# Big-Brother-Pikachu/Where2edit

Hardware: AMD Instinct MI355X
Metric: 1024^2 edited images/sec per mapper step (higher is better)
Workload: dtype f32; 1 GPU; BASELINE configs[1]: FFHQ-1024 StyleGAN2 + clip_loss mapper step (coach.py:79-92), 4 latents/GPU, LevelsMapper, Ranger, id_lambda=0; global_batch=4, per_gpu_batch=4, micro_batch=4, parallelism=dp1, conv_precision=f32, stabilise_steps=6, stabilised=True, hip_graph=True, side_stream=False, clip_precision=f32

## Files before the change

### include/w2e.h

```cpp
#ifndef W2E_H
#define W2E_H

#include <stddef.h>
#include <stdint.h>

#ifdef __cplusplus
extern "C" {
#endif

#define W2E_VERSION 7

int w2e_version(void);
const char* w2e_last_error(void);

int w2e_set_option(const char* name, const char* value);

#define W2E_PLANAR_PITCH(w) ((((w) + 1) + 15) & ~15)
int w2e_get_option(const char* name, int* value);

int w2e_upfirdn2d(const float* x, const float* kern, float* y, int64_t planes, int in_h, int in_w, int out_h,
                  int out_w, int kh, int kw, int up, int down, int pad_x0, int pad_y0, int flip, int in_layout, int in_pitch,
                  int act, const float* out_scale, const float* noise, const float* noise_w, const float* bias,
                  int channels, float slope, float gain, void* stream);
int w2e_blur_adjoint_actbwd(const float* gy, const float* y_fwd, const float* noise, const float* kern, float* gt, float* sums,
                            int64_t planes, int h, int w, float slope, float gain, void* stream);

#define W2E_FIR_GENERIC 0
#define W2E_FIR_DOWN4 1
#define W2E_FIR_TILE 2
#define W2E_FIR_TILE4 3
#define W2E_FIR_BLUR4 4
#define W2E_FIR_STREAM4 5
#define W2E_FIR_PLAN_FIELDS 9
int w2e_upfirdn2d_plan(int64_t planes, int in_h, int in_w, int out_h, int out_w, int kh, int kw, int up, int down, int pad_x0,
                       int in_layout, int in_pitch, int act, int x_misalign, int y_misalign, int64_t* out);
int w2e_upfirdn2d_planar_ok(int kh, int kw, int up, int down, int out_w);
int w2e_blur_adjoint_actbwd_plan(int64_t planes, int h, int w, int kh, int kw, int* fused);

int w2e_bias_act_fwd(const float* x, const float* bias, const float* noise, const float* noise_w, float* y,
                     int64_t outer, int64_t channels, int64_t inner, float slope, float gain, void* stream);
int w2e_bias_act_bwd(const float* gy, const float* y, float* gx, int64_t n, float slope, float gain, void* stream);
int w2e_bias_act_bwd_reduce(const float* gy, const float* y, const float* noise, float* gx, float* sums,
                            int64_t outer, int64_t channels, int64_t inner, float slope, float gain, void* stream);

int w2e_conv_pack(const float* weight, float* wp, int cout, int cin, float scale, int transpose, int flip,
                  void* stream);

#define W2E_CONV_SAME 0
#define W2E_CONV_UP 1
#define W2E_CONV_DOWN 2

int w2e_modconv3x3(int mode, const float* x, const float* wp, const float* in_scale, const float* out_scale,
                   float* y, int batch, int k_ch, int n_ch, int h, int w, int y_pitch, int act, const float* noise,
                   const float* noise_w, const float* bias, const float* dot_with, float* dot_out, void* stream);

#define W2E_CONV_PLAN_FIELDS 15
int w2e_conv3x3_plan(int mode, int batch, int k_ch, int n_ch, int h, int w, int prelu, int down_pad, int64_t* out);

int w2e_modconv_upblur_plan(int batch, int k_ch, int n_ch, int h, int w, int* fused);
int w2e_modconv_upblur(const float* x, const float* wp, const float* in_scale, const float* out_scale, const float* kern,
                       float* y, int batch, int k_ch, int n_ch, int h, int w, const float* noise, const float* noise_w,
                       const float* bias, void* stream);

int w2e_modconv_down_rgbfold_plan(int batch, int k_ch, int n_ch, int h, int w, int* fold);
int w2e_modconv_down_rgbfold(const float* x, const float* wp, const float* in_scale, const float* out_scale, float* gpre, int batch,
                             int k_ch, int n_ch, int h, int w, const float* dot_with, float* dot_out, const float* gy,
                             const float* wrgb, const float* style, const float* noise, float* sums3, float* gw, float slope,
                             float gain, void* stream);

int w2e_wino_weights_fused(const float* wp, float* uf, int k_ch, int n_ch, void* stream);
int w2e_wino_fused(const float* x, const float* in_scale, const float* uf, const float* out_scale, float* y, int batch, int k_ch,
                   int n_ch, int h, int w, int act, const float* noise, const float* noise_w, const float* bias, const float* slope,
                   const float* dot_with, float* dot_out, int wgs, void* stream);

int w2e_wino_pack_input(const float* x, const float* in_scale, float* vf, int batch, int k_ch, int h, int w, int tiles_padded, void* stream);
int w2e_wino_gemm(const float* uf, const float* vf, const float* out_scale, float* y, int batch, int k_ch, int n_ch, int h, int w,
                  int tiles_padded, int splits, float* workspace, int act, const float* noise, const float* noise_w, const float* bias,
                  const float* slope, const float* dot_with, float* dot_out, void* stream);

#define W2E_WINO_GENERATOR 0
#define W2E_WINO_ENCODER 1
#define W2E_WINO_AUTO (-1)
#define W2E_WINO_EPI_PLAIN 0
#define W2E_WINO_EPI_ACT 1
#define W2E_WINO_EPI_PRELU 2
#define W2E_WINO_EPI_DOT 3
#define W2E_WINO_PLAN_FIELDS 6
int w2e_wino_plan(int family, int request, int fused_allowed, int epilogue, int batch, int k_ch, int n_ch, int h, int w, int force_splits,
                  int64_t* out);

int w2e_demod_fwd(const float* s, const float* wsq, float* d, int batch, int cin, int cout, float eps, void* stream);
#define W2E_DEMOD_MAX_LAYERS 32
typedef struct {
    const float* s;
    const float* wsq;
    float* d;
    int cin, cout;
} w2e_demod_layer;
int w2e_demod_all_fwd(const w2e_demod_layer* layers, int n_layers, int batch, float eps, void* stream);
int w2e_demod_bwd(const float* sums, const float* dz, const float* noise_w, const float* bias, const float* d,
                  const float* s, const float* wsq, float* gs, float* gd, int batch, int cin, int cout, void* stream);

int w2e_modconv_wgrad_plan(int mode, int batch, int cin, int cout, int h, int w, int* splits);
int w2e_modconv_wgrad(int mode, const float* g, const float* x, const float* d, const float* s, float* slab, int batch, int cin,
                      int cout, int h, int w, int splits, void* stream);
int w2e_modconv_wgrad_finish(const float* slab, int splits, const float* weight, const float* sums, const float* dz,
                             const float* noise_w, const float* bias, const float* d, const float* s, float* dw, int batch, int cin,
                             int cout, int taps, float scale, void* stream);
int w2e_modconv_wsq(const float* weight, float* wsq, int cout, int cin, int taps, float scale, void* stream);

int w2e_fromrgb_fwd(const float* x, const float* weight, const float* bias, float* y, int batch, int channels, int64_t hw, float scale,
                    void* stream);
int w2e_fromrgb_bwd_rows(int batch, int64_t hw);
int w2e_fromrgb_bwd(const float* gy, const float* y, const float* x, const float* weight, float* gx, float* part, float* dw, float* db,
                    int batch, int channels, int64_t hw, float scale, void* stream);
int w2e_mbstd_fwd(const float* x, float* y, int batch, int channels, int hw, void* stream);
int w2e_mbstd_bwd(const float* gy, const float* x, float* gx, int batch, int channels, int hw, void* stream);
int w2e_fromrgb_jvp(const float* dx, const float* y, const float* weight, float* t, int batch, int channels, int64_t hw, float scale,
                    void* stream);
int w2e_mbstd_jvp(const float* x, const float* dx, float* y, int batch, int channels, int hw, void* stream);
int w2e_mbstd_hvp(const float* gy, const float* x, const float* dx, float* mu, int batch, int channels, int hw, void* stream);
int w2e_sumsq_rows_parts(int64_t n);
int w2e_sumsq_rows(const float* x, float* part, float* out, int batch, int64_t n, void* stream);

int w2e_style_affine_fwd(const float* latent, const float* w, const float* bias, const int* meta, float* out, int batch,
                         int n_latent, int dim, int rows, void* stream);
int w2e_style_affine_bwd(const float* gout, const float* w, const int* meta, float* glatent, int batch, int n_latent,
                         int dim, int rows, void* stream);

int w2e_torgb_fwd(const float* x, const float* wmod, const float* bias, const float* skip, const float* upk,
                  float* y, int batch, int cin, int h, int w, void* stream);
int w2e_torgb_bwd(const float* x, const float* wmod, const float* gy, float* gx, float* gwmod, int batch, int cin,
                  int h, int w, void* stream);
int w2e_torgb_bwd_acc(const float* x, const float* wmod, const float* gy, const float* gx_acc, float* gx, float* gwmod,
                      int batch, int cin, int h, int w, void* stream);
int w2e_torgb_styled_fwd(const float* x, const float* wsc, const float* style, const float* bias, const float* skip,
                         const float* upk, float* y, int batch, int cin, int h, int w, void* stream);
int w2e_torgb_styled_bwd(const float* x, const float* wsc, const float* style, const float* gy, const float* gx_acc,
                         float* gx, float* gstyle, int batch, int cin, int h, int w, void* stream);
int w2e_torgb_bwd_actbwd(const float* x, const float* wmod, const float* style, const float* gy, const float* gx_acc,
                         const float* noise, float* gpre, float* gw, float* sums3, int batch, int cin, int h, int w, float slope,
                         float gain, void* stream);

int w2e_clip_preproc_fwd(const float* img, float* out, int64_t planes, int size, void* stream);
int w2e_clip_preproc_bwd(const float* gout, float* gimg, int64_t planes, int size, void* stream);

int w2e_id_preproc_fwd(const float* img, float* out, int64_t planes, int size, void* stream);
int w2e_id_preproc_bwd(const float* gout, float* gimg, int64_t planes, int size, void* stream);

int w2e_mask_blend_fwd(const float* a, const float* b, const float* mask, float* out, int batch, int channels,
                       int h, int w, int ms, void* stream);
int w2e_mask_blend_bwd(const float* gout, const float* a, const float* b, const float* mask, float* ga, float* gb,
                       float* gmask, int batch, int channels, int h, int w, int ms, void* stream);

int w2e_mapper_pixelnorm(const float* x, float* h, int batch, int n_latent, int groups, const int* l0, const int* len, void* stream);
int w2e_mapper_linear(int mode, const float* a, const float* y_act, float* out, const float* const* w, const float* const* bias,
                      int batch, int n_latent, int groups, const int* l0, const int* len, float w_scale, float b_scale, int scatter,
                      int gathered, void* stream);
int w2e_mapper_wgrad(const float* gy, const float* y, const float* h_in, float* const* gw, float* const* gb, int batch, int n_latent,
                     int groups, const int* l0, const int* len, float w_scale, float b_scale, int gathered, void* stream);

int w2e_ranger_step(int count, float* const* p, const float* const* grad, float* const* exp_avg, float* const* exp_avg_sq,
                    float* const* slow_buffer, const int64_t* numel, const int64_t* row_len, double beta1, double beta2, double eps,
                    double neg_step_size, int rectified, double decay, int lookahead, double alpha, void* stream);

int w2e_adam_step(int count, float* const* p, const float* const* grad, float* const* exp_avg, float* const* exp_avg_sq,
                  const int64_t* numel, double beta1, double beta2, double eps, double step_size, double bias_correction2_sqrt,
                  double weight_decay, void* stream);

int w2e_ssmapper_pixelnorm(const float* const* x, float* h, int batch, int groups, const int* dims, void* stream);
int w2e_ssmapper_gather(const float* const* src, float* dst, int batch, int groups, const int* dims, void* stream);
int w2e_ssmapper_linear(int mode, const float* a, const float* y_act, float* out, const float* const* w, const float* const* bias,
                        int batch, int groups, const int* dims, const float* w_scale, float b_scale, void* stream);
int w2e_ssmapper_wgrad(const float* gy, const float* y, const float* h_in, float* const* gw, float* const* gb, int batch, int groups,
                       const int* dims, const float* w_scale, float b_scale, void* stream);

#ifdef __cplusplus
}
#endif
#endif
```

### where2edit_amd/coach.py

```python
import os

import torch
from torch import nn

from . import dist as w2e_dist
from .clip_loss import CLIPLoss
from .ranger import Ranger
from .styleclip_mapper import StyleCLIPMapper


FUSED_LOSS_TAIL = os.environ.get("W2E_FUSED_LOSS_TAIL", "1") != "0"


class Coach:
    def __init__(self, opts, net=None, clip_loss=None, id_loss=None, text_inputs=None, device=None, data_parallel=False):
        self.opts = opts
        self.global_step = 0
        self.device = device if device is not None else "cuda:0"
        self.opts.device = self.device
        self.net = (net if net is not None else StyleCLIPMapper(self.opts)).to(self.device)
        self.net.decoder.requires_grad_(False)
        if self.opts.id_lambda > 0:
            if id_loss is None:
                from .id_loss import IDLoss
                id_loss = IDLoss(self.opts)
            self.id_loss = id_loss.to(self.device).eval()
        if self.opts.clip_lambda > 0:
            self.clip_loss = (clip_loss if clip_loss is not None else CLIPLoss(opts)).to(self.device)
        if self.opts.latent_l2_lambda > 0:
            self.latent_l2_loss = nn.MSELoss().to(self.device).eval()
        self.optimizer = self.configure_optimizers()
        if text_inputs is None:
            text_inputs = synthetic_tokens(1)
        self.text_inputs = text_inputs.to(self.device)
        self.bucket = w2e_dist.GradBucket(self.net.mapper.parameters()) if data_parallel else None
        self.best_val_loss = None
        self._side = torch.cuda.Stream(device=self.device) if os.environ.get("W2E_SIDE_STREAM", "0") == "1" else None
        self._side_primed = False
        self.merge_forward = os.environ.get("W2E_MERGE_FORWARD", "1") != "0"

    def configure_optimizers(self):
        params = list(self.net.mapper.parameters())
        if self.opts.optim_name == "adam":
            return torch.optim.Adam(params, lr=self.opts.learning_rate)
        return Ranger(params, lr=self.opts.learning_rate)

    def forward_pair(self, w, mask=None):
        dec = self.net.decoder
        s_space = getattr(self.opts, "work_in_stylespace", False)
        att_layer = getattr(self.opts, "attention_layer", 0)
        if mask is not None and att_layer > 0:
            with torch.no_grad():
                x, _, _, feats = dec([w], input_is_latent=True, randomize_noise=False, truncation=1, return_features=True,
                                     input_is_stylespace=s_space)
            self._x_ready = None
            if callable(mask):
                mask = mask(feats)
            if s_space:
                delta = self.net.mapper(w)
                w_hat = [c + 0.1 * dc for c, dc in zip(w, delta)]
                x_hat, _, w_hat = dec([w_hat], input_is_latent=True, return_latents=True, randomize_noise=False, truncation=1,
                                      input_is_stylespace=True, attention_layer=att_layer, attention_map=mask, feature_map=feats)
                return x, x_hat, w_hat
            w_hat = w + 0.1 * self.net.mapper(w)
            x_hat, w_hat, _ = dec([w_hat], input_is_latent=True, return_latents=True, randomize_noise=False, truncation=1,
                                  attention_layer=att_layer, attention_map=mask, feature_map=feats)
            return x, x_hat, w_hat
        if self.merge_forward and self._side is None and s_space and torch.is_grad_enabled():
            from . import functional as K
            n = w[0].shape[0]
            delta = self.net.mapper(w)
            w_hat = [c + 0.1 * dc for c, dc in zip(w, delta)]
            with K.nograd_prefix(n):
                both, _, codes = dec([[torch.cat([c.detach(), ch]) for c, ch in zip(w, w_hat)]], input_is_latent=True, return_latents=True,
                                     randomize_noise=False, truncation=1, input_is_stylespace=True)
            self._x_ready = None
            return both[:n].detach(), K.tail_rows(both, n), [c[n:] for c in codes]
        if self.merge_forward and self._side is None and not s_space and torch.is_grad_enabled():
            from . import functional as K
            n = w.shape[0]
            w_hat = w + 0.1 * self.net.mapper(w)
            with K.nograd_prefix(n):
                both, lat, _ = dec([torch.cat([w.detach(), w_hat])], input_is_latent=True, return_latents=True, randomize_noise=False,
                                   truncation=1)
            self._x_ready = None
            return both[:n].detach(), K.tail_rows(both, n), lat[n:]
        main = torch.cuda.current_stream()
        if self._side is not None and not self._side_primed:
            with torch.no_grad():
                dec([w[:1]] if not s_space else [[c[:1] for c in w]], input_is_latent=True, randomize_noise=False, truncation=1,
                    input_is_stylespace=s_space)
            self._side_primed = True
        if self._side is not None:
            self._side.wait_stream(main)
            with torch.cuda.stream(self._side), torch.no_grad():
                x, _ = dec([w], input_is_latent=True, randomize_noise=False, truncation=1, input_is_stylespace=s_space)
            x.record_stream(main)
            self._x_ready = self._side.record_event()
        else:
            with torch.no_grad():
                x, _ = dec([w], input_is_latent=True, randomize_noise=False, truncation=1, input_is_stylespace=s_space)
            self._x_ready = None
        if s_space:
            delta = self.net.mapper(w)
            w_hat = [c + 0.1 * dc for c, dc in zip(w, delta)]
            x_hat, _, w_hat = dec([w_hat], input_is_latent=True, return_latents=True, randomize_noise=False,
                                  truncation=1, input_is_stylespace=True)
        else:
            w_hat = w + 0.1 * self.net.mapper(w)
            x_hat, w_hat, _ = dec([w_hat], input_is_latent=True, return_latents=True, randomize_noise=False, truncation=1)
        return x, x_hat, w_hat

    def calc_loss(self, w, x, w_hat, x_hat):
        loss_dict = {}
        loss = 0.0
        if getattr(self, "_x_ready", None) is not None:
            torch.cuda.current_stream().wait_event(self._x_ready)
            self._x_ready = None
        if self.opts.id_lambda > 0:
            loss_id, sim_improvement = self.id_loss(x_hat, x)
            loss_dict["loss_id"] = loss_id.detach()
            loss_dict["id_improve"] = sim_improvement
            loss = loss_id * self.opts.id_lambda
        s_space = getattr(self.opts, "work_in_stylespace", False)
        if self.opts.clip_lambda > 0 and self.opts.latent_l2_lambda > 0 and not s_space and torch.is_tensor(w_hat) and w_hat.is_cuda \
                and w_hat.dtype == torch.float32 and torch.is_tensor(w) and w.shape == w_hat.shape and w.dtype == w_hat.dtype \
                and w.device == w_hat.device and FUSED_LOSS_TAIL:
            from . import vit_hip
            sim = self.clip_loss(x_hat, self.text_inputs)
            tail, loss_dict["loss_clip"], loss_dict["loss_l2_latent"] = vit_hip.step_loss(sim, w_hat, w, self.opts.clip_lambda,
                                                                                            self.opts.latent_l2_lambda)
            loss = tail if self.opts.id_lambda <= 0 else loss + tail
            loss_dict["loss"] = loss.detach()
            return loss, loss_dict
        if self.opts.clip_lambda > 0:
            loss_clip = self.clip_loss(x_hat, self.text_inputs).mean()
            loss_dict["loss_clip"] = loss_clip.detach()
            loss = loss + loss_clip * self.opts.clip_lambda
        if self.opts.latent_l2_lambda > 0:
            if getattr(self.opts, "work_in_stylespace", False):
                loss_l2_latent = sum(self.latent_l2_loss(c_hat, c) for c_hat, c in zip(w_hat, w))
            else:
                loss_l2_latent = self.latent_l2_loss(w_hat, w)
            loss_dict["loss_l2_latent"] = loss_l2_latent.detach()
            loss = loss + loss_l2_latent * self.opts.latent_l2_lambda
        loss_dict["loss"] = loss.detach()
        return loss, loss_dict

    def train_step(self, w, mask=None):
        if self.bucket is not None:
            self.bucket.zero()
        else:
            self.optimizer.zero_grad()
        x, x_hat, w_hat = self.forward_pair(w, mask)
        loss, loss_dict = self.calc_loss(w, x, w_hat, x_hat)
        loss.backward()
        if self.bucket is not None:
            self.bucket.all_reduce_mean()
        self.optimizer.step()
        self.global_step += 1
        return loss_dict

    def accumulated_step(self, chunks, step=None):
        if self.bucket is None:
            raise RuntimeError("accumulated_step needs the flat gradient bucket: build the Coach with data_parallel=True")
        n = len(chunks)
        if n == 1:
            return step(chunks[0]) if step is not None else self.train_step(chunks[0])
        if getattr(self, "_acc", None) is None:
            self._acc = torch.zeros_like(self.bucket.flat)
        self._acc.zero_()
        sums = {}
        for c in chunks:
            if c.shape != chunks[0].shape:
                raise ValueError("accumulated_step: micro-batches must have equal shapes (the mean of means is the mean only then)")
            if step is not None:
                d = step(c, finish=False)
            else:
                self.bucket.zero()
                x, x_hat, w_hat = self.forward_pair(c)
                loss, d = self.calc_loss(c, x, w_hat, x_hat)
                loss.backward()
            self._acc.add_(self.bucket.flat, alpha=1.0 / n)
            for k_, v in d.items():
                if torch.is_tensor(v):
                    sums[k_] = v.detach() / n if k_ not in sums else sums[k_] + v.detach() / n
        self.bucket.flat.copy_(self._acc)
        self.bucket.all_reduce_mean()
        self.optimizer.step()
        self.global_step += 1
        return sums

    def capture_step(self, w, mask=None, warmup=3, side_stream=False):
        from . import profiling
        if profiling._active is not None:
            raise RuntimeError("capture_step: per-kernel HIP-event timing cannot be recorded inside a graph")
        eager_side = self._side
        try:
            if side_stream and self._side is None:
                self._side = torch.cuda.Stream(device=self.device)
            s_space = getattr(self.opts, "work_in_stylespace", False)
            static_w = [c.clone() for c in w] if s_space else w.clone()
            static_mask = mask if (mask is None or callable(mask)) else mask.clone()
            params = list(self.net.mapper.parameters())

            def body():
                if self.bucket is not None:
                    self.bucket.zero()
                else:
                    for p in params:
                        p.grad = None
                x, x_hat, w_hat = self.forward_pair(static_w, static_mask)
                loss, loss_dict = self.calc_loss(static_w, x, w_hat, x_hat)
                loss.backward()
                return loss_dict

            graph, static_out = capture_graph(body, "capture_step: the step", self.device, warmup, leaves=params)
        finally:
            self._side = eager_side
        static_grads = [p.grad for p in params]

        def step(w_new, mask_new=None, finish=True):
            if s_space:
                for dst, src in zip(static_w, w_new):
                    dst.copy_(src)
            else:
                static_w.copy_(w_new)
            if static_mask is not None and mask_new is not None and not callable(static_mask):
                static_mask.copy_(mask_new)
            graph.replay()
            if self.bucket is None:
                for p, g in zip(params, static_grads):
                    p.grad = g
            if not finish:
                return static_out
            if self.bucket is not None:
                self.bucket.all_reduce_mean()
            self.optimizer.step()
            self.global_step += 1
            return static_out

        step.graph = graph
        return step

    def train(self, latents, max_steps=None, generator=None):
        self.net.train()
        max_steps = max_steps if max_steps is not None else self.opts.max_steps
        bs = self.opts.batch_size
        log = []
        while self.global_step < max_steps:
            perm = torch.randperm(latents.shape[0], generator=generator)
            for i in range(0, latents.shape[0] - bs + 1, bs):
                if self.global_step >= max_steps:
                    break
                log.append(self.train_step(latents[perm[i:i + bs]].to(self.device)))
        return log

    @torch.no_grad()
    def validate(self, latents):
        self.net.eval()
        agg = []
        bs = getattr(self.opts, "test_batch_size", 1)
        for i in range(0, min(latents.shape[0], 201 * bs) - bs + 1, bs):
# ... 66 lines not shown
```

### where2edit_amd/csrc/common.h

```cpp
#pragma once
#include <hip/hip_runtime.h>
#include <stdarg.h>
#include <stdint.h>
#include <stdio.h>

#include "../../include/w2e.h"

namespace w2e {

void set_error(const char* fmt, ...);
const char* refusal(const char* fmt, ...);

struct Options {
    int conv_precision;
    int deterministic;
    int tune_cfg, tune_cfg_splits, tune_cfg_mode;
    int tune_upall, tune_dma, tune_fuse;
    int tune_upblur;
    int tune_rgbfold;
    int tune_mw;
    int tune_xcd;
    int tune_print, tune_blur, tune_gemm_s;
    int tune_skip, tune_clock;
};
const Options& options();

static inline bool big_lds_once(const void* fn, unsigned* done_mask, int bytes = 160 * 1024) {
    int dev = 0;
    if (hipGetDevice(&dev) != hipSuccess || dev < 0 || dev >= 32) return false;
    if (*done_mask & (1u << dev)) return true;
    if (hipFuncSetAttribute(fn, hipFuncAttributeMaxDynamicSharedMemorySize, bytes) != hipSuccess) {
        (void)hipGetLastError();
        return false;
    }
    *done_mask |= 1u << dev;
    return true;
}

int cu_count();

#define W2E_REQUIRE(cond, ...)        \
    do {                              \
        if (!(cond)) {                \
            w2e::set_error(__VA_ARGS__); \
            return 1;                 \
        }                             \
    } while (0)

#define W2E_LAUNCH_CHECK(name)                                                          \
    do {                                                                                \
        hipError_t e_ = hipGetLastError();                                              \
        if (e_ != hipSuccess) {                                                         \
            w2e::set_error("%s: launch failed: %s", name, hipGetErrorString(e_));       \
            return 2;                                                                   \
        }                                                                               \
    } while (0)

static inline int64_t ceil_div(int64_t a, int64_t b) { return (a + b - 1) / b; }

hipError_t zero_async(void* p, size_t bytes, hipStream_t s);

static inline int stream_grid(int64_t work_items, int block) {
    int64_t g = ceil_div(work_items, block);
    if (g > 2048) g = 2048;
    if (g < 1) g = 1;
    return (int)g;
}

}
```

### where2edit_amd/csrc/elementwise.hip

```cpp
#include "device.h"

namespace w2e {

template <bool VEC4>
__global__ void bias_act_fwd_kernel(const float* __restrict__ x, const float* __restrict__ bias,
                                    const float* __restrict__ noise, const float* __restrict__ noise_w,
                                    float* __restrict__ y, int64_t total, int64_t C, int64_t inner, float slope,
                                    float gain) {
    const float nw = (noise != nullptr) ? noise_w[0] : 0.f;
    const int64_t step = (int64_t)gridDim.x * blockDim.x;
    if (VEC4) {
        const int64_t n4 = total >> 2;
        for (int64_t q = (int64_t)blockIdx.x * blockDim.x + threadIdx.x; q < n4; q += step) {
            const int64_t e = q << 2;
            float4 v = reinterpret_cast<const float4*>(x)[q];
            float add[4] = {0.f, 0.f, 0.f, 0.f};
            if (inner == 1) {
                const int64_t c = e % C;
                if (bias) {
                    const float4 b = *reinterpret_cast<const float4*>(bias + c);
                    add[0] = b.x, add[1] = b.y, add[2] = b.z, add[3] = b.w;
                }
                if (noise) {
                    const float nz = nw * noise[0];
                    add[0] += nz, add[1] += nz, add[2] += nz, add[3] += nz;
                }
            } else {
                const int64_t i = e % inner;
                const float b = bias ? bias[(e / inner) % C] : 0.f;
                add[0] = add[1] = add[2] = add[3] = b;
                if (noise) {
                    const float4 nz = *reinterpret_cast<const float4*>(noise + i);
                    add[0] += nw * nz.x, add[1] += nw * nz.y, add[2] += nw * nz.z, add[3] += nw * nz.w;
                }
            }
            float r[4] = {v.x + add[0], v.y + add[1], v.z + add[2], v.w + add[3]};
#pragma unroll
            for (int k = 0; k < 4; ++k) r[k] = (r[k] > 0.f ? r[k] : r[k] * slope) * gain;
            reinterpret_cast<float4*>(y)[q] = make_float4(r[0], r[1], r[2], r[3]);
        }
    } else {
        for (int64_t e = (int64_t)blockIdx.x * blockDim.x + threadIdx.x; e < total; e += step) {
            const int64_t i = e % inner;
            float v = x[e] + (bias ? bias[(e / inner) % C] : 0.f) + (noise ? nw * noise[i] : 0.f);
            y[e] = (v > 0.f ? v : v * slope) * gain;
        }
    }
}

template <bool VEC4>
__global__ void bias_act_bwd_kernel(const float* __restrict__ gy, const float* __restrict__ y, float* __restrict__ gx,
                                    int64_t total, float slope, float gain) {
    const int64_t step = (int64_t)gridDim.x * blockDim.x;
    if (VEC4) {
        const int64_t n4 = total >> 2;
        for (int64_t q = (int64_t)blockIdx.x * blockDim.x + threadIdx.x; q < n4; q += step) {
            const float4 g = reinterpret_cast<const float4*>(gy)[q];
            const float4 o = reinterpret_cast<const float4*>(y)[q];
            float4 r;
            r.x = g.x * gain * (o.x > 0.f ? 1.f : slope);
            r.y = g.y * gain * (o.y > 0.f ? 1.f : slope);
            r.z = g.z * gain * (o.z > 0.f ? 1.f : slope);
            r.w = g.w * gain * (o.w > 0.f ? 1.f : slope);
            reinterpret_cast<float4*>(gx)[q] = r;
        }
    } else {
        for (int64_t e = (int64_t)blockIdx.x * blockDim.x + threadIdx.x; e < total; e += step)
            gx[e] = gy[e] * gain * (y[e] > 0.f ? 1.f : slope);
    }
}

__global__ void bias_act_bwd_reduce_kernel(const float* __restrict__ gy, const float* __restrict__ y,
                                           const float* __restrict__ noise, float* __restrict__ gx,
                                           float* __restrict__ sums, int64_t inner, int splits, float slope,
                                           float gain) {
    const int64_t row = blockIdx.x / splits;
    const int split = blockIdx.x % splits;
    const int64_t per = ((inner + splits - 1) / splits + 3) & ~int64_t(3);
    const int64_t lo = split * per;
    const int64_t hi = (lo + per < inner) ? lo + per : inner;
    const float* g = gy + row * inner;
    const float* o = y + row * inner;
    float* d = gx + row * inner;
    const float inv_pos = 1.f / gain, inv_neg = 1.f / (gain * slope);
    float s0 = 0.f, s1 = 0.f, s2 = 0.f;
    const bool vec = (inner & 3) == 0;
    if (vec) {
        for (int64_t e = lo + threadIdx.x * 4; e < hi; e += blockDim.x * 4) {
            const float4 gv = *reinterpret_cast<const float4*>(g + e);
            const float4 ov = *reinterpret_cast<const float4*>(o + e);
            float4 nz = make_float4(0.f, 0.f, 0.f, 0.f);
            if (noise) nz = *reinterpret_cast<const float4*>(noise + e);
            const float ga[4] = {gv.x, gv.y, gv.z, gv.w}, oa[4] = {ov.x, ov.y, ov.z, ov.w};
            const float na[4] = {nz.x, nz.y, nz.z, nz.w};
            float r[4];
#pragma unroll
            for (int k = 0; k < 4; ++k) {
                const bool pos = oa[k] > 0.f;
                r[k] = ga[k] * gain * (pos ? 1.f : slope);
                s0 += r[k] * (oa[k] * (pos ? inv_pos : inv_neg));
                s1 += r[k] * na[k];
                s2 += r[k];
            }
            *reinterpret_cast<float4*>(d + e) = make_float4(r[0], r[1], r[2], r[3]);
        }
    } else {
        for (int64_t e = lo + threadIdx.x; e < hi; e += blockDim.x) {
            const bool pos = o[e] > 0.f;
            const float r = g[e] * gain * (pos ? 1.f : slope);
            d[e] = r;
            s0 += r * (o[e] * (pos ? inv_pos : inv_neg));
            s1 += r * (noise ? noise[e] : 0.f);
            s2 += r;
        }
    }
    __shared__ float red[4][3];
    s0 = wave_sum(s0), s1 = wave_sum(s1), s2 = wave_sum(s2);
    const int wave = threadIdx.x >> 6;
    if ((threadIdx.x & 63) == 0) red[wave][0] = s0, red[wave][1] = s1, red[wave][2] = s2;
    __syncthreads();
    if (threadIdx.x < 3) {
        const float t = red[0][threadIdx.x] + red[1][threadIdx.x] + red[2][threadIdx.x] + red[3][threadIdx.x];
        if (splits == 1)
            sums[row * 3 + threadIdx.x] = t;
        else
            atomicAdd(&sums[row * 3 + threadIdx.x], t);
    }
}

__global__ void mask_blend_fwd_kernel(const float* __restrict__ a, const float* __restrict__ b,
                                      const float* __restrict__ mask, float* __restrict__ out, int64_t total, int C,
                                      int H, int W, int ms) {
    const float sy = (float)ms / (float)H, sx = (float)ms / (float)W;
    const int64_t step = (int64_t)gridDim.x * blockDim.x;
    for (int64_t e = (int64_t)blockIdx.x * blockDim.x + threadIdx.x; e < total; e += step) {
        const int x = (int)(e % W);
        const int yy = (int)((e / W) % H);
        const int64_t bi = e / ((int64_t)W * H * C);
        const float m = mask[(bi * ms + nearest_src(yy, sy, ms)) * ms + nearest_src(x, sx, ms)];
        out[e] = m * a[e] + (1.f - m) * b[e];
    }
}

__global__ void mask_blend_bwd_kernel(const float* __restrict__ go, const float* __restrict__ a,
                                      const float* __restrict__ b, const float* __restrict__ mask,
                                      float* __restrict__ ga, float* __restrict__ gb, float* __restrict__ gmask, int C,
                                      int H, int W, int ms) {
    const int bi = blockIdx.x / H, yy = blockIdx.x % H;
    const float sy = (float)ms / (float)H, sx = (float)ms / (float)W;
    const int my = nearest_src(yy, sy, ms);
    for (int x = threadIdx.x; x < W; x += blockDim.x) {
        const int mx = nearest_src(x, sx, ms);
        const float m = mask[((int64_t)bi * ms + my) * ms + mx];
        float acc = 0.f;
        for (int c = 0; c < C; ++c) {
            const int64_t e = (((int64_t)bi * C + c) * H + yy) * W + x;
            const float g = go[e];
            ga[e] = m * g;
            if (gb) gb[e] = (1.f - m) * g;
            if (gmask) acc += g * (a[e] - b[e]);
        }
        if (gmask) atomicAdd(&gmask[((int64_t)bi * ms + my) * ms + mx], acc);
    }
}

__device__ __forceinline__ int overlap(int lo, int hi, int s) {
    const int a = lo > 7 * s ? lo : 7 * s;
    const int b = hi < 7 * s + 7 ? hi : 7 * s + 7;
    return b > a ? b - a : 0;
}

__global__ void clip_preproc_fwd_kernel(const float* __restrict__ img, float* __restrict__ out, int64_t total, int size,
                                        int k) {
    const float inv = 1.f / (float)(k * k);
    const int64_t step = (int64_t)gridDim.x * blockDim.x;
    for (int64_t e = (int64_t)blockIdx.x * blockDim.x + threadIdx.x; e < total; e += step) {
        const int X = (int)(e % 224), Y = (int)((e / 224) % 224);
        const int64_t p = e / (224 * 224);
        const float* src = img + p * (int64_t)size * size;
        const int y0 = (k * Y) / 7, y1 = (k * Y + k - 1) / 7, x0 = (k * X) / 7, x1 = (k * X + k - 1) / 7;
        float acc = 0.f;
        for (int yy = y0; yy <= y1; ++yy) {
            const float wy = (float)overlap(k * Y, k * Y + k, yy);
            float row = 0.f;
            for (int xx = x0; xx <= x1; ++xx) row += (float)overlap(k * X, k * X + k, xx) * src[(int64_t)yy * size + xx];
            acc += wy * row;
        }
        out[e] = acc * inv;
    }
}

__global__ void clip_preproc_bwd_kernel(const float* __restrict__ gout, float* __restrict__ gimg, int64_t total,
                                        int size, int k) {
    const float inv = 1.f / (float)(k * k);
    const int64_t step = (int64_t)gridDim.x * blockDim.x;
    for (int64_t e = (int64_t)blockIdx.x * blockDim.x + threadIdx.x; e < total; e += step) {
        const int x = (int)(e % size), y = (int)((e / size) % size);
        const int64_t p = e / ((int64_t)size * size);
        const float* g = gout + p * 224 * 224;
        const int Y0 = (7 * y) / k, Y1 = (7 * y + 6) / k, X0 = (7 * x) / k, X1 = (7 * x + 6) / k;
        float acc = 0.f;
        for (int Y = Y0; Y <= Y1; ++Y) {
            const float wy = (float)overlap(k * Y, k * Y + k, y);
            float row = 0.f;
            for (int X = X0; X <= X1; ++X) row += (float)overlap(k * X, k * X + k, x) * g[Y * 224 + X];
            acc += wy * row;
        }
        gimg[e] = acc * inv;
    }
}

__device__ __forceinline__ int apool_lo(int i) { return (i * 188) / 112; }
__device__ __forceinline__ int apool_hi(int i) { return ((i + 1) * 188 + 111) / 112; }

__global__ void id_preproc_fwd_kernel(const float* __restrict__ img, float* __restrict__ out, int64_t total, int size, int k) {
    const int64_t step = (int64_t)gridDim.x * blockDim.x;
    const float inv_k2 = 1.f / (float)(k * k);
    for (int64_t e = (int64_t)blockIdx.x * blockDim.x + threadIdx.x; e < total; e += step) {
        const int X = (int)(e % 112), Y = (int)((e / 112) % 112);
        const float* src = img + (e / (112 * 112)) * (int64_t)size * size;
        const int r0 = apool_lo(Y), r1 = apool_hi(Y), c0 = apool_lo(X), c1 = apool_hi(X);
        float acc = 0.f;
        for (int r = r0; r < r1; ++r)
            for (int c = c0; c < c1; ++c) {
                const float* blk = src + (int64_t)(35 + r) * k * size + (32 + c) * k;
                float s = 0.f;
                for (int a = 0; a < k; ++a)
                    for (int b = 0; b < k; ++b) s += blk[a * size + b];
                acc += s * inv_k2;
            }
        out[e] = acc / (float)((r1 - r0) * (c1 - c0));
    }
}

__global__ void id_preproc_bwd_kernel(const float* __restrict__ gout, float* __restrict__ gimg, int64_t total, int size, int k) {
    const int64_t step = (int64_t)gridDim.x * blockDim.x;
    const float inv_k2 = 1.f / (float)(k * k);
    for (int64_t e = (int64_t)blockIdx.x * blockDim.x + threadIdx.x; e < total; e += step) {
        const int x = (int)(e % size), y = (int)((e / size) % size);
        const float* g = gout + (e / ((int64_t)size * size)) * 112 * 112;
        const int r = y / k - 35, c = x / k - 32;
        float acc = 0.f;
        if (r >= 0 && r < 188 && c >= 0 && c < 188) {
            const int Yc = (r * 112) / 188, Xc = (c * 112) / 188;
            for (int Y = Yc - 1; Y <= Yc + 1; ++Y) {
                if (Y < 0 || Y >= 112 || r < apool_lo(Y) || r >= apool_hi(Y)) continue;
                const float wy = 1.f / (float)(apool_hi(Y) - apool_lo(Y));
                for (int X = Xc - 1; X <= Xc + 1; ++X) {
                    if (X < 0 || X >= 112 || c < apool_lo(X) || c >= apool_hi(X)) continue;
                    acc += wy / (float)(apool_hi(X) - apool_lo(X)) * g[Y * 112 + X];
                }
            }
        }
        gimg[e] = acc * inv_k2;
    }
}

__global__ __launch_bounds__(256) void demod_fwd_kernel(const float* __restrict__ s, const float* __restrict__ wsq,
                                                        float* __restrict__ d, int B, int Cin, int Cout, float eps) {
    const int lane = threadIdx.x & 63;
    const int row = blockIdx.x * 4 + (threadIdx.x >> 6);
    if (row >= B * Cout) return;
    const int b = row / Cout, o = row - b * Cout;
    float acc = 0.f;
    for (int i = lane; i < Cin; i += 64) {
        const float v = s[(int64_t)b * Cin + i];
        acc += v * v * wsq[(int64_t)o * Cin + i];
    }
    acc = wave_sum(acc);
    if (lane == 0) d[row] = rsqrtf(acc + eps);
}

struct DemodAllLaunch {
    w2e_demod_layer layer[W2E_DEMOD_MAX_LAYERS];
    int batch;
    float eps;
};

__global__ __launch_bounds__(256) void demod_all_fwd_kernel(const DemodAllLaunch L) {
    const w2e_demod_layer& y = L.layer[blockIdx.y];
    const int lane = threadIdx.x & 63;
    const int row = blockIdx.x * 4 + (threadIdx.x >> 6);
    if (row >= L.batch * y.cout) return;
    const int b = row / y.cout, o = row - b * y.cout;
    const float* s = y.s + (int64_t)b * y.cin;
    const float* w = y.wsq + (int64_t)o * y.cin;
    float acc = 0.f;
    for (int i = lane; i < y.cin; i += 64) {
        const float v = s[i];
        acc += v * v * w[i];
    }
    acc = wave_sum(acc);
    if (lane == 0) y.d[row] = rsqrtf(acc + L.eps);
}

constexpr int DEMOD_OCH = 32;
__global__ __launch_bounds__(256) void demod_bwd_kernel(const float* __restrict__ sums, const float* __restrict__ dz_in,
                                                        const float* __restrict__ noise_w, const float* __restrict__ bias,
                                                        const float* __restrict__ d, const float* __restrict__ s,
                                                        const float* __restrict__ wsq, float* __restrict__ gs,
                                                        float* __restrict__ gd_out, int Cin, int Cout) {
    __shared__ float coef[DEMOD_OCH];
    const int b = blockIdx.y;
    const float nw = noise_w ? noise_w[0] : 0.f;
    const bool serial = gridDim.z == 1 && Cout > DEMOD_OCH;
    const int i_ser = blockIdx.x * 256 + threadIdx.x;
    float total = 0.f;
    for (int o_lo = blockIdx.z * DEMOD_OCH; o_lo < Cout; o_lo += DEMOD_OCH) {
    const int o_n = (Cout - o_lo < DEMOD_OCH) ? Cout - o_lo : DEMOD_OCH;
    __syncthreads();
    for (int oo = threadIdx.x; oo < o_n; oo += 256) {
        const int o = o_lo + oo;
        float dz;
        if (sums) {
            const float* q = sums + ((int64_t)b * Cout + o) * 3;
            dz = q[0] - nw * q[1] - (bias ? bias[o] : 0.f) * q[2];
        } else {
            dz = dz_in[(int64_t)b * Cout + o];
        }
        const float dv = d[(int64_t)b * Cout + o];
        coef[oo] = dz * dv * dv;
        if (gd_out && blockIdx.x == 0) gd_out[(int64_t)b * Cout + o] = dz / dv;
    }
    __syncthreads();
    const int i = blockIdx.x * 256 + threadIdx.x;
    float acc = 0.f;
    if (i < Cin) {
        const float* wq = wsq + (int64_t)o_lo * Cin + i;
#pragma unroll 16
        for (int oo = 0; oo < o_n; ++oo) acc += coef[oo] * wq[(int64_t)oo * Cin];
    }
    if (!serial) {
        if (i < Cin) atomicAdd(&gs[(int64_t)b * Cin + i], -s[(int64_t)b * Cin + i] * acc);
        return;
    }
    total += acc;
    }
    if (i_ser < Cin) gs[(int64_t)b * Cin + i_ser] += -s[(int64_t)b * Cin + i_ser] * total;
}


__global__ __launch_bounds__(256) void style_affine_fwd_kernel(const float* __restrict__ latent, const float* __restrict__ w,
                                                               const float* __restrict__ bias, const int4* __restrict__ meta,
                                                               float* __restrict__ out, int B, int L, int D, int R) {
    const int lane = threadIdx.x & 63;
    const int r = blockIdx.x * 4 + (threadIdx.x >> 6);
    if (r >= R) return;
    const int4 m = meta[r];
    const float bs = bias ? bias[r] : 0.f;
    for (int b = 0; b < B; ++b) {
        const float* lat = latent + ((int64_t)b * L + m.x) * D;
        float acc = 0.f;
        for (int k = lane * 4; k < D; k += 256) {
            const float4 wv = *reinterpret_cast<const float4*>(w + (int64_t)r * D + k);
            const float4 lv = *reinterpret_cast<const float4*>(lat + k);
            acc += wv.x * lv.x + wv.y * lv.y + wv.z * lv.z + wv.w * lv.w;
        }
        acc = wave_sum(acc);
        if (lane == 0) out[(int64_t)m.y * B + (int64_t)b * m.z + m.w] = acc + bs;
    }
}

__global__ __launch_bounds__(256) void style_affine_bwd_kernel(const float* __restrict__ gout, const float* __restrict__ w,
                                                               const int4* __restrict__ meta, float* __restrict__ glatent,
                                                               int B, int L, int D, int R) {
    __shared__ float g[32];
    const int b = blockIdx.y;
    const bool serial = gridDim.x == 1 && R > 32;
    for (int r0 = blockIdx.x * 32; r0 < R; r0 += 32) {
    __syncthreads();
    if (threadIdx.x < 32) {
        const int r = r0 + threadIdx.x;
        float v = 0.f;
        if (r < R) {
            const int4 m = meta[r];
            v = gout[(int64_t)m.y * B + (int64_t)b * m.z + m.w];
        }
        g[threadIdx.x] = v;
    }
    __syncthreads();
    const int widx = meta[r0].x;
    const int nr = (R - r0 < 32) ? R - r0 : 32;
    for (int k = threadIdx.x; k < D; k += 256) {
        float acc = 0.f;
#pragma unroll 8
        for (int i = 0; i < nr; ++i) acc += g[i] * w[(int64_t)(r0 + i) * D + k];
        if (serial) glatent[((int64_t)b * L + widx) * D + k] += acc;
        else atomicAdd(&glatent[((int64_t)b * L + widx) * D + k], acc);
    }
    if (!serial) break;
    }
}

}

using namespace w2e;

extern "C" {


int w2e_bias_act_fwd(const float* x, const float* bias, const float* noise, const float* noise_w, float* y,
                     int64_t outer, int64_t channels, int64_t inner, float slope, float gain, void* stream) {
    W2E_REQUIRE(x && y, "bias_act_fwd: null tensor");
    W2E_REQUIRE(outer >= 0 && channels > 0 && inner > 0, "bias_act_fwd: bad dims %lld %lld %lld", (long long)outer,
                (long long)channels, (long long)inner);
    W2E_REQUIRE(!noise || noise_w, "bias_act_fwd: noise without noise_w");
    const int64_t total = outer * channels * inner;
    if (total == 0) return 0;
    const bool vec = ((inner & 3) == 0) || (inner == 1 && (channels & 3) == 0 && !noise);
    hipStream_t s = (hipStream_t)stream;
    if (vec)
        bias_act_fwd_kernel<true><<<stream_grid(total / 4, 256), 256, 0, s>>>(x, bias, noise, noise_w, y, total,
                                                                                channels, inner, slope, gain);
    else
        bias_act_fwd_kernel<false><<<stream_grid(total, 256), 256, 0, s>>>(x, bias, noise, noise_w, y, total, channels,
                                                                             inner, slope, gain);
    W2E_LAUNCH_CHECK("bias_act_fwd");
    return 0;
}

int w2e_bias_act_bwd(const float* gy, const float* y, float* gx, int64_t n, float slope, float gain, void* stream) {
    W2E_REQUIRE(gy && y && gx, "bias_act_bwd: null tensor");
    if (n <= 0) return 0;
    hipStream_t s = (hipStream_t)stream;
    if ((n & 3) == 0)
        bias_act_bwd_kernel<true><<<stream_grid(n / 4, 256), 256, 0, s>>>(gy, y, gx, n, slope, gain);
    else
        bias_act_bwd_kernel<false><<<stream_grid(n, 256), 256, 0, s>>>(gy, y, gx, n, slope, gain);
    W2E_LAUNCH_CHECK("bias_act_bwd");
    return 0;
}

int w2e_bias_act_bwd_reduce(const float* gy, const float* y, const float* noise, float* gx, float* sums,
                            int64_t outer, int64_t channels, int64_t inner, float slope, float gain, void* stream) {
    W2E_REQUIRE(gy && y && gx && sums, "bias_act_bwd_reduce: null tensor");
    W2E_REQUIRE(slope != 0.f && gain != 0.f, "bias_act_bwd_reduce: slope and gain must be non-zero");
    const int64_t rows = outer * channels;
    if (rows == 0 || inner == 0) return 0;
    hipStream_t s = (hipStream_t)stream;
    int splits = 1;
    if (rows < 2048 && !options().deterministic) {
        splits = (int)ceil_div(2048, rows);
        const int64_t max_splits = ceil_div(inner, 1024);
        if (splits > max_splits) splits = (int)max_splits;
        if (splits < 1) splits = 1;
    }
    W2E_REQUIRE(rows * splits < (int64_t)1 << 31, "bias_act_bwd_reduce: grid too large");
    if (splits > 1 && zero_async(sums, sizeof(float) * 3 * rows, s) != hipSuccess) {
        set_error("bias_act_bwd_reduce: memset failed");
        return 2;
    }
    bias_act_bwd_reduce_kernel<<<(int)(rows * splits), 256, 0, s>>>(gy, y, noise, gx, sums, inner, splits, slope, gain);
    W2E_LAUNCH_CHECK("bias_act_bwd_reduce");
    return 0;
}

int w2e_mask_blend_fwd(const float* a, const float* b, const float* mask, float* out, int batch, int channels, int h,
                       int w, int ms, void* stream) {
    W2E_REQUIRE(a && b && mask && out, "mask_blend_fwd: null tensor");
    W2E_REQUIRE(batch >= 0 && channels > 0 && h > 0 && w > 0 && ms > 0, "mask_blend_fwd: bad dims");
    const int64_t total = (int64_t)batch * channels * h * w;
    if (total == 0) return 0;
    mask_blend_fwd_kernel<<<stream_grid(total, 256), 256, 0, (hipStream_t)stream>>>(a, b, mask, out, total, channels, h,
                                                                                     w, ms);
    W2E_LAUNCH_CHECK("mask_blend_fwd");
    return 0;
}

int w2e_mask_blend_bwd(const float* gout, const float* a, const float* b, const float* mask, float* ga, float* gb,
                       float* gmask, int batch, int channels, int h, int w, int ms, void* stream) {
    W2E_REQUIRE(gout && mask && ga, "mask_blend_bwd: null tensor");
    W2E_REQUIRE(!gmask || (a && b), "mask_blend_bwd: gmask needs a and b");
    W2E_REQUIRE(batch >= 0 && channels > 0 && h > 0 && w > 0 && ms > 0, "mask_blend_bwd: bad dims");
    if (batch == 0) return 0;
    hipStream_t s = (hipStream_t)stream;
    W2E_REQUIRE(!(options().deterministic && gmask && (h != ms || w != ms)),
                "mask_blend_bwd: deterministic mode needs the mask at the feature resolution (%dx%d vs %d)", h, w, ms);
    if (gmask && zero_async(gmask, sizeof(float) * (size_t)batch * ms * ms, s) != hipSuccess) {
        set_error("mask_blend_bwd: memset failed");
        return 2;
    }
    const int threads = w >= 256 ? 256 : (w >= 128 ? 128 : 64);
    mask_blend_bwd_kernel<<<batch * h, threads, 0, s>>>(gout, a, b, mask, ga, gb, gmask, channels, h, w, ms);
    W2E_LAUNCH_CHECK("mask_blend_bwd");
    return 0;
}

int w2e_clip_preproc_fwd(const float* img, float* out, int64_t planes, int size, void* stream) {
    W2E_REQUIRE(img && out, "clip_preproc_fwd: null tensor");
    W2E_REQUIRE(size >= 32 && size % 32 == 0, "clip_preproc_fwd: size %d must be a positive multiple of 32", size);
    const int64_t total = planes * 224 * 224;
    if (total <= 0) return 0;
    clip_preproc_fwd_kernel<<<stream_grid(total, 256), 256, 0, (hipStream_t)stream>>>(img, out, total, size, size / 32);
    W2E_LAUNCH_CHECK("clip_preproc_fwd");
    return 0;
}

int w2e_clip_preproc_bwd(const float* gout, float* gimg, int64_t planes, int size, void* stream) {
    W2E_REQUIRE(gout && gimg, "clip_preproc_bwd: null tensor");
    W2E_REQUIRE(size >= 32 && size % 32 == 0, "clip_preproc_bwd: size %d must be a positive multiple of 32", size);
    const int64_t total = planes * (int64_t)size * size;
    if (total <= 0) return 0;
    clip_preproc_bwd_kernel<<<stream_grid(total, 256), 256, 0, (hipStream_t)stream>>>(gout, gimg, total, size, size / 32);
    W2E_LAUNCH_CHECK("clip_preproc_bwd");
    return 0;
}

int w2e_demod_fwd(const float* s, const float* wsq, float* d, int batch, int cin, int cout, float eps, void* stream) {
    W2E_REQUIRE(s && wsq && d, "demod_fwd: null tensor");
    W2E_REQUIRE(batch >= 0 && cin > 0 && cout > 0, "demod_fwd: bad dims");
    if (batch == 0) return 0;
    demod_fwd_kernel<<<(unsigned)ceil_div((int64_t)batch * cout, 4), 256, 0, (hipStream_t)stream>>>(s, wsq, d, batch, cin, cout, eps);
    W2E_LAUNCH_CHECK("demod_fwd");
    return 0;
}

int w2e_demod_all_fwd(const w2e_demod_layer* layers, int n_layers, int batch, float eps, void* stream) {
    W2E_REQUIRE(layers, "demod_all_fwd: null layers");
    W2E_REQUIRE(n_layers >= 1 && n_layers <= W2E_DEMOD_MAX_LAYERS, "demod_all_fwd: 1 <= n_layers <= %d", W2E_DEMOD_MAX_LAYERS);
    W2E_REQUIRE(batch >= 0, "demod_all_fwd: bad dims");
    if (batch == 0) return 0;
    DemodAllLaunch L{};
    int max_cout = 0;
    for (int j = 0; j < n_layers; ++j) {
        W2E_REQUIRE(layers[j].s && layers[j].wsq && layers[j].d && layers[j].cin > 0 && layers[j].cout > 0,
                    "demod_all_fwd: layer %d: null tensor or bad dims", j);
        L.layer[j] = layers[j];
        if (layers[j].cout > max_cout) max_cout = layers[j].cout;
    }
    L.batch = batch, L.eps = eps;
    dim3 grid((unsigned)ceil_div((int64_t)batch * max_cout, 4), (unsigned)n_layers);
    demod_all_fwd_kernel<<<grid, 256, 0, (hipStream_t)stream>>>(L);
    W2E_LAUNCH_CHECK("demod_all_fwd");
    return 0;
}

int w2e_demod_bwd(const float* sums, const float* dz, const float* noise_w, const float* bias, const float* d,
                  const float* s, const float* wsq, float* gs, float* gd, int batch, int cin, int cout, void* stream) {
    W2E_REQUIRE((sums != nullptr) != (dz != nullptr), "demod_bwd: give exactly one of sums / dz");
    W2E_REQUIRE(d && s && wsq && gs, "demod_bwd: null tensor");
    W2E_REQUIRE(batch >= 0 && cin > 0 && cout > 0 && batch < 65536, "demod_bwd: bad dims");
    if (batch == 0) return 0;
    dim3 grid((unsigned)ceil_div(cin, 256), (unsigned)batch, options().deterministic ? 1u : (unsigned)ceil_div(cout, DEMOD_OCH));
    demod_bwd_kernel<<<grid, 256, 0, (hipStream_t)stream>>>(sums, dz, noise_w, bias, d, s, wsq, gs, gd, cin, cout);
    W2E_LAUNCH_CHECK("demod_bwd");
    return 0;
}

int w2e_id_preproc_fwd(const float* img, float* out, int64_t planes, int size, void* stream) {
    W2E_REQUIRE(img && out, "id_preproc_fwd: null tensor");
    W2E_REQUIRE(size >= 256 && size % 256 == 0, "id_preproc_fwd: size %d must be a positive multiple of 256", size);
    const int64_t total = planes * 112 * 112;
    if (total <= 0) return 0;
    id_preproc_fwd_kernel<<<stream_grid(total, 256), 256, 0, (hipStream_t)stream>>>(img, out, total, size, size / 256);
    W2E_LAUNCH_CHECK("id_preproc_fwd");
    return 0;
}

int w2e_id_preproc_bwd(const float* gout, float* gimg, int64_t planes, int size, void* stream) {
    W2E_REQUIRE(gout && gimg, "id_preproc_bwd: null tensor");
    W2E_REQUIRE(size >= 256 && size % 256 == 0, "id_preproc_bwd: size %d must be a positive multiple of 256", size);
    const int64_t total = planes * (int64_t)size * size;
    if (total <= 0) return 0;
    id_preproc_bwd_kernel<<<stream_grid(total, 256), 256, 0, (hipStream_t)stream>>>(gout, gimg, total, size, size / 256);
    W2E_LAUNCH_CHECK("id_preproc_bwd");
    return 0;
}

int w2e_style_affine_fwd(const float* latent, const float* w, const float* bias, const int* meta, float* out, int batch,
                         int n_latent, int dim, int rows, void* stream) {
    W2E_REQUIRE(latent && w && meta && out, "style_affine_fwd: null tensor");
    W2E_REQUIRE(batch >= 0 && n_latent > 0 && dim > 0 && (dim & 3) == 0 && rows > 0, "style_affine_fwd: bad dims");
    if (batch == 0) return 0;
    style_affine_fwd_kernel<<<(unsigned)ceil_div(rows, 4), 256, 0, (hipStream_t)stream>>>(
        latent, w, bias, reinterpret_cast<const int4*>(meta), out, batch, n_latent, dim, rows);
    W2E_LAUNCH_CHECK("style_affine_fwd");
    return 0;
}

int w2e_style_affine_bwd(const float* gout, const float* w, const int* meta, float* glatent, int batch, int n_latent,
                         int dim, int rows, void* stream) {
    W2E_REQUIRE(gout && w && meta && glatent, "style_affine_bwd: null tensor");
    W2E_REQUIRE(batch >= 0 && batch < 65536 && n_latent > 0 && dim > 0 && rows > 0, "style_affine_bwd: bad dims");
    if (batch == 0) return 0;
    if (zero_async(glatent, sizeof(float) * (size_t)batch * n_latent * dim, (hipStream_t)stream) != hipSuccess) {
        set_error("style_affine_bwd: memset failed");
        return 2;
    }
    dim3 grid(options().deterministic ? 1u : (unsigned)ceil_div(rows, 32), (unsigned)batch);
    style_affine_bwd_kernel<<<grid, 256, 0, (hipStream_t)stream>>>(gout, w, reinterpret_cast<const int4*>(meta), glatent, batch,
                                                                 n_latent, dim, rows);
    W2E_LAUNCH_CHECK("style_affine_bwd");
    return 0;
}


}
```

### where2edit_amd/csrc/runtime.hip

```cpp
#include <stdlib.h>
#include <string.h>

#include "common.h"

namespace w2e {

static thread_local char g_err[512] = "";

void set_error(const char* fmt, ...) {
    va_list ap;
    va_start(ap, fmt);
    vsnprintf(g_err, sizeof(g_err), fmt, ap);
    va_end(ap);
}

const char* refusal(const char* fmt, ...) {
    static thread_local char text[256];
    va_list ap;
    va_start(ap, fmt);
    vsnprintf(text, sizeof(text), fmt, ap);
    va_end(ap);
    return text;
}

static Options g_opt;

static int parse_precision(const char* v) { return (v && strcmp(v, "bf16x3") == 0) ? 1 : 0; }

static bool apply(Options& o, const char* name, const char* value) {
    const int iv = value ? atoi(value) : 0;
    if (!strcmp(name, "conv_precision")) o.conv_precision = parse_precision(value);
    else if (!strcmp(name, "deterministic")) o.deterministic = iv != 0;
    else if (!strcmp(name, "tune_cfg")) {
        o.tune_cfg = -1, o.tune_cfg_splits = 1, o.tune_cfg_mode = -1;
        if (value && *value) sscanf(value, "%d,%d,%d", &o.tune_cfg, &o.tune_cfg_splits, &o.tune_cfg_mode);
    } else if (!strcmp(name, "tune_upall")) o.tune_upall = (value && *value) ? iv : -1;
    else if (!strcmp(name, "tune_dma")) o.tune_dma = (value && *value) ? iv : -1;
    else if (!strcmp(name, "tune_print")) o.tune_print = iv;
    else if (!strcmp(name, "tune_blur")) o.tune_blur = iv;
    else if (!strcmp(name, "tune_gemm_s")) o.tune_gemm_s = iv;
    else if (!strcmp(name, "tune_fuse")) o.tune_fuse = (value && *value) ? iv : -1;
    else if (!strcmp(name, "tune_xcd")) o.tune_xcd = (value && *value) ? iv : -1;
    else if (!strcmp(name, "tune_mw")) o.tune_mw = (value && *value) ? iv : -1;
    else if (!strcmp(name, "tune_upblur")) o.tune_upblur = (value && *value) ? iv : -1;
    else if (!strcmp(name, "tune_rgbfold")) o.tune_rgbfold = (value && *value) ? iv : -1;
#ifdef W2E_TUNING
    else if (!strcmp(name, "tune_skip")) o.tune_skip = iv;
    else if (!strcmp(name, "tune_clock")) o.tune_clock = iv;
#endif
    else return false;
    return true;
}

static Options from_env() {
    Options o{};
    o.tune_cfg = -1, o.tune_cfg_splits = 1, o.tune_cfg_mode = -1, o.tune_upall = -1, o.tune_dma = -1, o.tune_fuse = -1, o.tune_xcd = -1, o.tune_mw = -1, o.tune_upblur = -1, o.tune_rgbfold = -1;
    static const char* const kEnv[][2] = {
        {"W2E_CONV_PRECISION", "conv_precision"}, {"W2E_DETERMINISTIC", "deterministic"}, {"W2E_TUNE_CFG", "tune_cfg"},
        {"W2E_TUNE_UPALL", "tune_upall"},         {"W2E_TUNE_DMA", "tune_dma"},           {"W2E_TUNE_PRINT", "tune_print"},
        {"W2E_TUNE_BLUR", "tune_blur"},           {"W2E_TUNE_GEMM_S", "tune_gemm_s"},     {"W2E_TUNE_FUSE", "tune_fuse"},
        {"W2E_TUNE_SKIP", "tune_skip"},           {"W2E_TUNE_CLOCK", "tune_clock"},       {"W2E_TUNE_XCD", "tune_xcd"},
        {"W2E_TUNE_MW", "tune_mw"},               {"W2E_TUNE_UPBLUR", "tune_upblur"},
        {"W2E_TUNE_RGBFOLD", "tune_rgbfold"}};
    for (const auto& e : kEnv)
        if (const char* v = getenv(e[0])) apply(o, e[1], v);
    return o;
}

struct OptionsInit {
    OptionsInit() { g_opt = from_env(); }
};
static OptionsInit g_opt_init;

const Options& options() { return g_opt; }

int cu_count() {
    static int cached[32];
    int dev = 0;
    if (hipGetDevice(&dev) != hipSuccess || dev < 0 || dev >= 32) return 256;
    if (!cached[dev]) {
        hipDeviceProp_t prop;
        cached[dev] = (hipGetDeviceProperties(&prop, dev) == hipSuccess && prop.multiProcessorCount > 0) ? prop.multiProcessorCount : 256;
    }
    return cached[dev];
}

__global__ void zero_kernel(unsigned* __restrict__ p, size_t words) {
    const size_t step = (size_t)gridDim.x * blockDim.x;
    for (size_t i = (size_t)blockIdx.x * blockDim.x + threadIdx.x; i < words; i += step) p[i] = 0u;
}

__global__ void zero4_kernel(uint4* __restrict__ p, size_t quads) {
    const size_t step = (size_t)gridDim.x * blockDim.x;
    for (size_t i = (size_t)blockIdx.x * blockDim.x + threadIdx.x; i < quads; i += step) p[i] = make_uint4(0u, 0u, 0u, 0u);
}

hipError_t zero_async(void* p, size_t bytes, hipStream_t s) {
    if (bytes == 0) return hipSuccess;
    if ((bytes & 3) != 0 || ((uintptr_t)p & 3) != 0) return hipErrorInvalidValue;
    if (((uintptr_t)p & 15) == 0 && (bytes & 15) == 0) {
        const size_t quads = bytes >> 4;
        zero4_kernel<<<stream_grid((int64_t)quads, 256), 256, 0, s>>>(reinterpret_cast<uint4*>(p), quads);
    } else {
        const size_t words = bytes >> 2;
        zero_kernel<<<stream_grid((int64_t)words, 256), 256, 0, s>>>(reinterpret_cast<unsigned*>(p), words);
    }
    return hipGetLastError();
}

}

extern "C" {

int w2e_version(void) { return W2E_VERSION; }
const char* w2e_last_error(void) { return w2e::g_err; }

int w2e_set_option(const char* name, const char* value) {
    W2E_REQUIRE(name != nullptr, "set_option: null name");
    W2E_REQUIRE(w2e::apply(w2e::g_opt, name, value), "set_option: unknown option '%s'", name);
    return 0;
}

int w2e_get_option(const char* name, int* value) {
    W2E_REQUIRE(name && value, "get_option: null argument");
    const w2e::Options& o = w2e::g_opt;
    if (!strcmp(name, "conv_precision")) *value = o.conv_precision;
    else if (!strcmp(name, "deterministic")) *value = o.deterministic;
    else if (!strcmp(name, "tune_cfg")) *value = o.tune_cfg;
    else if (!strcmp(name, "tune_fuse")) *value = o.tune_fuse;
    else if (!strcmp(name, "tune_blur")) *value = o.tune_blur;
    else if (!strcmp(name, "tune_upblur")) *value = o.tune_upblur;
    else if (!strcmp(name, "tune_rgbfold")) *value = o.tune_rgbfold;
    else if (!strcmp(name, "tuning_build")) {
#ifdef W2E_TUNING
        *value = 1;
#else
        *value = 0;
#endif
    } else W2E_REQUIRE(false, "get_option: unknown option '%s'", name);
    return 0;
}

}
```

### where2edit_amd/csrc/torgb.hip

```cpp
#include "device.h"

namespace w2e {

template <int CG, int V>
__global__ __launch_bounds__(256) void torgb_fwd_kernel(const float* __restrict__ x, const float* __restrict__ wmod,
                                                        const float* __restrict__ style,
                                                        const float* __restrict__ bias, const float* __restrict__ skip,
                                                        const float* __restrict__ upk, float* __restrict__ y, int cin,
                                                        int H, int W) {
    constexpr int PQ = 256 / CG;
    extern __shared__ __attribute__((aligned(16))) float smem[];
    float* wsm = smem;
    float* red = smem + 3 * cin;
    __shared__ float kf[16];
    const int b = blockIdx.y, tid = threadIdx.x;
    const int64_t HW = (int64_t)H * W;
    if (style) {
        for (int i = tid; i < cin; i += 256) {
            const float st = style[(int64_t)b * cin + i];
            wsm[i] = wmod[i] * st, wsm[cin + i] = wmod[cin + i] * st, wsm[2 * cin + i] = wmod[2 * cin + i] * st;
        }
    } else {
        for (int i = tid; i < 3 * cin; i += 256) wsm[i] = wmod[(int64_t)b * 3 * cin + i];
    }
    if (tid < 16 && skip) kf[tid] = upk[15 - tid];
    __syncthreads();
    const int cg = tid / PQ, pq = tid % PQ;
    const int64_t p0 = ((int64_t)blockIdx.x * PQ + pq) * V;
    float acc[3][V];
#pragma unroll
    for (int c = 0; c < 3; ++c)
#pragma unroll
        for (int v = 0; v < V; ++v) acc[c][v] = 0.f;
    if (p0 < HW) {
        const float* xp = x + (int64_t)b * cin * HW + p0;
#pragma unroll 4
        for (int i = cg; i < cin; i += CG) {
            float xv[V];
            if (V == 4) {
                const float4 t = *reinterpret_cast<const float4*>(xp + i * HW);
                xv[0] = t.x, xv[1] = t.y, xv[2] = t.z, xv[3] = t.w;
            } else {
                xv[0] = xp[i * HW];
            }
            const float w0 = wsm[i], w1 = wsm[cin + i], w2 = wsm[2 * cin + i];
#pragma unroll
            for (int v = 0; v < V; ++v) acc[0][v] += w0 * xv[v], acc[1][v] += w1 * xv[v], acc[2][v] += w2 * xv[v];
        }
    }
    if (CG > 1) {
#pragma unroll
        for (int c = 0; c < 3; ++c)
#pragma unroll
            for (int v = 0; v < V; ++v) red[(cg * PQ + pq) * 3 * V + c * V + v] = acc[c][v];
        __syncthreads();
        if (cg != 0) return;
        for (int g = 1; g < CG; ++g)
#pragma unroll
            for (int c = 0; c < 3; ++c)
#pragma unroll
                for (int v = 0; v < V; ++v) acc[c][v] += red[(g * PQ + pq) * 3 * V + c * V + v];
    }
    if (p0 >= HW) return;
    const int Hs = H >> 1, Ws = W >> 1;
#pragma unroll
    for (int c = 0; c < 3; ++c) {
        const float bs = bias ? bias[c] : 0.f;
#pragma unroll
        for (int v = 0; v < V; ++v) {
            float r = acc[c][v] + bs;
            if (skip) {
                const int py = (int)((p0 + v) / W), px = (int)((p0 + v) % W);
                const float* sp = skip + ((int64_t)b * 3 + c) * Hs * Ws;
                float u = 0.f;
#pragma unroll
                for (int a = 0; a < 2; ++a) {
                    const int ky = (py & 1) + 2 * a, sy = (py + ky - 2) >> 1;
                    if (py + ky - 2 < 0 || sy >= Hs) continue;
#pragma unroll
                    for (int d = 0; d < 2; ++d) {
                        const int kx = (px & 1) + 2 * d, sx = (px + kx - 2) >> 1;
                        if (px + kx - 2 < 0 || sx >= Ws) continue;
                        u += kf[ky * 4 + kx] * sp[sy * Ws + sx];
                    }
                }
                r += u;
            }
            acc[c][v] = r;
        }
        float* dst = y + ((int64_t)b * 3 + c) * HW + p0;
        if (V == 4) *reinterpret_cast<float4*>(dst) = make_float4(acc[c][0], acc[c][1], acc[c][2], acc[c][3]);
        else dst[0] = acc[c][0];
    }
}

template <int V, bool ACC, bool ACTB>
__global__ __launch_bounds__(256) void torgb_bwd_kernel(const float* __restrict__ x, const float* __restrict__ wmod,
                                                        const float* __restrict__ style,
                                                        const float* __restrict__ gy, const float* __restrict__ gx_acc,
                                                        float* __restrict__ gx, float* __restrict__ gwmod, int cin,
                                                        int64_t HW, int splits, int64_t per_split,
                                                        const float* __restrict__ noise, float* __restrict__ sums3, float slope, float gain) {
    const int lane = threadIdx.x & 63, wave = threadIdx.x >> 6;
    const int split = blockIdx.x % splits;
    const int i = (blockIdx.x / splits) * 4 + wave;
    const int b = blockIdx.y;
    if (i >= cin) return;
    float w0, w1, w2;
    if (style) {
        const float st = style[(int64_t)b * cin + i];
        w0 = wmod[i] * st, w1 = wmod[cin + i] * st, w2 = wmod[2 * cin + i] * st;
    } else {
        w0 = wmod[((int64_t)b * 3 + 0) * cin + i], w1 = wmod[((int64_t)b * 3 + 1) * cin + i],
        w2 = wmod[((int64_t)b * 3 + 2) * cin + i];
    }
    const float* xp = x + ((int64_t)b * cin + i) * HW;
    float* gp = gx + ((int64_t)b * cin + i) * HW;
    const float* ap = ACC ? gx_acc + ((int64_t)b * cin + i) * HW : nullptr;
    const float* g0 = gy + (int64_t)b * 3 * HW;
    const int64_t lo = split * per_split, hi = (lo + per_split < HW) ? lo + per_split : HW;
    float s0 = 0.f, s1 = 0.f, s2 = 0.f;
    float t_pre = 0.f, t_noise = 0.f, t_sum = 0.f;
    const float inv_pos = 1.f / gain, inv_neg = 1.f / (gain * slope);
    auto act_bwd = [&](float r, float xval, float nz) __attribute__((always_inline)) {
        const bool pos = xval > 0.f;
        const float g = r * gain * (pos ? 1.f : slope);
        t_pre += g * (xval * (pos ? inv_pos : inv_neg)), t_noise += g * nz, t_sum += g;
        return g;
    };
    if (V == 4) {
#pragma unroll 2
        for (int64_t p = lo + lane * 4; p < hi; p += 256) {
            const float4 xv = *reinterpret_cast<const float4*>(xp + p);
            const float4 a = *reinterpret_cast<const float4*>(g0 + p);
            const float4 bb = *reinterpret_cast<const float4*>(g0 + HW + p);
            const float4 c = *reinterpret_cast<const float4*>(g0 + 2 * HW + p);
            float4 nz = make_float4(0.f, 0.f, 0.f, 0.f);
            if (ACTB && noise) nz = *reinterpret_cast<const float4*>(noise + p);
            float4 r;
            r.x = w0 * a.x + w1 * bb.x + w2 * c.x;
            r.y = w0 * a.y + w1 * bb.y + w2 * c.y;
            r.z = w0 * a.z + w1 * bb.z + w2 * c.z;
            r.w = w0 * a.w + w1 * bb.w + w2 * c.w;
            if (ACC) {
                const float4 av = *reinterpret_cast<const float4*>(ap + p);
                r.x += av.x, r.y += av.y, r.z += av.z, r.w += av.w;
            }
            if (ACTB) r.x = act_bwd(r.x, xv.x, nz.x), r.y = act_bwd(r.y, xv.y, nz.y), r.z = act_bwd(r.z, xv.z, nz.z), r.w = act_bwd(r.w, xv.w, nz.w);
            *reinterpret_cast<float4*>(gp + p) = r;
            s0 += xv.x * a.x + xv.y * a.y + xv.z * a.z + xv.w * a.w;
            s1 += xv.x * bb.x + xv.y * bb.y + xv.z * bb.z + xv.w * bb.w;
            s2 += xv.x * c.x + xv.y * c.y + xv.z * c.z + xv.w * c.w;
        }
    } else {
        for (int64_t p = lo + lane; p < hi; p += 64) {
            const float xv = xp[p], a = g0[p], bb = g0[HW + p], c = g0[2 * HW + p];
            float r = w0 * a + w1 * bb + w2 * c + (ACC ? ap[p] : 0.f);
            if (ACTB) r = act_bwd(r, xv, noise ? noise[p] : 0.f);
            gp[p] = r;
            s0 += xv * a, s1 += xv * bb, s2 += xv * c;
        }
    }
    if (ACTB) {
        t_pre = wave_sum(t_pre), t_noise = wave_sum(t_noise), t_sum = wave_sum(t_sum);
        if (lane == 0) {
            float* d3 = sums3 + ((int64_t)b * cin + i) * 3;
            if (splits == 1) d3[0] = t_pre, d3[1] = t_noise, d3[2] = t_sum;
            else atomicAdd(d3, t_pre), atomicAdd(d3 + 1, t_noise), atomicAdd(d3 + 2, t_sum);
        }
    }
    s0 = wave_sum(s0), s1 = wave_sum(s1), s2 = wave_sum(s2);
    if (lane == 0) {
        if (style) {
            const float g = wmod[i] * s0 + wmod[cin + i] * s1 + wmod[2 * cin + i] * s2;
            float* d = gwmod + (int64_t)b * cin + i;
            if (splits == 1) d[0] = g;
            else atomicAdd(d, g);
        } else {
            float* d = gwmod + (int64_t)b * 3 * cin + i;
            if (splits == 1) d[0] = s0, d[cin] = s1, d[2 * cin] = s2;
            else atomicAdd(d, s0), atomicAdd(d + cin, s1), atomicAdd(d + 2 * cin, s2);
        }
    }
}

}

using namespace w2e;

static int torgb_fwd_impl(const float* x, const float* wmod, const float* style, const float* bias, const float* skip,
                          const float* upk, float* y, int batch, int cin, int h, int w, void* stream) {
    W2E_REQUIRE(x && wmod && y, "torgb_fwd: null tensor");
    W2E_REQUIRE(batch >= 0 && cin > 0 && h > 0 && w > 0, "torgb_fwd: bad dims");
    W2E_REQUIRE(!skip || (upk && (h % 2 == 0) && (w % 2 == 0)), "torgb_fwd: skip needs the 4x4 kernel and even h,w");
    W2E_REQUIRE(batch < 65536, "torgb_fwd: batch too large");
    if (batch == 0) return 0;
    hipStream_t s = (hipStream_t)stream;
    const int64_t hw = (int64_t)h * w;
    const bool vec = (hw & 3) == 0;
    const int v = vec ? 4 : 1;
    const int64_t groups = ceil_div(hw, v);
    const int cg = groups >= 16384 ? 1 : (groups >= 1024 ? 4 : 16);
    const int pq = 256 / cg;
    dim3 grid((unsigned)ceil_div(groups, pq), (unsigned)batch);
    const size_t lds = sizeof(float) * ((size_t)3 * cin + (cg > 1 ? (size_t)256 * 3 * v : 0));
#define W2E_TORGB(CG, V) torgb_fwd_kernel<CG, V><<<grid, 256, lds, s>>>(x, wmod, style, bias, skip, upk, y, cin, h, w)
    if (vec) {
        if (cg == 1) W2E_TORGB(1, 4);
        else if (cg == 4) W2E_TORGB(4, 4);
        else W2E_TORGB(16, 4);
    } else {
        if (cg == 1) W2E_TORGB(1, 1);
        else if (cg == 4) W2E_TORGB(4, 1);
        else W2E_TORGB(16, 1);
    }
#undef W2E_TORGB
    W2E_LAUNCH_CHECK("torgb_fwd");
    return 0;
}

extern "C" int w2e_torgb_fwd(const float* x, const float* wmod, const float* bias, const float* skip, const float* upk,
                             float* y, int batch, int cin, int h, int w, void* stream) {
    return torgb_fwd_impl(x, wmod, nullptr, bias, skip, upk, y, batch, cin, h, w, stream);
}

extern "C" int w2e_torgb_styled_fwd(const float* x, const float* wsc, const float* style, const float* bias, const float* skip,
                                    const float* upk, float* y, int batch, int cin, int h, int w, void* stream) {
    W2E_REQUIRE(style, "torgb_styled_fwd: null style");
    return torgb_fwd_impl(x, wsc, style, bias, skip, upk, y, batch, cin, h, w, stream);
}

static int torgb_bwd_impl(const float* x, const float* wmod, const float* style, const float* gy, const float* gx_acc,
                          float* gx, float* gwmod, int batch, int cin, int h, int w, void* stream, bool actb = false,
                          const float* noise = nullptr, float* sums3 = nullptr, float slope = 0.f, float gain = 1.f);

extern "C" int w2e_torgb_bwd(const float* x, const float* wmod, const float* gy, float* gx, float* gwmod, int batch,
                             int cin, int h, int w, void* stream) {
    return torgb_bwd_impl(x, wmod, nullptr, gy, nullptr, gx, gwmod, batch, cin, h, w, stream);
}

extern "C" int w2e_torgb_bwd_acc(const float* x, const float* wmod, const float* gy, const float* gx_acc, float* gx,
                                 float* gwmod, int batch, int cin, int h, int w, void* stream) {
    return torgb_bwd_impl(x, wmod, nullptr, gy, gx_acc, gx, gwmod, batch, cin, h, w, stream);
}

extern "C" int w2e_torgb_styled_bwd(const float* x, const float* wsc, const float* style, const float* gy,
                                    const float* gx_acc, float* gx, float* gstyle, int batch, int cin, int h, int w,
                                    void* stream) {
    W2E_REQUIRE(style, "torgb_styled_bwd: null style");
    return torgb_bwd_impl(x, wsc, style, gy, gx_acc, gx, gstyle, batch, cin, h, w, stream);
}

extern "C" int w2e_torgb_bwd_actbwd(const float* x, const float* wmod, const float* style, const float* gy, const float* gx_acc,
                                    const float* noise, float* gpre, float* gw, float* sums3, int batch, int cin, int h, int w,
                                    float slope, float gain, void* stream) {
    W2E_REQUIRE(sums3, "torgb_bwd_actbwd: null sums");
    W2E_REQUIRE(gain > 0.f && slope > 0.f, "torgb_bwd_actbwd: gain and slope must be positive");
    return torgb_bwd_impl(x, wmod, style, gy, gx_acc, gpre, gw, batch, cin, h, w, stream, true, noise, sums3, slope, gain);
}

static int torgb_bwd_impl(const float* x, const float* wmod, const float* style, const float* gy, const float* gx_acc,
                          float* gx, float* gwmod, int batch, int cin, int h, int w, void* stream, bool actb, const float* noise,
                          float* sums3, float slope, float gain) {
    W2E_REQUIRE(x && wmod && gy && gx && gwmod, "torgb_bwd: null tensor");
    W2E_REQUIRE(batch >= 0 && cin > 0 && h > 0 && w > 0, "torgb_bwd: bad dims");
    W2E_REQUIRE(batch < 65536, "torgb_bwd: batch too large");
    if (batch == 0) return 0;
    hipStream_t s = (hipStream_t)stream;
    const int64_t hw = (int64_t)h * w;
    const int64_t waves = (int64_t)batch * cin;
    int splits = 1;
    if (waves < 8192 && !options().deterministic) {
        splits = (int)ceil_div(8192, waves);
        const int64_t max_splits = ceil_div(hw, 4096);
        if (splits > max_splits) splits = (int)max_splits;
    }
    int64_t per_split = ceil_div(hw, splits);
    per_split = (per_split + 255) & ~int64_t(255);
    splits = (int)ceil_div(hw, per_split);
    if (splits > 1 && (zero_async(gwmod, sizeof(float) * (style ? 1 : 3) * (size_t)batch * cin, s) != hipSuccess ||
                       (actb && zero_async(sums3, sizeof(float) * 3 * (size_t)batch * cin, s) != hipSuccess))) {
        set_error("torgb_bwd: memset failed");
        return 2;
    }
    dim3 grid((unsigned)(ceil_div(cin, 4) * splits), (unsigned)batch);
#define W2E_TORGB_BWD(V, ACC, ACTB) \
    torgb_bwd_kernel<V, ACC, ACTB><<<grid, 256, 0, s>>>(x, wmod, style, gy, gx_acc, gx, gwmod, cin, hw, splits, per_split, noise, sums3, slope, gain)
    if ((hw & 3) == 0) {
        if (actb) {
            if (gx_acc) W2E_TORGB_BWD(4, true, true);
            else W2E_TORGB_BWD(4, false, true);
        } else {
            if (gx_acc) W2E_TORGB_BWD(4, true, false);
            else W2E_TORGB_BWD(4, false, false);
        }
    } else {
        if (actb) {
            if (gx_acc) W2E_TORGB_BWD(1, true, true);
            else W2E_TORGB_BWD(1, false, true);
        } else {
            if (gx_acc) W2E_TORGB_BWD(1, true, false);
            else W2E_TORGB_BWD(1, false, false);
        }
    }
#undef W2E_TORGB_BWD
    W2E_LAUNCH_CHECK("torgb_bwd");
    return 0;
}
```

### where2edit_amd/csrc/upfirdn2d.hip

```cpp
#include <stdlib.h>

#include "common.h"

namespace w2e {

constexpr int MAXK = 16;

#ifdef W2E_TUNING
#define W2E_BLUR_SKIP(p, bit) (((p).tune & (bit)) != 0)
#else
#define W2E_BLUR_SKIP(p, bit) false
#endif

struct UpfirdnParams {
    const float* x;
    const float* kern;
    float* y;
    int64_t planes;
    int in_h, in_w, out_h, out_w, kh, kw, up, down, pad_x0, pad_y0, flip;
    int tune;
    int planar;
    int act;
    const float* out_scale;
    const float* noise;
    const float* noise_w;
    const float* bias;
    int channels;
    float slope, gain;
    const float* y_fwd;
    float* sums;
};

__device__ __forceinline__ float epilogue(const UpfirdnParams& p, float v, int64_t plane, int oy, int ox, float nw) {
    if (!p.act) return v;
    if (p.out_scale) v *= p.out_scale[plane];
    if (p.noise) v += nw * p.noise[(int64_t)oy * p.out_w + ox];
    if (p.bias) v += p.bias[plane % p.channels];
    return (v > 0.f ? v : v * p.slope) * p.gain;
}

constexpr int TW = 64, TH = 32;
constexpr int MAX_TILE_K = 8;

template <bool ACT>
__global__ __launch_bounds__(256) void upfirdn_tile4_kernel(UpfirdnParams p, int tiles_x, int tiles_y, unsigned pw_magic) {
    extern __shared__ __attribute__((aligned(16))) float smem[];
    float* tile = smem;
    constexpr int PW = TW + 3, PH = TH + 3, PITCH = (PW + 3) & ~3;
    const int tid = threadIdx.x;
    float kr[16];
#pragma unroll
    for (int i = 0; i < 16; ++i) kr[i] = p.flip ? p.kern[15 - i] : p.kern[i];
    const float nw = (ACT && p.noise) ? p.noise_w[0] : 0.f;
    const int tiles_per_plane = tiles_x * tiles_y;
    const int n_tiles = tiles_per_plane * (int)p.planes;
    const int ly = (tid >> 4) * 2, lx = (tid & 15) * 4;
    for (int t = blockIdx.x; t < n_tiles; t += gridDim.x) {
        const int plane = t / tiles_per_plane;
        const int rem = t - plane * tiles_per_plane;
        const int ty = rem / tiles_x, tx = rem - ty * tiles_x;
        const float* src = p.x + (int64_t)plane * p.in_h * p.in_w;
        const int oy0 = ty * TH, ox0 = tx * TW;
        const int iy0 = oy0 - p.pad_y0, ix0 = ox0 - p.pad_x0;
        __syncthreads();
#pragma unroll
        for (int it = 0; it < (PH * PW + 255) / 256; ++it) {
            const int i = tid + it * 256;
            const int r = (int)__umulhi((unsigned)i, pw_magic), c = i - r * PW;
            const int iy = iy0 + r, ix = ix0 + c;
            const bool ok = iy >= 0 && iy < p.in_h && ix >= 0 && ix < p.in_w;
            const int cy = iy < 0 ? 0 : (iy >= p.in_h ? p.in_h - 1 : iy), cx = ix < 0 ? 0 : (ix >= p.in_w ? p.in_w - 1 : ix);
            const float v = W2E_BLUR_SKIP(p, 1) ? 1.f : src[cy * p.in_w + cx];
            if (i < PH * PW) tile[r * PITCH + c] = ok ? v : 0.f;
        }
        __syncthreads();
        float acc0[4] = {0.f, 0.f, 0.f, 0.f}, acc1[4] = {0.f, 0.f, 0.f, 0.f};
#pragma unroll
        for (int r = 0; r < (W2E_BLUR_SKIP(p, 2) ? 1 : 5); ++r) {
            const float4 a = *reinterpret_cast<const float4*>(tile + (ly + r) * PITCH + lx);
            const float4 b = *reinterpret_cast<const float4*>(tile + (ly + r) * PITCH + lx + 4);
            const float win[8] = {a.x, a.y, a.z, a.w, b.x, b.y, b.z, b.w};
#pragma unroll
            for (int kx = 0; kx < 4; ++kx) {
#pragma unroll
                for (int j = 0; j < 4; ++j) {
                    if (r < 4) acc0[j] += kr[r * 4 + kx] * win[kx + j];
                    if (r >= 1) acc1[j] += kr[(r - 1) * 4 + kx] * win[kx + j];
                }
            }
        }
        const int ox = ox0 + lx;
        float e_scale = 1.f, e_bias = 0.f;
        if (ACT) {
            if (p.out_scale) e_scale = p.out_scale[plane];
            if (p.bias) e_bias = p.bias[plane % p.channels];
        }
#pragma unroll
        for (int yy = 0; yy < 2; ++yy) {
            const int oy = oy0 + ly + yy;
            if (oy >= p.out_h || ox >= p.out_w) continue;
            float v[4];
#pragma unroll
            for (int j = 0; j < 4; ++j) {
                float e = yy ? acc1[j] : acc0[j];
                if (ACT) {
                    e = e * e_scale + e_bias;
                    if (p.noise) e += nw * p.noise[oy * p.out_w + (ox + j < p.out_w ? ox + j : ox)];
                    e = (e > 0.f ? e : e * p.slope) * p.gain;
                }
                v[j] = e;
            }
            float* dst = p.y + ((int64_t)plane * p.out_h + oy) * p.out_w + ox;
            if (W2E_BLUR_SKIP(p, 4) && v[0] != 123456.75f) continue;
            if (ox + 3 < p.out_w && (p.out_w & 3) == 0) {
                *reinterpret_cast<float4*>(dst) = make_float4(v[0], v[1], v[2], v[3]);
            } else {
#pragma unroll
                for (int j = 0; j < 4; ++j)
                    if (ox + j < p.out_w) dst[j] = v[j];
            }
        }
    }
}

template <bool ACT, bool PLANAR>
__global__ __launch_bounds__(256) void upfirdn_blur4_kernel(UpfirdnParams p, int tiles_x, int tiles_y) {
    extern __shared__ __attribute__((aligned(16))) float smem[];
    constexpr int PW = TW + 3, PH = TH + 3;
    constexpr int NQ = PLANAR ? ((PW + 1) / 2 + 1 + 3) / 4 + 1 : (PW + 3) / 4 + 1;
    constexpr int PE = 4 * NQ;
    constexpr int SLOTS = (PLANAR ? 2 : 1) * PH * NQ;
    constexpr int NIT = (SLOTS + 255) / 256;
    static_assert(TW == 64 && TH == 32, "thread mapping: 64 lanes along x, 4 waves x 8 rows");
    const int tid = threadIdx.x;
    float kr[16];
#pragma unroll
    for (int i = 0; i < 16; ++i) kr[i] = p.flip ? p.kern[15 - i] : p.kern[i];
    float kh[4], kv[4];
    bool separable = kr[0] != 0.f;
    {
        float kmax = 0.f;
#pragma unroll
        for (int i = 0; i < 16; ++i) kmax = fmaxf(kmax, fabsf(kr[i]));
#pragma unroll
        for (int i = 0; i < 4; ++i) kh[i] = kr[i], kv[i] = separable ? kr[4 * i] / kr[0] : 0.f;
#pragma unroll
        for (int i = 0; i < 16; ++i) separable = separable && fabsf(kr[i] - kv[i >> 2] * kh[i & 3]) <= 1e-7f * kmax;
    }
    const float nw = (ACT && p.noise) ? p.noise_w[0] : 0.f;
    const int hp = (p.in_h + 1) >> 1, wpp = W2E_PLANAR_PITCH((p.in_w - 1) >> 1);
    const int64_t plane_stride = PLANAR ? (int64_t)4 * hp * wpp : (int64_t)p.in_h * p.in_w;
    const int row_len = PLANAR ? wpp : p.in_w;

    const int tx = blockIdx.x % tiles_x, g0 = blockIdx.x / tiles_x, gstep = gridDim.x / tiles_x;
    const int ox0 = tx * TW, ix0 = ox0 - p.pad_x0;
// ... 550 lines not shown
    return up == 1 && down == 1 && kh == 4 && kw == 4 && out_w >= MIN_TILE_W;
}

static int plan_stream4(const char* name, int64_t planes, int out_h, int lanes, FirPlan* pl) {
    const int col_groups = (int)ceil_div(lanes, 64), strips = (int)ceil_div(out_h, SR);
    const int64_t waves = planes * col_groups * strips;
    W2E_REQUIRE(waves < ((int64_t)1 << 31), "%s: tensor too large", name);
    pl->kernel = W2E_FIR_STREAM4, pl->grid = ceil_div(waves, 4), pl->block = 256, pl->lds = 0;
    pl->args[0] = col_groups, pl->args[1] = strips;
    return 0;
}

static int fir_plan(int64_t planes, int in_h, int in_w, int out_h, int out_w, int kh, int kw, int up, int down, int pad_x0, int in_layout,
                    int in_pitch, int act, unsigned x_misalign, unsigned y_misalign, const Options& opt, FirPlan* pl) {
    *pl = FirPlan{};
    W2E_REQUIRE(planes >= 0 && in_h > 0 && in_w > 0 && out_h >= 0 && out_w >= 0, "upfirdn2d: bad sizes");
    W2E_REQUIRE(kh >= 1 && kw >= 1 && kh <= MAXK && kw <= MAXK, "upfirdn2d: kernel %dx%d unsupported (max %d)", kh, kw,
                MAXK);
    W2E_REQUIRE(up >= 1 && down >= 1, "upfirdn2d: up/down must be >= 1");
    const int64_t total = planes * out_h * out_w;
    if (total == 0) return 0;
    W2E_REQUIRE(in_layout == 0 || (in_layout == 1 && planar_ok(kh, kw, up, down, out_w)),
                "upfirdn2d: the phase-planar input layout is implemented for the 4x4, up=down=1 tile kernel only");
    W2E_REQUIRE(in_layout == 0 || in_pitch == W2E_PLANAR_PITCH((in_w - 1) >> 1),
                "upfirdn2d: planar input with a row pitch of %d floats, this library's layout has %d (W2E_PLANAR_PITCH, ABI %d): rebuild the caller",
                in_pitch, W2E_PLANAR_PITCH((in_w - 1) >> 1), W2E_VERSION);
    const int tune = opt.tune_blur;
    pl->act = act != 0, pl->block = 256;
    if (up == 1 && down == 1 && out_w >= MIN_TILE_W && kh <= MAX_TILE_K && kw <= MAX_TILE_K) {
        const int tiles_x = (int)ceil_div(out_w, TW), tiles_y = (int)ceil_div(out_h, TH);
        const int64_t n_tiles = planes * tiles_x * tiles_y;
        W2E_REQUIRE(n_tiles < ((int64_t)1 << 31) && (int64_t)in_h * in_w < ((int64_t)1 << 31), "upfirdn2d: tensor too large");
        const bool aligned_x = x_misalign == 0;
        pl->args[0] = tiles_x, pl->args[1] = tiles_y;
        if (kh == 4 && kw == 4) {
            pl->planar = in_layout;
            const bool vec = !in_layout && (in_w & 3) == 0 && aligned_x;
            const bool stream_ok = !(tune & 8) && out_w >= 256 && aligned_x && y_misalign == 0 &&
                                   (in_layout ? (pad_x0 == 1 && (out_w & 3) == 0 && in_w == out_w + 1)
                                              : (pad_x0 == 2 && (in_w & 3) == 0 && out_w <= in_w + 1));
            if (stream_ok) {
                const int lanes = (!in_layout && out_w == in_w + 1) ? out_w / 4 : (int)ceil_div(out_w, 4);
                return plan_stream4("upfirdn2d", planes, out_h, lanes, pl);
            }
            if (in_layout || vec) {
                const int64_t items = planes * tiles_y;
                int gsteps = 256 * 8 / tiles_x;
                if (gsteps < 1) gsteps = 1;
                if (gsteps > items) gsteps = (int)items;
                constexpr int PWc = TW + 3, PHc = TH + 3;
                pl->kernel = W2E_FIR_BLUR4, pl->grid = gsteps * tiles_x;
                pl->lds = in_layout ? sizeof(float) * 2 * PHc * 4 * (((PWc + 1) / 2 + 1 + 3) / 4 + 1) : sizeof(float) * PHc * 4 * ((PWc + 3) / 4 + 1);
                return 0;
            }
        }
        const int pw = TW + kw - 1, pitch = (pw + 3) & ~3;
        pl->kernel = (kh == 4 && kw == 4) ? W2E_FIR_TILE4 : W2E_FIR_TILE;
        pl->grid = n_tiles < 16384 ? n_tiles : 16384;
        pl->lds = sizeof(float) * (MAXK * MAXK + (size_t)(TH + kh) * pitch + 16);
        pl->args[2] = (unsigned)(((uint64_t)1 << 32) / (unsigned)pw + 1);
    } else if (up == 1 && kh == 4 && kw == 4 && !act && !in_layout && planes * in_h * in_w < ((int64_t)1 << 29) && total < ((int64_t)1 << 31)) {
        pl->kernel = W2E_FIR_DOWN4, pl->grid = ceil_div(total, 256), pl->args[0] = total;
    } else {
        pl->kernel = W2E_FIR_GENERIC, pl->grid = stream_grid(total, 256), pl->args[0] = total;
    }
    return 0;
}

static int fir_plan_actbwd(int64_t planes, int h, int w, const Options& opt, FirPlan* pl) {
    *pl = FirPlan{};
    W2E_REQUIRE(planes >= 0 && h > 0 && w >= 256 && (w & 3) == 0, "blur_adjoint_actbwd: needs a width >= 256 that is a multiple of 4 (got %dx%d)", h, w);
    W2E_REQUIRE(!opt.deterministic, "blur_adjoint_actbwd: the sums are joined with fp32 atomics (use w2e_bias_act_bwd_reduce + w2e_upfirdn2d in deterministic mode)");
    if (planes == 0) return 0;
    W2E_REQUIRE((int64_t)(h + 1) * (w + 1) < ((int64_t)1 << 29), "blur_adjoint_actbwd: plane too large");
    pl->actbwd = 1;
    return plan_stream4("blur_adjoint_actbwd", planes, h + 1, w / 4, pl);
}

static void fir_print(const FirPlan& pl, const UpfirdnParams& p) {
    fprintf(stderr, "upfirdn variant kernel %s act %d planar %d actbwd %d up %d down %d taps %dx%d %lld %dx%d -> %dx%d\n", kFirNames[pl.kernel], pl.act,
            pl.planar, pl.actbwd, p.up, p.down, p.kh, p.kw, (long long)p.planes, p.in_h, p.in_w, p.out_h, p.out_w);
}

static void launch_args(void (*k)(UpfirdnParams, int, int, unsigned), const FirPlan& pl, const UpfirdnParams& p, hipStream_t s) {
    k<<<(unsigned)pl.grid, pl.block, pl.lds, s>>>(p, (int)pl.args[0], (int)pl.args[1], (unsigned)pl.args[2]);
}
static void launch_args(void (*k)(UpfirdnParams, int, int), const FirPlan& pl, const UpfirdnParams& p, hipStream_t s) {
    k<<<(unsigned)pl.grid, pl.block, pl.lds, s>>>(p, (int)pl.args[0], (int)pl.args[1]);
}
static void launch_args(void (*k)(UpfirdnParams, int64_t), const FirPlan& pl, const UpfirdnParams& p, hipStream_t s) {
    k<<<(unsigned)pl.grid, pl.block, pl.lds, s>>>(p, pl.args[0]);
}
template <auto KERNEL>
static void launch_kernel(const FirPlan& pl, const UpfirdnParams& p, hipStream_t s) {
    launch_args(KERNEL, pl, p, s);
}

struct FirEntry {
    int kernel, act, planar, actbwd;
    void (*launch)(const FirPlan&, const UpfirdnParams&, hipStream_t);
};
static const FirEntry kFirTable[] = {
    {W2E_FIR_GENERIC, -1, -1, 0, launch_kernel<upfirdn_generic_kernel>},
    {W2E_FIR_DOWN4, -1, -1, 0, launch_kernel<upfirdn_down4_kernel>},
    {W2E_FIR_TILE, -1, -1, 0, launch_kernel<upfirdn_tile_kernel>},
    {W2E_FIR_TILE4, 0, -1, 0, launch_kernel<upfirdn_tile4_kernel<false>>},
    {W2E_FIR_TILE4, 1, -1, 0, launch_kernel<upfirdn_tile4_kernel<true>>},
    {W2E_FIR_BLUR4, 0, 0, 0, launch_kernel<upfirdn_blur4_kernel<false, false>>},
    {W2E_FIR_BLUR4, 1, 0, 0, launch_kernel<upfirdn_blur4_kernel<true, false>>},
    {W2E_FIR_BLUR4, 0, 1, 0, launch_kernel<upfirdn_blur4_kernel<false, true>>},
    {W2E_FIR_BLUR4, 1, 1, 0, launch_kernel<upfirdn_blur4_kernel<true, true>>},
    {W2E_FIR_STREAM4, 0, 0, 0, launch_kernel<upfirdn_stream4_kernel<false, false>>},
    {W2E_FIR_STREAM4, 1, 0, 0, launch_kernel<upfirdn_stream4_kernel<true, false>>},
    {W2E_FIR_STREAM4, 0, 1, 0, launch_kernel<upfirdn_stream4_kernel<false, true>>},
    {W2E_FIR_STREAM4, 1, 1, 0, launch_kernel<upfirdn_stream4_kernel<true, true>>},
    {W2E_FIR_STREAM4, 0, 0, 1, launch_kernel<upfirdn_stream4_kernel<false, false, true>>},
};

static int fir_launch(const FirPlan& pl, const UpfirdnParams& p, hipStream_t s) {
    for (const FirEntry& e : kFirTable) {
        if (e.kernel == pl.kernel && (e.act < 0 || e.act == pl.act) && (e.planar < 0 || e.planar == pl.planar) && e.actbwd == pl.actbwd) {
            e.launch(pl, p, s);
            return 0;
        }
    }
    set_error("upfirdn2d: internal: kernel %s act %d planar %d actbwd %d not instantiated", kFirNames[pl.kernel], pl.act, pl.planar, pl.actbwd);
    return 1;
}

}

using namespace w2e;

extern "C" int w2e_upfirdn2d(const float* x, const float* kern, float* y, int64_t planes, int in_h, int in_w, int out_h,
                             int out_w, int kh, int kw, int up, int down, int pad_x0, int pad_y0, int flip, int in_layout, int in_pitch,
                             int act, const float* out_scale, const float* noise, const float* noise_w, const float* bias,
                             int channels, float slope, float gain, void* stream) {
    W2E_REQUIRE(x && kern && y, "upfirdn2d: null tensor");
    W2E_REQUIRE(!noise || noise_w, "upfirdn2d: noise without noise_w");
    W2E_REQUIRE(!act || !bias || channels > 0, "upfirdn2d: bias needs channels");
    const Options& opt = options();
    FirPlan pl;
    const int rc = fir_plan(planes, in_h, in_w, out_h, out_w, kh, kw, up, down, pad_x0, in_layout, in_pitch, act, (unsigned)((uintptr_t)x & 15),
                            (unsigned)((uintptr_t)y & 15), opt, &pl);
    if (rc != 0 || pl.grid == 0) return rc;
    const UpfirdnParams p{x, kern, y, planes, in_h, in_w, out_h, out_w, kh, kw, up, down, pad_x0, pad_y0, flip, opt.tune_blur, in_layout,
                          act, out_scale, noise, noise_w, bias, channels > 0 ? channels : 1, slope, gain, nullptr, nullptr};
    if (opt.tune_print) fir_print(pl, p);
    if (fir_launch(pl, p, (hipStream_t)stream) != 0) return 1;
    W2E_LAUNCH_CHECK("upfirdn2d");
    return 0;
}

extern "C" int w2e_blur_adjoint_actbwd(const float* gy, const float* y_fwd, const float* noise, const float* kern, float* gt,
                                       float* sums, int64_t planes, int h, int w, float slope, float gain, void* stream) {
    W2E_REQUIRE(gy && y_fwd && kern && gt && sums, "blur_adjoint_actbwd: null tensor");
    W2E_REQUIRE(((uintptr_t)gy & 15) == 0 && ((uintptr_t)y_fwd & 15) == 0 && ((uintptr_t)gt & 15) == 0 && (!noise || ((uintptr_t)noise & 15) == 0),
                "blur_adjoint_actbwd: tensors must be 16-byte aligned");
    W2E_REQUIRE(gain > 0.f && slope > 0.f, "blur_adjoint_actbwd: gain and slope must be positive");
    const Options& opt = options();
    FirPlan pl;
    const int rc = fir_plan_actbwd(planes, h, w, opt, &pl);
    if (rc != 0 || pl.grid == 0) return rc;
    hipStream_t s = (hipStream_t)stream;
    if (zero_async(sums, sizeof(float) * 3 * (size_t)planes, s) != hipSuccess) {
        set_error("blur_adjoint_actbwd: zero fill failed");
        return 2;
    }
    const UpfirdnParams p{gy, kern, gt, planes, h, w, h + 1, w + 1, 4, 4, 1, 1, 2, 2, 0, opt.tune_blur & 7, 0,
                          0, nullptr, noise, nullptr, nullptr, 1, slope, gain, y_fwd, sums};
    if (opt.tune_print) fir_print(pl, p);
    if (fir_launch(pl, p, s) != 0) return 1;
    W2E_LAUNCH_CHECK("blur_adjoint_actbwd");
    return 0;
}

extern "C" int w2e_upfirdn2d_plan(int64_t planes, int in_h, int in_w, int out_h, int out_w, int kh, int kw, int up, int down, int pad_x0,
                                  int in_layout, int in_pitch, int act, int x_misalign, int y_misalign, int64_t* out) {
    W2E_REQUIRE(out != nullptr, "upfirdn2d_plan: null argument");
    FirPlan pl;
    const int rc = fir_plan(planes, in_h, in_w, out_h, out_w, kh, kw, up, down, pad_x0, in_layout, in_pitch, act, (unsigned)x_misalign & 15,
                            (unsigned)y_misalign & 15, options(), &pl);
    if (rc != 0) return rc;
    const int64_t fields[W2E_FIR_PLAN_FIELDS] = {pl.kernel, pl.act, pl.planar, pl.grid, pl.block, (int64_t)pl.lds, pl.args[0], pl.args[1], pl.args[2]};
    for (int i = 0; i < W2E_FIR_PLAN_FIELDS; ++i) out[i] = fields[i];
    return 0;
}

extern "C" int w2e_upfirdn2d_planar_ok(int kh, int kw, int up, int down, int out_w) { return planar_ok(kh, kw, up, down, out_w) ? 1 : 0; }

extern "C" int w2e_blur_adjoint_actbwd_plan(int64_t planes, int h, int w, int kh, int kw, int* fused) {
    W2E_REQUIRE(fused != nullptr, "blur_adjoint_actbwd_plan: null argument");
    const Options& opt = options();
    FirPlan pl;
    *fused = (opt.tune_fuse != 0 && kh == 4 && kw == 4 && fir_plan_actbwd(planes, h, w, opt, &pl) == 0) ? 1 : 0;
    return 0;
}
```

### where2edit_amd/functional.py

```python
import ctypes
import functools
import math
import os

import torch
from torch.autograd.function import once_differentiable

from . import _lib, profiling
from ._lib import CONSTS, call, ptr, stream_ptr

SQRT2 = math.sqrt(2.0)

_NOGRAD_PREFIX = 0
_POISON = os.environ.get("W2E_DEBUG_POISON", "0") == "1"


def set_debug_poison(on=True):
    global _POISON
    _POISON = bool(on)


def _grad_rows(shape, n_skip, device, like=None):
    buf = torch.empty(shape, device=device, dtype=torch.float32) if like is None else torch.empty_like(like)
    if _POISON and n_skip:
        buf[:n_skip].fill_(float("nan"))
    return buf


class nograd_prefix:
    def __init__(self, n):
        self.n = int(n)

    def __enter__(self):
        global _NOGRAD_PREFIX
        self.prev, _NOGRAD_PREFIX = _NOGRAD_PREFIX, self.n
        return self

    def __exit__(self, *exc):
        global _NOGRAD_PREFIX
        _NOGRAD_PREFIX = self.prev


class _TailRows(torch.autograd.Function):

    @staticmethod
    def forward(ctx, x, n):
        ctx.n, ctx.full = n, x.shape[0]
        return x[n:]

    @staticmethod
    @once_differentiable
    def backward(ctx, g):
        out = _grad_rows((ctx.full,) + tuple(g.shape[1:]), ctx.n, g.device)
        out[ctx.n:].copy_(g)
        return out, None


def tail_rows(x, n):
    return _TailRows.apply(x, n)


class GradPool:

    __slots__ = ("buf", "off", "hint")

    def __init__(self, hint):
        self.buf, self.off, self.hint = None, 0, int(hint)

    def zeros(self, shape, device):
        n = 1
        for v in shape:
            n *= int(v)
        n_al = (n + 63) & ~63
        if self.buf is None or self.off + n_al > self.buf.numel() or self.buf.device != torch.device(device):
            self.buf, self.off = torch.zeros(max(n_al, self.hint), device=device, dtype=torch.float32), 0
        out = self.buf[self.off:self.off + n].view(shape)
        self.off += n_al
        return out


_GRAD_POOL = None


class grad_pool:

    def __init__(self, hint):
        self.pool = GradPool(hint)

    def __enter__(self):
        global _GRAD_POOL
        self.prev, _GRAD_POOL = _GRAD_POOL, self.pool
        return self.pool

    def __exit__(self, *exc):
        global _GRAD_POOL
        _GRAD_POOL = self.prev
        return False


def _zeros_with_tail(full, n, tail_shape, device, pool=None):
    shape = (full,) + tuple(tail_shape)
    buf = pool.zeros(shape, device) if pool is not None else torch.zeros(shape, device=device, dtype=torch.float32)
    return buf, (buf[n:] if n else buf)


def _c(t):
    return t if t.is_contiguous() else t.contiguous()


def _upfirdn2d_raw(x, kernel, out_h, out_w, up, down, pad_x0, pad_y0, flip, act=None, planar_hw=None, out=None):
    n, c = x.shape[0], x.shape[1]
    h, w = planar_hw if planar_hw is not None else (x.shape[2], x.shape[3])
    if planar_hw is not None and tuple(x.shape[2:]) != (2, 2, (h + 1) // 2, planar_pitch((w - 1) // 2)):
        raise RuntimeError(f"upfirdn2d: a phase-planar input of a {h}x{w} image must be [N,C,2,2,{(h + 1) // 2},{planar_pitch((w - 1) // 2)}] "
                           f"(W2E_PLANAR_PITCH, include/w2e.h), got {tuple(x.shape)}")
    kh, kw = kernel.shape
    y = out if out is not None else torch.empty((n, c, out_h, out_w), device=x.device, dtype=torch.float32)
    if act is None:
        a = (0, None, None, None, None, 1, 0.2, SQRT2)
    else:
        out_scale, noise, noise_w, bias = act
        a = (1, ptr(out_scale), ptr(noise), ptr(noise_w), ptr(bias), c, 0.2, SQRT2)
    sp = profiling.span("upfirdn2d", 4.0 * n * c * (h * w + out_h * out_w))
    call("w2e_upfirdn2d", ptr(x), ptr(kernel), ptr(y), n * c, h, w, out_h, out_w, kh, kw, up, down, pad_x0, pad_y0,
         int(flip), int(planar_hw is not None), x.shape[-1] if planar_hw is not None else 0, *a, stream_ptr())
    if sp is not None:
        sp.end()
    return y


_FirPlanFields = ctypes.c_int64 * CONSTS["W2E_FIR_PLAN_FIELDS"]


def upfirdn_plan(planes, in_hw, out_hw, kernel_shape, up=1, down=1, pad_x0=0, planar=False, act=False, x_misalign=0, y_misalign=0):
    out = _FirPlanFields()
    call("w2e_upfirdn2d_plan", planes, *in_hw, *out_hw, *kernel_shape, up, down, pad_x0, int(planar),
         planar_pitch((in_hw[1] - 1) // 2) if planar else 0, int(act), x_misalign, y_misalign, out)
    return out[:]


def fir_planar_ok(kernel_shape, out_w):
    return bool(_lib.load().w2e_upfirdn2d_planar_ok(kernel_shape[0], kernel_shape[1], 1, 1, out_w))


class _UpFirDn2d(torch.autograd.Function):
    @staticmethod
    def forward(ctx, x, kernel, up, down, pad0, pad1):
        x = _c(x)
        kernel = _c(kernel.to(torch.float32))
        n, c, h, w = x.shape
        kh, kw = kernel.shape
        out_h = (h * up + pad0 + pad1 - kh) // down + 1
        out_w = (w * up + pad0 + pad1 - kw) // down + 1
        if out_h <= 0 or out_w <= 0:
            raise RuntimeError(f"upfirdn2d: empty output {out_h}x{out_w}")
        ctx.save_for_backward(kernel)
        ctx.geom = (h, w, up, down, pad0)
        return _upfirdn2d_raw(x, kernel, out_h, out_w, up, down, pad0, pad0, True)

    @staticmethod
    @once_differentiable
    def backward(ctx, gy):
        (kernel,) = ctx.saved_tensors
        h, w, up, down, pad0 = ctx.geom
        kh, kw = kernel.shape
        gx = _upfirdn2d_raw(_c(gy), kernel, h, w, down, up, kw - 1 - pad0, kh - 1 - pad0, False)
        return gx, None, None, None, None, None


def upfirdn2d(input, kernel, up=1, down=1, pad=(0, 0)):
    return _UpFirDn2d.apply(input, kernel, up, down, pad[0], pad[1])


class _BiasAct(torch.autograd.Function):

    @staticmethod
    def forward(ctx, x, bias, slope, gain, channel_last):
        x = _c(x)
        bias = _c(bias)
        if channel_last:
            outer, ch, inner = x.numel() // x.shape[-1], x.shape[-1], 1
        else:
            outer, ch, inner = x.shape[0], x.shape[1], x.numel() // (x.shape[0] * x.shape[1])
        if bias.numel() != ch:
            raise RuntimeError(f"fused_leaky_relu: bias has {bias.numel()} entries, expected {ch}")
        y = torch.empty_like(x)
        call("w2e_bias_act_fwd", ptr(x), ptr(bias), None, None, ptr(y), outer, ch, inner, slope, gain, stream_ptr())
        ctx.save_for_backward(y)
        ctx.cfg = (slope, gain, channel_last, ch)
        return y

    @staticmethod
    @once_differentiable
    def backward(ctx, gy):
        (y,) = ctx.saved_tensors
        slope, gain, channel_last, ch = ctx.cfg
        gy = _c(gy)
        gx = torch.empty_like(y)
        call("w2e_bias_act_bwd", ptr(gy), ptr(y), ptr(gx), y.numel(), slope, gain, stream_ptr())
        gb = None
        if ctx.needs_input_grad[1]:
            gb = gx.reshape(-1, ch).sum(0) if channel_last else gx.reshape(gx.shape[0], ch, -1).sum((0, 2))
        return gx, gb, None, None, None


def fused_leaky_relu(input, bias, negative_slope=0.2, scale=2 ** 0.5):
    if input.ndim < 2:
        raise RuntimeError("fused_leaky_relu expects at least 2 dims")
    channel_last = input.ndim == 3 or input.ndim == 2
    return _BiasAct.apply(input, bias, float(negative_slope), float(scale), channel_last)


def conv_pack(weight, scale, transpose, flip):
    cout, cin = weight.shape[0], weight.shape[1]
    kd, nd = (cout, cin) if transpose else (cin, cout)
    wp = torch.empty(((kd + 7) // 8, 9, 2, nd, 4), device=weight.device, dtype=torch.float32)
    call("w2e_conv_pack", ptr(_c(weight.detach())), ptr(wp), cout, cin, float(scale), int(transpose), int(flip),
         stream_ptr())
    return wp


MODE_SAME, MODE_UP, MODE_DOWN = (CONSTS[f"W2E_CONV_{m}"] for m in ("SAME", "UP", "DOWN"))

def _parse_winograd(v):
    table = {"": "auto", "auto": "auto", "0": False, "4": 4, "8": 8}
    if v not in table:
        raise ValueError(f"W2E_WINOGRAD={v!r}: expected 'auto', '0' (direct kernels), '4' (GEMM form) or '8' (fused form)")
    return table[v]


WINOGRAD = _parse_winograd(os.environ.get("W2E_WINOGRAD", ""))
WINO_LOG = None


FUSED = 8


def set_winograd(mode):
    global WINOGRAD
    if mode not in ("auto", False, 4, 8):
        raise ValueError("set_winograd: 'auto', False, 4 or 8")
    WINOGRAD = mode


FUSED_WGS = 0
GEMM_SPLITS = 0

GENERATOR, ENCODER = CONSTS["W2E_WINO_GENERATOR"], CONSTS["W2E_WINO_ENCODER"]
EPI_PLAIN, EPI_ACT, EPI_PRELU, EPI_DOT = (CONSTS[f"W2E_WINO_EPI_{e}"] for e in ("PLAIN", "ACT", "PRELU", "DOT"))

# ... 143 lines not shown
    n, c = a.shape[0], a.shape[1]
    out = torch.empty_like(a)
    zero = torch.zeros((n, c), device=a.device, dtype=torch.float32)
    call("w2e_se_apply_bwd", ptr(a), ptr(_c(s)), ptr(zero), ptr(out), n, c, a.shape[2] * a.shape[3], stream_ptr())
    return out


def demod_coefficients(s, wsq, eps=1e-8):
    b, cin = s.shape
    cout = wsq.shape[0]
    d = torch.empty((b, cout), device=s.device, dtype=torch.float32)
    call("w2e_demod_fwd", ptr(s), ptr(wsq), ptr(d), b, cin, cout, float(eps), stream_ptr())
    return d


def demod_coefficients_all(styles, wsqs, eps=1e-8):
    b = styles[0].shape[0]
    couts = [w.shape[0] for w in wsqs]
    buf = torch.empty(b * sum(couts), device=styles[0].device, dtype=torch.float32)
    descs = (_lib.DemodLayer * len(styles))()
    out, off = [], 0
    for j, (s, w) in enumerate(zip(styles, wsqs)):
        if s.shape != (b, w.shape[1]) or not s.is_contiguous() or not w.is_contiguous():
            raise RuntimeError(f"demod_coefficients_all: layer {j}: style {tuple(s.shape)} for wsq {tuple(w.shape)}")
        d = buf[off:off + b * couts[j]].view(b, couts[j])
        off += b * couts[j]
        descs[j].s, descs[j].wsq, descs[j].d, descs[j].cin, descs[j].cout = ptr(s).value, ptr(w).value, ptr(d).value, w.shape[1], couts[j]
        out.append(d)
    call("w2e_demod_all_fwd", descs, len(styles), b, float(eps), stream_ptr())
    return out


WGRAD_SAME, WGRAD_UP, WGRAD_CENTRE = 0, 1, 2


def modconv_wsq(weight, scale):
    cout, cin = weight.shape[1], weight.shape[2]
    wsq = torch.empty((cout, cin), device=weight.device, dtype=torch.float32)
    call("w2e_modconv_wsq", ptr(_c(weight.detach())), ptr(wsq), cout, cin, weight.shape[3] * weight.shape[4], float(scale), stream_ptr())
    return wsq


def modconv_wgrad(mode, g, x, d, s, weight, scale, sums=None, dz=None, noise_w=None, bias=None):
    b, cin, h, w = x.shape
    cout = weight.shape[1]
    taps = 1 if mode == WGRAD_CENTRE else 9
    splits = ctypes.c_int(0)
    call("w2e_modconv_wgrad_plan", mode, b, cin, cout, h, w, ctypes.byref(splits))
    slab = torch.empty(splits.value * taps * cout * cin, device=x.device, dtype=torch.float32)
    sp = profiling.span("modconv_wgrad", 2.0 * b * cin * cout * taps * h * w)
    st = stream_ptr()
    call("w2e_modconv_wgrad", mode, ptr(_c(g)), ptr(_c(x)), ptr(d), ptr(_c(s)), ptr(slab), b, cin, cout, h, w, splits.value, st)
    dw = torch.empty(weight.shape, device=x.device, dtype=torch.float32)
    if d is not None:
        call("w2e_modconv_wgrad_finish", ptr(slab), splits.value, ptr(_c(weight.detach())), ptr(sums), ptr(dz), ptr(noise_w), ptr(bias),
             ptr(d), ptr(_c(s)), ptr(dw), b, cin, cout, taps, float(scale), st)
    else:
        call("w2e_modconv_wgrad_finish", ptr(slab), splits.value, None, None, None, None, None, None, None, ptr(dw), b, cin, cout, taps,
             float(scale), st)
    if sp is not None:
        sp.end()
    return dw


def planar_pitch(w):
    return (w + 1 + 15) & ~15


def unplanar(t, in_w):
    b, n, _, _, hp, wpp = t.shape
    w = in_w
    return t.permute(0, 1, 4, 2, 5, 3).reshape(b, n, 2 * hp, 2 * wpp)[:, :, :2 * hp - 1, :2 * w + 1].contiguous()


class ActLink:

    __slots__ = ("noise", "gpre", "sums")

    def __init__(self, noise):
        self.noise, self.gpre, self.sums = noise, None, None

    def take(self, gout):
        gpre, sums = self.gpre, self.sums
        self.gpre = self.sums = None
        if gpre is None:
            return None
        if gpre is not gout:
            raise RuntimeError("where2edit_amd: the gradient of a StyledConv output that was routed through its ToRGB node "
                               "(ActLink) reached the StyledConv backward as a different tensor -- a tensor hook, retain_grad() "
                               "or a second consumer on that activation is not supported on the fused training path "
                               "(use return_features=True / the unfused modules to tap activations)")
        return sums


class RgbFoldLink:

    __slots__ = ("gy", "saved", "gpre", "sums", "gw")

    def __init__(self):
        self.gy = self.saved = self.gpre = self.sums = self.gw = None

    def usable(self, x, n_skip):
        if self.gy is None or self.saved is None:
            return False
        xs, _, _, _, ns = self.saved
        return ns == n_skip and xs.shape[0] == x.shape[0] + n_skip and xs.data_ptr() + 4 * n_skip * xs[0].numel() == x.data_ptr() \
            and tuple(xs.shape[1:]) == tuple(x.shape[1:]) and tuple(self.gy.shape) == (xs.shape[0], 3) + tuple(xs.shape[2:])

    def take(self, gy, gx_next):
        gpre, sums, gw, rec = self.gpre, self.sums, self.gw, self.gy
        self.gpre = self.sums = self.gw = self.gy = None
        if gpre is None:
            return None
        if gx_next is not gpre or gy is not rec:
            raise RuntimeError("where2edit_amd: the ToRGB backward was folded into the stride-2 input-gradient conv of the level above "
                               "(RgbFoldLink), but the gradients reached the ToRGB node as different tensors -- a tensor hook, "
                               "retain_grad() or a second consumer on the passed-through activation or on the RGB skip image is not "
                               "supported on the fused training path (use return_features=True / the unfused modules to tap "
                               "activations, or the option tune_rgbfold = 0)")
        return gpre, sums, gw


class _StyledConv(torch.autograd.Function):

    @staticmethod
    def forward(ctx, x, s, wsq, noise, noise_w, bias, packs, blur_kernel, upsample, fuse_act, link=None, d_pre=None, weight=None,
                wscale=1.0, fold=None):
        x, s = _c(x), _c(s)
        b, cin, h, w = x.shape
        wp_f, wp_b = packs
        d = None
        if wsq is not None:
            d = d_pre if d_pre is not None else demod_coefficients(s, wsq)
        act = (noise, noise_w, bias) if fuse_act else None
        if upsample and fuse_act and tuple(blur_kernel.shape) == (4, 4) and _upblur_planned(b, cin, wp_f.shape[3], h, w):
            out = _modconv_upblur_raw(x, wp_f, s, d, blur_kernel, h, w, act)
        elif upsample:
            t, _ = _modconv_raw(MODE_UP, x, wp_f, s, d, h, w)
            if fir_planar_ok(blur_kernel.shape, 2 * w):
                out = _upfirdn2d_raw(t, blur_kernel, 2 * h, 2 * w, 1, 1, 1, 1, True,
                                     act=((None,) + act) if fuse_act else None, planar_hw=(2 * h + 1, 2 * w + 1))
            else:
                out = _upfirdn2d_raw(unplanar(t, w), blur_kernel, 2 * h, 2 * w, 1, 1, 1, 1, True,
                                     act=((None,) + act) if fuse_act else None)
        else:
            out, _ = _modconv_raw(MODE_SAME, x, wp_f, s, d, h, w, act=act)
        ctx.save_for_backward(x, s, d, wsq, noise, noise_w, bias, out, wp_b, blur_kernel, weight)
        ctx.cfg = (upsample, fuse_act)
        ctx.wscale = float(wscale)
        ctx.link = link
        ctx.fold = fold if (upsample and weight is None and d is not None) else None
        ctx.n_skip = _NOGRAD_PREFIX if _NOGRAD_PREFIX < b else 0
        ctx.pool = _GRAD_POOL
        return out

    @staticmethod
    @once_differentiable
    def backward(ctx, gout):
        x, s, d, wsq, noise, noise_w, bias, out, wp_b, blur_kernel, weight = ctx.saved_tensors
        upsample, fuse_act = ctx.cfg
        n_skip, full = ctx.n_skip, x.shape[0]
        gout_full = gout
        gout = _c(gout)
        if n_skip:
            x, s, out, gout = x[n_skip:], s[n_skip:], out[n_skip:], gout[n_skip:]
            d = d[n_skip:] if d is not None else None
        b, cin, h, w = x.shape
        cout, oh, ow = out.shape[1], out.shape[2], out.shape[3]
        gx_full = _grad_rows((full, cin, h, w), n_skip, x.device) if n_skip else None
        gx_out = gx_full[n_skip:] if n_skip else None
        gs_full, gs_out = _zeros_with_tail(full, n_skip, (cin,), x.device, ctx.pool)
        g_bias = g_nw = g_noise = sums = dz = None
        blurred = False
        want_noise = fuse_act and noise is not None and ctx.needs_input_grad[3]
        pre_sums = ctx.link.take(gout_full) if (fuse_act and ctx.link is not None) else None
        if pre_sums is not None:
            gpre, sums = gout, pre_sums
        elif fuse_act:
            sums = torch.empty((b, cout, 3), device=x.device, dtype=torch.float32)
            if upsample and not want_noise and _blur_actbwd_planned(b * cout, oh, ow, blur_kernel.shape):
                gpre = torch.empty((b, cout, oh + 1, ow + 1), device=x.device, dtype=torch.float32)
                sp = profiling.span("upfirdn2d", 4.0 * b * cout * (2 * oh * ow + (oh + 1) * (ow + 1)))
                call("w2e_blur_adjoint_actbwd", ptr(gout), ptr(out), ptr(noise), ptr(blur_kernel), ptr(gpre), ptr(sums), b * cout, oh, ow,
                     0.2, SQRT2, stream_ptr())
                if sp is not None:
                    sp.end()
                blurred = True
            else:
                gpre = torch.empty_like(out)
                call("w2e_bias_act_bwd_reduce", ptr(gout), ptr(out), ptr(noise), ptr(gpre), ptr(sums), b, cout, oh * ow,
                     0.2, SQRT2, stream_ptr())
        else:
            gpre = gout
            if d is not None:
                dz = (gout * out).sum((2, 3))
        if fuse_act:
            if bias is not None and ctx.needs_input_grad[5]:
                g_bias = sums[..., 2].sum(0)
            if noise is not None and ctx.needs_input_grad[4]:
                g_nw = sums[..., 1].sum().reshape(1)
        if want_noise:
            g_noise = torch.empty_like(noise)
            call("w2e_noise_grad", ptr(gpre), ptr(noise_w), ptr(g_noise), b * cout, oh * ow, 0, stream_ptr())
        if upsample and not blurred:
            gpre = _upfirdn2d_raw(gpre, blur_kernel, 2 * h + 1, 2 * w + 1, 1, 1, 2, 2, False)
        g_w = None
        if weight is not None and ctx.needs_input_grad[12]:
            wmode = WGRAD_UP if upsample else (WGRAD_CENTRE if weight.shape[-1] == 1 else WGRAD_SAME)
            g_w = modconv_wgrad(wmode, gpre, x, d, s, weight, ctx.wscale, sums=sums if d is not None and fuse_act else None,
                                dz=dz, noise_w=noise_w if (fuse_act and noise is not None) else None, bias=bias if fuse_act else None)
        mode = MODE_DOWN if upsample else MODE_SAME
        if _lib.get_option("deterministic") and not (mode == MODE_SAME and _wino_form(gpre, gpre.shape[1], cin, h, w, x)):
            raw, _ = _modconv_raw(mode, gpre, wp_b, d, None, h, w)
            gs = _channel_dot(raw, x, out=gs_out)
            gx = _scale_planes(raw, s)
            if n_skip:
                gx_out.copy_(gx)
        elif ctx.fold is not None and ctx.fold.usable(x, n_skip) and _rgbfold_planned(b, gpre.shape[1], cin, h, w):
            fold = ctx.fold
            xr, wrgb, st, nz, _ = fold.saved
            rgb_full = fold.gy.shape[0]
            gw_full, gw = _zeros_with_tail(rgb_full, n_skip, (cin,) if st is not None else (3, cin), x.device, ctx.pool)
            sums3 = ctx.pool.zeros((b, cin, 3), x.device) if ctx.pool is not None else None
            gx, gs, sums3, _ = _modconv_down_rgbfold_raw(
                gpre, wp_b, d, s, h, w, x, fold.gy[n_skip:] if n_skip else fold.gy, wrgb if (st is not None or not n_skip) else wrgb[n_skip:],
                None if st is None else (st[n_skip:] if n_skip else st), nz, out=gx_out, dot_out=gs_out, sums3=sums3, gw=gw)
            fold.gpre, fold.sums, fold.gw = (gx_full if n_skip else gx), sums3, gw_full
        else:
            gx, gs = _modconv_raw(mode, gpre, wp_b, d, s, h, w, dot_with=x, out=gx_out, dot_out=gs_out)
        if d is not None:
            call("w2e_demod_bwd", ptr(sums), ptr(dz), ptr(noise_w) if (fuse_act and noise is not None) else None,
                 ptr(bias) if fuse_act else None, ptr(d), ptr(s), ptr(wsq), ptr(gs), None, b, cin, cout, stream_ptr())
        if n_skip:
            gx = gx_full
        return gx, gs_full, None, g_noise, g_nw, g_bias, None, None, None, None, None, None, g_w, None, None


def styled_conv(x, s, wsq, noise, noise_w, bias, packs, blur_kernel, upsample, link=None, demod=None, weight=None, wscale=1.0, fold=None):
    return _StyledConv.apply(x, s, wsq, noise, noise_w, bias, packs, blur_kernel, upsample, True, link, demod, weight, wscale, fold)


def modconv(x, s, wsq, packs, blur_kernel, upsample, weight=None, wscale=1.0):
    return _StyledConv.apply(x, s, wsq, None, None, None, packs, blur_kernel, upsample, False, None, None, weight, wscale)


def modconv_down_plain(x, s, d, wp_f, h, w):
    y, _ = _modconv_raw(MODE_DOWN, _c(x), wp_f, _c(s) if s is not None else None, _c(d) if d is not None else None, h, w)
    return y


class _StyleAffineAll(torch.autograd.Function):

    @staticmethod
    def forward(ctx, latent, pack):
        import ctypes
        latent = _c(latent)
        b, n_latent, dim = latent.shape
        w, bias, meta, widths = pack
        rows = w.shape[0]
        out = torch.empty(b * rows, device=latent.device, dtype=torch.float32)
        call("w2e_style_affine_fwd", ptr(latent), ptr(w), ptr(bias), ctypes.c_void_p(meta.data_ptr()), ptr(out), b, n_latent,
             dim, rows, stream_ptr())
        ctx.pack = pack
        ctx.geom = (b, n_latent, dim)
        ctx.n_skip = _NOGRAD_PREFIX if _NOGRAD_PREFIX < b else 0
        ctx.pool = _GRAD_POOL
        outs, off = [], 0
        for cw in widths:
            outs.append(out[off * b:(off + cw) * b].view(b, cw))
            off += cw
        return tuple(outs)

    @staticmethod
    @once_differentiable
    def backward(ctx, *gs):
        import ctypes
        b, n_latent, dim = ctx.geom
        n_skip = ctx.n_skip
        b -= n_skip
        w, bias, meta, widths = ctx.pack
        parts = [(g[n_skip:].reshape(-1) if g is not None else torch.zeros(b * cw, device=w.device, dtype=torch.float32))
                 for g, cw in zip(gs, widths)]
        flat = torch.cat(parts)
        glat_full, glat = _zeros_with_tail(b + n_skip, n_skip, (n_latent, dim), w.device, ctx.pool)
        call("w2e_style_affine_bwd", ptr(flat), ptr(w), ctypes.c_void_p(meta.data_ptr()), ptr(glat), b, n_latent, dim,
             w.shape[0], stream_ptr())
        return glat_full, None


def style_affine_all(latent, pack):
    return _StyleAffineAll.apply(latent, pack)


class _ToRGB(torch.autograd.Function):

    @staticmethod
    def forward(ctx, x, wmod, style, bias, skip, upk, passthrough=False, producer_act=None, fold_out=None, fold_skip=None):
        x_in = x
        x, wmod = _c(x), _c(wmod)
        b, cin, h, w = x.shape
        y = torch.empty((b, 3, h, w), device=x.device, dtype=torch.float32)
        skip_c = _c(skip) if skip is not None else None
        bias_c = _c(bias.reshape(-1)) if bias is not None else None
        if style is None:
            call("w2e_torgb_fwd", ptr(x), ptr(wmod), ptr(bias_c), ptr(skip_c), ptr(upk) if skip is not None else None,
                 ptr(y), b, cin, h, w, stream_ptr())
        else:
            style = _c(style.reshape(b, cin))
            if wmod.numel() != 3 * cin:
                raise RuntimeError(f"to_rgb: the shared weight must be [3,{cin}], got {tuple(wmod.shape)}")
            call("w2e_torgb_styled_fwd", ptr(x), ptr(wmod), ptr(style), ptr(bias_c), ptr(skip_c),
                 ptr(upk) if skip is not None else None, ptr(y), b, cin, h, w, stream_ptr())
        ctx.save_for_backward(x, wmod, style, upk if skip is not None else None, producer_act.noise if producer_act is not None else None)
        ctx.link = producer_act
        ctx.n_skip = _NOGRAD_PREFIX if _NOGRAD_PREFIX < b else 0
        ctx.fold_out = fold_out if (passthrough and producer_act is not None) else None
        ctx.fold_skip = fold_skip if skip is not None else None
        if ctx.fold_out is not None:
            ctx.fold_out.saved = (x.detach(), wmod.detach(), style.detach() if style is not None else None, producer_act.noise, ctx.n_skip)
        ctx.has = (bias is not None, skip is not None, tuple(bias.shape) if bias is not None else None)
        ctx.pool = _GRAD_POOL
        if passthrough:
            return y, x_in.view_as(x_in)
        return y

    @staticmethod
    @once_differentiable
    def backward(ctx, gy, gx_next=None):
        x, wmod, style, upk, act_noise = ctx.saved_tensors
        has_bias, has_skip, bias_shape = ctx.has
        n_skip = ctx.n_skip
        b, cin, h, w = x.shape
        if gy is None:
            return gx_next, None, None, None, None, None, None, None, None, None
        folded = ctx.fold_out.take(gy, gx_next) if ctx.fold_out is not None else None
        gy = _c(gy)
        if folded is not None:
            gx, sums3, gw_full = folded
            gys = gy[n_skip:] if n_skip else gy
            ctx.link.gpre, ctx.link.sums = gx, sums3
            return (gx,) + _rgb_small_grads(ctx, gys, gw_full, wmod, style, upk, n_skip, b, h, w, x.device)
        gx = _grad_rows(None, n_skip, x.device, like=x)
        acc = _c(gx_next) if gx_next is not None else None
        if n_skip:
            xs, gys, gxs = x[n_skip:], gy[n_skip:], gx[n_skip:]
            accs = acc[n_skip:] if acc is not None else None
        else:
            xs, gys, gxs, accs = x, gy, gx, acc
        ws = wmod if style is not None else (wmod[n_skip:] if n_skip else wmod)
        sts = None if style is None else (style[n_skip:] if n_skip else style)
        gw_full, gw = _zeros_with_tail(b, n_skip, (cin,) if style is not None else (3, cin), x.device, ctx.pool)
        if ctx.link is not None:
            sums3 = torch.empty((b - n_skip, cin, 3), device=x.device, dtype=torch.float32)
            call("w2e_torgb_bwd_actbwd", ptr(xs), ptr(ws), ptr(sts), ptr(gys), ptr(accs), ptr(act_noise), ptr(gxs), ptr(gw), ptr(sums3),
                 b - n_skip, cin, h, w, 0.2, SQRT2, stream_ptr())
            ctx.link.gpre, ctx.link.sums = gx, sums3
        elif style is None:
            call("w2e_torgb_bwd_acc", ptr(xs), ptr(ws), ptr(gys), ptr(accs), ptr(gxs), ptr(gw), b - n_skip, cin, h, w, stream_ptr())
        else:
            call("w2e_torgb_styled_bwd", ptr(xs), ptr(ws), ptr(sts), ptr(gys), ptr(accs), ptr(gxs), ptr(gw), b - n_skip, cin, h, w,
                 stream_ptr())
        return (gx,) + _rgb_small_grads(ctx, gys, gw_full, wmod, style, upk, n_skip, b, h, w, x.device)


def _rgb_small_grads(ctx, gys, gw_full, wmod, style, upk, n_skip, b, h, w, device):
    has_bias, has_skip, bias_shape = ctx.has
    g_wmod, g_style = (gw_full.view_as(wmod), None) if style is None else (None, gw_full)
    gb = gys.sum((0, 2, 3)).reshape(bias_shape) if (has_bias and ctx.needs_input_grad[3]) else None
    gskip = None
    if has_skip:
        gskip = _grad_rows((b, 3, h // 2, w // 2), n_skip, device)
        _upfirdn2d_raw(gys, upk, h // 2, w // 2, 1, 2, 1, 1, False, out=gskip[n_skip:] if n_skip else gskip)
        if ctx.fold_skip is not None:
            ctx.fold_skip.gy = gskip
    return g_wmod, g_style, gb, gskip, None, None, None, None, None


def to_rgb(x, wmod, bias, skip, upk, passthrough=False, style=None, producer_act=None, fold_out=None, fold_skip=None):
    return _ToRGB.apply(x, wmod, style, bias, skip, upk, passthrough, producer_act, fold_out, fold_skip)


class _ClipPreproc(torch.autograd.Function):
    @staticmethod
    def forward(ctx, img):
        img = _c(img)
        n, c, h, w = img.shape
        if h != w:
            raise RuntimeError("clip_preprocess expects square images")
        out = torch.empty((n, c, 224, 224), device=img.device, dtype=torch.float32)
        call("w2e_clip_preproc_fwd", ptr(img), ptr(out), n * c, h, stream_ptr())
        ctx.shape = img.shape
        return out

    @staticmethod
    @once_differentiable
    def backward(ctx, gout):
        n, c, h, w = ctx.shape
        gimg = torch.empty(ctx.shape, device=gout.device, dtype=torch.float32)
        call("w2e_clip_preproc_bwd", ptr(_c(gout)), ptr(gimg), n * c, h, stream_ptr())
        return gimg


def clip_preprocess(img):
    return _ClipPreproc.apply(img)


class _IdPreproc(torch.autograd.Function):
    @staticmethod
    def forward(ctx, img):
        img = _c(img)
        n, c, h, w = img.shape
        out = torch.empty((n, c, 112, 112), device=img.device, dtype=torch.float32)
        call("w2e_id_preproc_fwd", ptr(img), ptr(out), n * c, h, stream_ptr())
        ctx.shape = img.shape
        return out

    @staticmethod
    @once_differentiable
    def backward(ctx, gout):
        n, c, h, w = ctx.shape
        gimg = torch.empty(ctx.shape, device=gout.device, dtype=torch.float32)
        call("w2e_id_preproc_bwd", ptr(_c(gout)), ptr(gimg), n * c, h, stream_ptr())
        return gimg


def id_preprocess(img):
    return _IdPreproc.apply(img)


class _MaskBlend(torch.autograd.Function):
    @staticmethod
    def forward(ctx, a, b, mask):
        a, b, mask = _c(a), _c(b), _c(mask)
        n, c, h, w = a.shape
        if b.shape != a.shape or mask.shape[0] != n or mask.shape[1] != 1 or mask.shape[2] != mask.shape[3]:
            raise RuntimeError(f"mask_blend: shapes {tuple(a.shape)} {tuple(b.shape)} {tuple(mask.shape)}")
        out = torch.empty_like(a)
        call("w2e_mask_blend_fwd", ptr(a), ptr(b), ptr(mask), ptr(out), n, c, h, w, mask.shape[2], stream_ptr())
        ctx.save_for_backward(a, b, mask)
        return out

    @staticmethod
    @once_differentiable
    def backward(ctx, gout):
        a, b, mask = ctx.saved_tensors
        n, c, h, w = a.shape
        gout = _c(gout)
        ga = torch.empty_like(a)
        gb = torch.empty_like(b) if ctx.needs_input_grad[1] else None
        gm = torch.empty_like(mask) if ctx.needs_input_grad[2] else None
        call("w2e_mask_blend_bwd", ptr(gout), ptr(a), ptr(b), ptr(mask), ptr(ga), ptr(gb), ptr(gm), n, c, h, w,
             mask.shape[2], stream_ptr())
        return ga, gb, gm


def mask_blend(new, old, mask):
    return _MaskBlend.apply(new, old, mask)
```

### where2edit_amd/stylegan2.py

```python
import math
import os
import random

import torch
from torch import nn
from torch.nn import functional as F

from . import functional as K
from .derived import derived, invalidate as invalidate_caches
from .op import FusedLeakyReLU, fused_leaky_relu, upfirdn2d


def _trainable_weight(mod):
    if torch.is_grad_enabled() and mod.weight.requires_grad:
        if getattr(mod, "_train_weight", False):
            return True
        raise RuntimeError(
            "where2edit_amd: a ModulatedConv2d weight requires grad (decoder fine-tuning).  The HIP kernels treat the decoder as frozen -- "
            "as the path they serve does (coach.py:174-180 optimises net.mapper only) -- unless asked otherwise; there is no "
            "stock-op fallback.  Call stylegan2.freeze_conv_weights(decoder) (or decoder.requires_grad_(False)); gradients to latents, "
            "styles, noise strengths and biases are unaffected; or `train_conv_weights` to fine-tune them.")
    return False


# ... 292 lines not shown
        self.bias = nn.Parameter(torch.zeros(1, 3, 1, 1))

    def forward(self, input, style, skip=None, input_is_stylespace=False, passthrough=False, producer_act=None, fold_out=None,
                fold_skip=None):
        conv = self.conv
        batch = input.shape[0]
        style = conv._style(style, batch, input_is_stylespace)
        w = conv.weight
        st = None
        if torch.is_grad_enabled() and w.requires_grad:
            wmod = (conv.scale * w.view(1, 3, conv.in_channel)) * style.reshape(batch, 1, conv.in_channel)
        else:
            wmod = derived(self, "_wsc", (w,), lambda: (conv.scale * w.detach().view(3, conv.in_channel)).contiguous())
            st = style.reshape(batch, conv.in_channel)
        fuse_skip = skip is not None and self.upsample.kernel.shape == (4, 4) and self.upsample.factor == 2
        passed = None
        if passthrough:
            out, passed = K.to_rgb(input, wmod, self.bias, skip if fuse_skip else None, self.upsample.kernel if fuse_skip else None,
                                   True, style=st, producer_act=None if _NO_RGBACT else producer_act,
                                   fold_out=None if _NO_RGBACT else fold_out, fold_skip=fold_skip if fuse_skip else None)
        else:
            out = K.to_rgb(input, wmod, self.bias, skip if fuse_skip else None, self.upsample.kernel if fuse_skip else None,
                           style=st, producer_act=None if _NO_RGBACT else producer_act, fold_skip=fold_skip if fuse_skip else None)
        if skip is not None and not fuse_skip:
            out = out + self.upsample(skip)
        if passthrough:
            return out, style, passed
        return out, style


class Generator(nn.Module):

    def __init__(self, size, style_dim, n_mlp, channel_multiplier=2, blur_kernel=[1, 3, 3, 1], lr_mlp=0.01):
        super().__init__()
        self.size = size
        self.style_dim = style_dim
        layers = [PixelNorm()]
        for _ in range(n_mlp):
            layers.append(EqualLinear(style_dim, style_dim, lr_mul=lr_mlp, activation="fused_lrelu"))
        self.style = nn.Sequential(*layers)
        self.channels = {4: 512, 8: 512, 16: 512, 32: 512, 64: 256 * channel_multiplier,
                         128: 128 * channel_multiplier, 256: 64 * channel_multiplier,
                         512: 32 * channel_multiplier, 1024: 16 * channel_multiplier}
        self.input = ConstantInput(self.channels[4])
        self.conv1 = StyledConv(self.channels[4], self.channels[4], 3, style_dim, blur_kernel=blur_kernel)
        self.to_rgb1 = ToRGB(self.channels[4], style_dim, upsample=False)
        self.log_size = int(math.log(size, 2))
        self.num_layers = (self.log_size - 2) * 2 + 1
        self.convs = nn.ModuleList()
        self.upsamples = nn.ModuleList()
        self.to_rgbs = nn.ModuleList()
        self.noises = nn.Module()
        in_channel = self.channels[4]
        for layer_idx in range(self.num_layers):
            res = (layer_idx + 5) // 2
            self.noises.register_buffer(f"noise_{layer_idx}", torch.randn(1, 1, 2 ** res, 2 ** res))
        for i in range(3, self.log_size + 1):
            out_channel = self.channels[2 ** i]
            self.convs.append(StyledConv(in_channel, out_channel, 3, style_dim, upsample=True, blur_kernel=blur_kernel))
            self.convs.append(StyledConv(out_channel, out_channel, 3, style_dim, blur_kernel=blur_kernel))
            self.to_rgbs.append(ToRGB(out_channel, style_dim))
            in_channel = out_channel
        self.n_latent = self.log_size * 2 - 2

    def make_noise(self):
        device = self.input.input.device
        noises = [torch.randn(1, 1, 2 ** 2, 2 ** 2, device=device)]
        for i in range(3, self.log_size + 1):
            for _ in range(2):
                noises.append(torch.randn(1, 1, 2 ** i, 2 ** i, device=device))
        return noises

    def mean_latent(self, n_latent):
        latent_in = torch.randn(n_latent, self.style_dim, device=self.input.input.device)
        return self.style(latent_in).mean(0, keepdim=True)

    def get_latent(self, input):
        return self.style(input)

    def _prepare(self, styles, inject_index, truncation, truncation_latent, input_is_latent, input_is_stylespace, noise,
                 randomize_noise):
        if not input_is_latent and not input_is_stylespace:
            styles = [self.style(s) for s in styles]
        if noise is None:
            if randomize_noise:
                noise = [None] * self.num_layers
            else:
                noise = [getattr(self.noises, f"noise_{i}") for i in range(self.num_layers)]
        if truncation < 1 and not input_is_stylespace:
            styles = [truncation_latent + truncation * (s - truncation_latent) for s in styles]
        if input_is_stylespace:
            latent = styles[0]
        elif len(styles) < 2:
            latent = styles[0].unsqueeze(1).repeat(1, self.n_latent, 1) if styles[0].ndim < 3 else styles[0]
        else:
            if inject_index is None:
                inject_index = random.randint(1, self.n_latent - 1)
            latent = torch.cat([styles[0].unsqueeze(1).repeat(1, inject_index, 1),
                                styles[1].unsqueeze(1).repeat(1, self.n_latent - inject_index, 1)], 1)
        return latent, noise

    def _layers(self):
        plan = [(self.conv1, False, 0, 0), (self.to_rgb1, True, 1, None)]
        i = 1
        for j in range(len(self.to_rgbs)):
            plan.append((self.convs[2 * j], False, i, 1 + 2 * j))
            plan.append((self.convs[2 * j + 1], False, i + 1, 2 + 2 * j))
            plan.append((self.to_rgbs[j], True, i + 2, None))
            i += 2
        return plan

    def _style_pack(self, plan):
        mods = [m.conv.modulation for m, _, _, _ in plan]

        def build():
            with torch.no_grad():
                w = torch.cat([m.weight.detach().float() * m.scale for m in mods]).contiguous()
                b = torch.cat([m.bias.detach().float() * m.lr_mul for m in mods]).contiguous()
                meta, off = [], 0
                for (_, _, widx, _), m in zip(plan, mods):
                    cw = m.weight.shape[0]
                    meta.append(torch.stack([torch.full((cw,), widx), torch.full((cw,), off), torch.full((cw,), cw),
                                             torch.arange(cw)], 1))
                    off += cw
                meta = torch.cat(meta).to(device=w.device, dtype=torch.int32).contiguous()
            return w, b, meta, [m.weight.shape[0] for m in mods]

        return derived(self, "_style_pack_val", [t for m in mods for t in (m.weight, m.bias)], build)

    def _batched_styles(self, latent, plan):
        if not (torch.is_tensor(latent) and latent.ndim == 3 and latent.is_cuda):
            return None
        mods = [m.conv.modulation for m, _, _, _ in plan]
        if any(m.bias is None or m.weight.shape[0] % 32 for m in mods):
            return None
        if torch.is_grad_enabled() and any(m.weight.requires_grad or m.bias.requires_grad for m in mods):
            return None
        return K.style_affine_all(latent, self._style_pack(plan))

    def style_codes(self, styles, inject_index=None, truncation=1, truncation_latent=None, input_is_latent=False):
        latent, _ = self._prepare(styles, inject_index, truncation, truncation_latent, input_is_latent, False, None, False)
        plan = self._layers()
        batch = latent.shape[0]
        batched = self._batched_styles(latent, plan)
        if batched is not None:
            return latent, [s.view(batch, 1, s.shape[1], 1, 1) for s in batched]
        return latent, [mod.conv._style(latent[:, widx], batch, False) for mod, _, widx, _ in plan]

    def _synthesis(self, latent, noise, input_is_stylespace, on_layer=None, hook_layers=None):
        if not torch.is_grad_enabled():
            return self._synthesis_pass(latent, noise, input_is_stylespace, on_layer, hook_layers)
        batch = (latent[0] if input_is_stylespace else latent).shape[0]
        widths = sum(m.conv.in_channel for m, _, _, _ in self._layers())
        with K.grad_pool(batch * (3 * widths + 64 * (len(self._layers()) + 12) + self.n_latent * self.style_dim)):
            return self._synthesis_pass(latent, noise, input_is_stylespace, on_layer, hook_layers)

    def _synthesis_pass(self, latent, noise, input_is_stylespace, on_layer, hook_layers):
        hook_all = on_layer
        stylespace_in = input_is_stylespace
        batch_ref = latent[0] if input_is_stylespace else latent
        out = self.input(batch_ref)
        skip = None
        style_vector = []
        plan = self._layers()
        batched = None if input_is_stylespace else self._batched_styles(latent, plan)
        if batched is not None:
            batch = latent.shape[0]
            latent = [s.view(batch, 1, s.shape[1], 1, 1) for s in batched]
            input_is_stylespace = True
        demods = {}
        if batched is not None and batched[0].is_cuda:
            idx = [n for n, (m, is_rgb, _, _) in enumerate(plan)
                   if not is_rgb and m.conv.demodulate and m.conv.kernel_size == 3 and not m.conv._live()]
            if idx:
                demods = dict(zip(idx, K.demod_coefficients_all([batched[n] for n in idx], [plan[n][0].conv._derived()[2] for n in idx])))
        producer = None
        fold = None
        fold_ok = (hook_all is None and not stylespace_in and torch.is_grad_enabled() and not _NO_RGBPASS and not _NO_RGBACT
                   and out.is_cuda and K._lib.get_option("tune_rgbfold") != 0)
        for n, (mod, is_rgb, widx, nidx) in enumerate(plan):
            sty = latent[n] if input_is_stylespace else latent[:, widx]
            on_layer = hook_all if (hook_layers is None or n in hook_layers) else None
            if is_rgb:
                if on_layer is None and n + 1 < len(plan) and torch.is_grad_enabled() and out.requires_grad and not _NO_RGBPASS:
                    link = K.RgbFoldLink() if (fold_ok and producer is not None) else None
                    skip, s, out = mod(out, sty, skip, input_is_stylespace=input_is_stylespace, passthrough=True, producer_act=producer,
                                       fold_out=link, fold_skip=fold)
                    fold = link
                elif on_layer is None and n + 1 == len(plan) and torch.is_grad_enabled() and out.requires_grad and not _NO_RGBPASS:
                    skip, s = mod(out, sty, skip, input_is_stylespace=input_is_stylespace, producer_act=producer, fold_skip=fold)
                    fold = None
                else:
                    skip, s = mod(out, sty, skip, input_is_stylespace=input_is_stylespace)
                    fold = None
                if on_layer is not None:
                    skip = on_layer(n, True, skip)
                producer = None
            else:
                out, s = mod(out, sty, noise=noise[nidx], input_is_stylespace=input_is_stylespace, demod=demods.get(n),
                             fold=fold if mod.conv.upsample else None)
                producer = getattr(mod, "_act_noise", None)
                if on_layer is not None:
                    out = on_layer(n, False, out)
                    producer = None
                    fold = None
            style_vector.append(s)
        return skip, style_vector

    def forward(self, styles, return_latents=False, inject_index=None, truncation=1, truncation_latent=None,
                input_is_latent=False, input_is_stylespace=False, noise=None, randomize_noise=True):
        latent, noise = self._prepare(styles, inject_index, truncation, truncation_latent, input_is_latent,
                                      input_is_stylespace, noise, randomize_noise)
        image, style_vector = self._synthesis(latent, noise, input_is_stylespace)
        if return_latents:
            return image, latent, style_vector
        return image, None


_DISC_BLUR = (1, 3, 3, 1)


class ConvLayer(nn.Sequential):

    def __init__(self, in_channel, out_channel, kernel_size, downsample=False, blur_kernel=[1, 3, 3, 1], bias=True, activate=True):
        layers = []
        if downsample:
            factor = 2
            p = (len(blur_kernel) - factor) + (kernel_size - 1)
            layers.append(Blur(blur_kernel, pad=((p + 1) // 2, p // 2)))
            stride = 2
            padding = 0
        else:
            stride = 1
            padding = kernel_size // 2
        layers.append(EqualConv2d(in_channel, out_channel, kernel_size, padding=padding, stride=stride, bias=bias and not activate))
        if activate:
            layers.append(FusedLeakyReLU(out_channel) if bias else ScaledLeakyReLU(0.2))
        super().__init__(*layers)
        self.padding = padding
        self._form = None
        if tuple(blur_kernel) == _DISC_BLUR or not downsample:
            if not downsample and activate and bias and kernel_size == 1 and in_channel == 3:
                self._form = "fromrgb"
            elif not downsample and activate and bias and kernel_size == 3:
                self._form = "same"
            elif downsample and activate and bias and kernel_size == 3:
                self._form = "down"
            elif downsample and not activate and not bias and kernel_size == 1:
                self._form = "skip"

    def forward(self, input):
        from . import disc_hip
        if self._form == "fromrgb":
            return disc_hip.fromrgb(self, input)
        if self._form == "same":
            return disc_hip.convact(self, input)
        if self._form in ("down", "skip"):
            raise NotImplementedError("a down-sampling ConvLayer runs inside ResBlock.forward (its blur is shared with the block's "
                                      "other branch); call the ResBlock")
        raise NotImplementedError("ConvLayer kernels exist for the Discriminator's configurations only: fromRGB (3 -> C, 1x1), the "
                                  "stride-1 3x3 with bias + activation, and the ResBlock's down-sampling 3x3 / 1x1 with the "
                                  "[1, 3, 3, 1] blur")


class ResBlock(nn.Module):

    def __init__(self, in_channel, out_channel, blur_kernel=[1, 3, 3, 1]):
        super().__init__()
        self.conv1 = ConvLayer(in_channel, in_channel, 3)
        self.conv2 = ConvLayer(in_channel, out_channel, 3, downsample=True, blur_kernel=blur_kernel)
        self.skip = ConvLayer(in_channel, out_channel, 1, downsample=True, activate=False, bias=False, blur_kernel=blur_kernel)
        self._blur = tuple(blur_kernel)

    def forward(self, input):
        from . import disc_hip
        if self._blur != _DISC_BLUR:
            raise NotImplementedError("ResBlock kernels exist for the [1, 3, 3, 1] blur (the Discriminator's default) only")
        if input.shape[2] % 2 or input.shape[3] % 2:
            raise NotImplementedError("ResBlock kernels need an even input size")
        return disc_hip.resblock(self, input)


class Discriminator(nn.Module):

    def __init__(self, size, channel_multiplier=2, blur_kernel=[1, 3, 3, 1]):
        super().__init__()
        channels = {4: 512, 8: 512, 16: 512, 32: 512, 64: 256 * channel_multiplier, 128: 128 * channel_multiplier,
                    256: 64 * channel_multiplier, 512: 32 * channel_multiplier, 1024: 16 * channel_multiplier}
        convs = [ConvLayer(3, channels[size], 1)]
        log_size = int(math.log(size, 2))
        in_channel = channels[size]
        for i in range(log_size, 2, -1):
            out_channel = channels[2 ** (i - 1)]
            convs.append(ResBlock(in_channel, out_channel, blur_kernel))
            in_channel = out_channel
        self.convs = nn.Sequential(*convs)
        self.stddev_group = 4
        self.stddev_feat = 1
        self.final_conv = ConvLayer(in_channel + 1, channels[4], 3)
        self.final_linear = nn.Sequential(
            EqualLinear(channels[4] * 4 * 4, channels[4], activation="fused_lrelu"),
            EqualLinear(channels[4], 1),
        )

    def forward(self, input):
        from . import disc_hip
        if self.stddev_group != 4 or self.stddev_feat != 1:
# ... 13 lines not shown
```

Baseline: 269.3 images/s.

## Defer demodulation backward into one batched kernel and prezero style-grad arena

Adds a backward-tail mode in which each modulated conv's demodulation backward is not launched per layer. It is recorded and later run for all layers at once in a single batched demod_bwd_all kernel inside the style-affine backward. Reduction buffers come prezeroed from the grad-pool arena, so the per-kernel memsets are skipped. When all style gradients live in the arena, the affine backward reads it directly and the torch.cat is dropped. The goal is fewer small launches and memsets in the decoder backward, at the cost of more bookkeeping and a larger pool.

Result: no change. 271.0 images/s (median of 6 runs) (+0.7%).

```diff
diff --git a/include/w2e.h b/include/w2e.h
--- a/include/w2e.h
+++ b/include/w2e.h
@@ -100,6 +100,18 @@
 int w2e_demod_all_fwd(const w2e_demod_layer* layers, int n_layers, int batch, float eps, void* stream);
 int w2e_demod_bwd(const float* sums, const float* dz, const float* noise_w, const float* bias, const float* d,
                   const float* s, const float* wsq, float* gs, float* gd, int batch, int cin, int cout, void* stream);
+#define W2E_DEMOD_BWD_ROW 9
+int w2e_demod_bwd_all(const int64_t* rows, int n_layers, int batch, void* stream);
+
+int w2e_torgb_styled_bwd_prezeroed(const float* x, const float* wsc, const float* style, const float* gy, const float* gx_acc,
+                                   float* gx, float* gstyle, int batch, int cin, int h, int w, void* stream);
+int w2e_torgb_bwd_actbwd_prezeroed(const float* x, const float* wmod, const float* style, const float* gy, const float* gx_acc,
+                                   const float* noise, float* gpre, float* gw, float* sums3, int batch, int cin, int h, int w,
+                                   float slope, float gain, void* stream);
+int w2e_blur_adjoint_actbwd_prezeroed(const float* gy, const float* y_fwd, const float* noise, const float* kern, float* gt,
+                                      float* sums, int64_t planes, int h, int w, float slope, float gain, void* stream);
+int w2e_bias_act_bwd_reduce_prezeroed(const float* gy, const float* y, const float* noise, float* gx, float* sums, int64_t outer,
+                                      int64_t channels, int64_t inner, float slope, float gain, void* stream);
 
 int w2e_modconv_wgrad_plan(int mode, int batch, int cin, int cout, int h, int w, int* splits);
 int w2e_modconv_wgrad(int mode, const float* g, const float* x, const float* d, const float* s, float* slab, int batch, int cin,
diff --git a/where2edit_amd/coach.py b/where2edit_amd/coach.py
--- a/where2edit_amd/coach.py
+++ b/where2edit_amd/coach.py
@@ -80,7 +80,7 @@
             from . import functional as K
             n = w.shape[0]
             w_hat = w + 0.1 * self.net.mapper(w)
-            with K.nograd_prefix(n):
+            with K.nograd_prefix(n), K.backward_tail():
                 both, lat, _ = dec([torch.cat([w.detach(), w_hat])], input_is_latent=True, return_latents=True, randomize_noise=False,
                                    truncation=1)
             self._x_ready = None
@@ -107,8 +107,10 @@
             x_hat, _, w_hat = dec([w_hat], input_is_latent=True, return_latents=True, randomize_noise=False,
                                   truncation=1, input_is_stylespace=True)
         else:
+            from . import functional as K
             w_hat = w + 0.1 * self.net.mapper(w)
-            x_hat, w_hat, _ = dec([w_hat], input_is_latent=True, return_latents=True, randomize_noise=False, truncation=1)
+            with K.backward_tail():
+                x_hat, w_hat, _ = dec([w_hat], input_is_latent=True, return_latents=True, randomize_noise=False, truncation=1)
         return x, x_hat, w_hat
 
     def calc_loss(self, w, x, w_hat, x_hat):
diff --git a/where2edit_amd/csrc/common.h b/where2edit_amd/csrc/common.h
--- a/where2edit_amd/csrc/common.h
+++ b/where2edit_amd/csrc/common.h
@@ -18,6 +18,7 @@
     int tune_upall, tune_dma, tune_fuse;
     int tune_upblur;
     int tune_rgbfold;
+    int tune_tail;
     int tune_mw;
     int tune_xcd;
     int tune_print, tune_blur, tune_gemm_s;
diff --git a/where2edit_amd/csrc/demod_bwd.h b/where2edit_amd/csrc/demod_bwd.h
--- /dev/null
+++ b/where2edit_amd/csrc/demod_bwd.h
@@ -0,0 +1,49 @@
+#pragma once
+#include "common.h"
+
+namespace w2e {
+
+constexpr int DEMOD_OCH = 32;
+
+__device__ __forceinline__ void demod_bwd_block(const float* __restrict__ sums, const float* __restrict__ dz_in,
+                                                const float* __restrict__ noise_w, const float* __restrict__ bias,
+                                                const float* __restrict__ d, const float* __restrict__ s,
+                                                const float* __restrict__ wsq, float* __restrict__ gs, float* __restrict__ gd_out,
+                                                int Cin, int Cout, int b, int xblk, int o_first, bool serial, float* coef) {
+    const float nw = noise_w ? noise_w[0] : 0.f;
+    const int i_ser = xblk * 256 + threadIdx.x;
+    float total = 0.f;
+    for (int o_lo = o_first; o_lo < Cout; o_lo += DEMOD_OCH) {
+    const int o_n = (Cout - o_lo < DEMOD_OCH) ? Cout - o_lo : DEMOD_OCH;
+    __syncthreads();
+    for (int oo = threadIdx.x; oo < o_n; oo += 256) {
+        const int o = o_lo + oo;
+        float dz;
+        if (sums) {
+            const float* q = sums + ((int64_t)b * Cout + o) * 3;
+            dz = q[0] - nw * q[1] - (bias ? bias[o] : 0.f) * q[2];
+        } else {
+            dz = dz_in[(int64_t)b * Cout + o];
+        }
+        const float dv = d[(int64_t)b * Cout + o];
+        coef[oo] = dz * dv * dv;
+        if (gd_out && xblk == 0) gd_out[(int64_t)b * Cout + o] = dz / dv;
+    }
+    __syncthreads();
+    const int i = xblk * 256 + threadIdx.x;
+    float acc = 0.f;
+    if (i < Cin) {
+        const float* wq = wsq + (int64_t)o_lo * Cin + i;
+#pragma unroll 16
+        for (int oo = 0; oo < o_n; ++oo) acc += coef[oo] * wq[(int64_t)oo * Cin];
+    }
+    if (!serial) {
+        if (i < Cin) atomicAdd(&gs[(int64_t)b * Cin + i], -s[(int64_t)b * Cin + i] * acc);
+        return;
+    }
+    total += acc;
+    }
+    if (i_ser < Cin) gs[(int64_t)b * Cin + i_ser] += -s[(int64_t)b * Cin + i_ser] * total;
+}
+
+}
diff --git a/where2edit_amd/csrc/elementwise.hip b/where2edit_amd/csrc/elementwise.hip
--- a/where2edit_amd/csrc/elementwise.hip
+++ b/where2edit_amd/csrc/elementwise.hip
@@ -1,4 +1,6 @@
+#include "demod_bwd.h"
 #include "device.h"
+#include "genbwd.h"
 
 namespace w2e {
 
@@ -294,49 +296,14 @@
     if (lane == 0) y.d[row] = rsqrtf(acc + L.eps);
 }
 
-constexpr int DEMOD_OCH = 32;
 __global__ __launch_bounds__(256) void demod_bwd_kernel(const float* __restrict__ sums, const float* __restrict__ dz_in,
                                                         const float* __restrict__ noise_w, const float* __restrict__ bias,
                                                         const float* __restrict__ d, const float* __restrict__ s,
                                                         const float* __restrict__ wsq, float* __restrict__ gs,
                                                         float* __restrict__ gd_out, int Cin, int Cout) {
     __shared__ float coef[DEMOD_OCH];
-    const int b = blockIdx.y;
-    const float nw = noise_w ? noise_w[0] : 0.f;
-    const bool serial = gridDim.z == 1 && Cout > DEMOD_OCH;
-    const int i_ser = blockIdx.x * 256 + threadIdx.x;
-    float total = 0.f;
-    for (int o_lo = blockIdx.z * DEMOD_OCH; o_lo < Cout; o_lo += DEMOD_OCH) {
-    const int o_n = (Cout - o_lo < DEMOD_OCH) ? Cout - o_lo : DEMOD_OCH;
-    __syncthreads();
-    for (int oo = threadIdx.x; oo < o_n; oo += 256) {
-        const int o = o_lo + oo;
-        float dz;
-        if (sums) {
-            const float* q = sums + ((int64_t)b * Cout + o) * 3;
-            dz = q[0] - nw * q[1] - (bias ? bias[o] : 0.f) * q[2];
-        } else {
-            dz = dz_in[(int64_t)b * Cout + o];
-        }
-        const float dv = d[(int64_t)b * Cout + o];
-        coef[oo] = dz * dv * dv;
-        if (gd_out && blockIdx.x == 0) gd_out[(int64_t)b * Cout + o] = dz / dv;
-    }
-    __syncthreads();
-    const int i = blockIdx.x * 256 + threadIdx.x;
-    float acc = 0.f;
-    if (i < Cin) {
-        const float* wq = wsq + (int64_t)o_lo * Cin + i;
-#pragma unroll 16
-        for (int oo = 0; oo < o_n; ++oo) acc += coef[oo] * wq[(int64_t)oo * Cin];
-    }
-    if (!serial) {
-        if (i < Cin) atomicAdd(&gs[(int64_t)b * Cin + i], -s[(int64_t)b * Cin + i] * acc);
-        return;
-    }
-    total += acc;
-    }
-    if (i_ser < Cin) gs[(int64_t)b * Cin + i_ser] += -s[(int64_t)b * Cin + i_ser] * total;
+    demod_bwd_block(sums, dz_in, noise_w, bias, d, s, wsq, gs, gd_out, Cin, Cout, blockIdx.y, blockIdx.x, blockIdx.z * DEMOD_OCH,
+                    gridDim.z == 1 && Cout > DEMOD_OCH, coef);
 }
 
 
@@ -433,6 +400,13 @@
 
 int w2e_bias_act_bwd_reduce(const float* gy, const float* y, const float* noise, float* gx, float* sums,
                             int64_t outer, int64_t channels, int64_t inner, float slope, float gain, void* stream) {
+    return bias_act_bwd_reduce_impl(gy, y, noise, gx, sums, outer, channels, inner, slope, gain, stream, false);
+}
+
+}
+
+int w2e::bias_act_bwd_reduce_impl(const float* gy, const float* y, const float* noise, float* gx, float* sums, int64_t outer,
+                                  int64_t channels, int64_t inner, float slope, float gain, void* stream, bool prezeroed) {
     W2E_REQUIRE(gy && y && gx && sums, "bias_act_bwd_reduce: null tensor");
     W2E_REQUIRE(slope != 0.f && gain != 0.f, "bias_act_bwd_reduce: slope and gain must be non-zero");
     const int64_t rows = outer * channels;
@@ -446,7 +420,7 @@
         if (splits < 1) splits = 1;
     }
     W2E_REQUIRE(rows * splits < (int64_t)1 << 31, "bias_act_bwd_reduce: grid too large");
-    if (splits > 1 && zero_async(sums, sizeof(float) * 3 * rows, s) != hipSuccess) {
+    if (splits > 1 && !prezeroed && zero_async(sums, sizeof(float) * 3 * rows, s) != hipSuccess) {
         set_error("bias_act_bwd_reduce: memset failed");
         return 2;
     }
@@ -454,6 +428,8 @@
     W2E_LAUNCH_CHECK("bias_act_bwd_reduce");
     return 0;
 }
+
+extern "C" {
 
 int w2e_mask_blend_fwd(const float* a, const float* b, const float* mask, float* out, int batch, int channels, int h,
                        int w, int ms, void* stream) {
diff --git a/where2edit_amd/csrc/genbwd.h b/where2edit_amd/csrc/genbwd.h
--- /dev/null
+++ b/where2edit_amd/csrc/genbwd.h
@@ -0,0 +1,16 @@
+#pragma once
+#include "common.h"
+
+namespace w2e {
+
+int torgb_bwd_impl(const float* x, const float* wmod, const float* style, const float* gy, const float* gx_acc, float* gx,
+                   float* gwmod, int batch, int cin, int h, int w, void* stream, bool actb = false, const float* noise = nullptr,
+                   float* sums3 = nullptr, float slope = 0.f, float gain = 1.f, bool prezeroed = false);
+
+int blur_adjoint_actbwd_impl(const float* gy, const float* y_fwd, const float* noise, const float* kern, float* gt, float* sums,
+                             int64_t planes, int h, int w, float slope, float gain, void* stream, bool prezeroed);
+
+int bias_act_bwd_reduce_impl(const float* gy, const float* y, const float* noise, float* gx, float* sums, int64_t outer,
+                             int64_t channels, int64_t inner, float slope, float gain, void* stream, bool prezeroed);
+
+}
diff --git a/where2edit_amd/csrc/genbwd.hip b/where2edit_amd/csrc/genbwd.hip
--- /dev/null
+++ b/where2edit_amd/csrc/genbwd.hip
@@ -0,0 +1,85 @@
+#include "demod_bwd.h"
+#include "genbwd.h"
+
+namespace w2e {
+
+struct DemodBwdRow {
+    const float *sums, *noise_w, *bias, *d, *s, *wsq;
+    float* gs;
+    int cin, cout;
+};
+
+struct DemodBwdAllLaunch {
+    DemodBwdRow row[W2E_DEMOD_MAX_LAYERS];
+    int slices;
+};
+
+__global__ __launch_bounds__(256) void demod_bwd_all_kernel(const DemodBwdAllLaunch L) {
+    __shared__ float coef[DEMOD_OCH];
+    const int layer = blockIdx.z / L.slices;
+    const int o_first = (blockIdx.z - layer * L.slices) * DEMOD_OCH;
+    const DemodBwdRow& y = L.row[layer];
+    if ((int)blockIdx.x * 256 >= y.cin || o_first >= y.cout) return;
+    demod_bwd_block(y.sums, nullptr, y.noise_w, y.bias, y.d, y.s, y.wsq, y.gs, nullptr, y.cin, y.cout, blockIdx.y, blockIdx.x, o_first,
+                    L.slices == 1 && y.cout > DEMOD_OCH, coef);
+}
+
+}
+
+using namespace w2e;
+
+extern "C" {
+
+int w2e_demod_bwd_all(const int64_t* rows, int n_layers, int batch, void* stream) {
+    W2E_REQUIRE(rows, "demod_bwd_all: null table");
+    W2E_REQUIRE(n_layers >= 1 && n_layers <= W2E_DEMOD_MAX_LAYERS, "demod_bwd_all: 1 <= n_layers <= %d", W2E_DEMOD_MAX_LAYERS);
+    W2E_REQUIRE(batch >= 0 && batch < 65536, "demod_bwd_all: bad dims");
+    DemodBwdAllLaunch L{};
+    int max_cin = 0, max_cout = 0;
+    for (int j = 0; j < n_layers; ++j) {
+        const int64_t* r = rows + (int64_t)j * W2E_DEMOD_BWD_ROW;
+        DemodBwdRow& y = L.row[j];
+        y.sums = reinterpret_cast<const float*>(r[0]), y.noise_w = reinterpret_cast<const float*>(r[1]);
+        y.bias = reinterpret_cast<const float*>(r[2]), y.d = reinterpret_cast<const float*>(r[3]);
+        y.s = reinterpret_cast<const float*>(r[4]), y.wsq = reinterpret_cast<const float*>(r[5]);
+        y.gs = reinterpret_cast<float*>(r[6]);
+        W2E_REQUIRE(y.sums && y.d && y.s && y.wsq && y.gs && r[7] > 0 && r[8] > 0 && r[7] < ((int64_t)1 << 24) && r[8] < ((int64_t)1 << 20),
+                    "demod_bwd_all: layer %d: null tensor or bad dims", j);
+        y.cin = (int)r[7], y.cout = (int)r[8];
+        if (y.cin > max_cin) max_cin = y.cin;
+        if (y.cout > max_cout) max_cout = y.cout;
+    }
+    if (batch == 0) return 0;
+    L.slices = options().deterministic ? 1 : (int)ceil_div(max_cout, DEMOD_OCH);
+    W2E_REQUIRE((int64_t)n_layers * L.slices < 65536, "demod_bwd_all: too many output-channel slices");
+    dim3 grid((unsigned)ceil_div(max_cin, 256), (unsigned)batch, (unsigned)(n_layers * L.slices));
+    demod_bwd_all_kernel<<<grid, 256, 0, (hipStream_t)stream>>>(L);
+    W2E_LAUNCH_CHECK("demod_bwd_all");
+    return 0;
+}
+
+int w2e_torgb_styled_bwd_prezeroed(const float* x, const float* wsc, const float* style, const float* gy, const float* gx_acc,
+                                   float* gx, float* gstyle, int batch, int cin, int h, int w, void* stream) {
+    W2E_REQUIRE(style, "torgb_styled_bwd_prezeroed: null style");
+    return torgb_bwd_impl(x, wsc, style, gy, gx_acc, gx, gstyle, batch, cin, h, w, stream, false, nullptr, nullptr, 0.f, 1.f, true);
+}
+
+int w2e_torgb_bwd_actbwd_prezeroed(const float* x, const float* wmod, const float* style, const float* gy, const float* gx_acc,
+                                   const float* noise, float* gpre, float* gw, float* sums3, int batch, int cin, int h, int w,
+                                   float slope, float gain, void* stream) {
+    W2E_REQUIRE(sums3, "torgb_bwd_actbwd_prezeroed: null sums");
+    W2E_REQUIRE(gain > 0.f && slope > 0.f, "torgb_bwd_actbwd_prezeroed: gain and slope must be positive");
+    return torgb_bwd_impl(x, wmod, style, gy, gx_acc, gpre, gw, batch, cin, h, w, stream, true, noise, sums3, slope, gain, true);
+}
+
+int w2e_blur_adjoint_actbwd_prezeroed(const float* gy, const float* y_fwd, const float* noise, const float* kern, float* gt,
+                                      float* sums, int64_t planes, int h, int w, float slope, float gain, void* stream) {
+    return blur_adjoint_actbwd_impl(gy, y_fwd, noise, kern, gt, sums, planes, h, w, slope, gain, stream, true);
+}
+
+int w2e_bias_act_bwd_reduce_prezeroed(const float* gy, const float* y, const float* noise, float* gx, float* sums, int64_t outer,
+                                      int64_t channels, int64_t inner, float slope, float gain, void* stream) {
+    return bias_act_bwd_reduce_impl(gy, y, noise, gx, sums, outer, channels, inner, slope, gain, stream, true);
+}
+
+}
diff --git a/where2edit_amd/csrc/runtime.hip b/where2edit_amd/csrc/runtime.hip
--- a/where2edit_amd/csrc/runtime.hip
+++ b/where2edit_amd/csrc/runtime.hip
@@ -44,6 +44,7 @@
     else if (!strcmp(name, "tune_mw")) o.tune_mw = (value && *value) ? iv : -1;
     else if (!strcmp(name, "tune_upblur")) o.tune_upblur = (value && *value) ? iv : -1;
     else if (!strcmp(name, "tune_rgbfold")) o.tune_rgbfold = (value && *value) ? iv : -1;
+    else if (!strcmp(name, "tune_tail")) o.tune_tail = (value && *value) ? iv : -1;
 #ifdef W2E_TUNING
     else if (!strcmp(name, "tune_skip")) o.tune_skip = iv;
     else if (!strcmp(name, "tune_clock")) o.tune_clock = iv;
@@ -54,14 +55,14 @@
 
 static Options from_env() {
     Options o{};
-    o.tune_cfg = -1, o.tune_cfg_splits = 1, o.tune_cfg_mode = -1, o.tune_upall = -1, o.tune_dma = -1, o.tune_fuse = -1, o.tune_xcd = -1, o.tune_mw = -1, o.tune_upblur = -1, o.tune_rgbfold = -1;
+    o.tune_cfg = -1, o.tune_cfg_splits = 1, o.tune_cfg_mode = -1, o.tune_upall = -1, o.tune_dma = -1, o.tune_fuse = -1, o.tune_xcd = -1, o.tune_mw = -1, o.tune_upblur = -1, o.tune_rgbfold = -1, o.tune_tail = -1;
     static const char* const kEnv[][2] = {
         {"W2E_CONV_PRECISION", "conv_precision"}, {"W2E_DETERMINISTIC", "deterministic"}, {"W2E_TUNE_CFG", "tune_cfg"},
         {"W2E_TUNE_UPALL", "tune_upall"},         {"W2E_TUNE_DMA", "tune_dma"},           {"W2E_TUNE_PRINT", "tune_print"},
         {"W2E_TUNE_BLUR", "tune_blur"},           {"W2E_TUNE_GEMM_S", "tune_gemm_s"},     {"W2E_TUNE_FUSE", "tune_fuse"},
         {"W2E_TUNE_SKIP", "tune_skip"},           {"W2E_TUNE_CLOCK", "tune_clock"},       {"W2E_TUNE_XCD", "tune_xcd"},
         {"W2E_TUNE_MW", "tune_mw"},               {"W2E_TUNE_UPBLUR", "tune_upblur"},
-        {"W2E_TUNE_RGBFOLD", "tune_rgbfold"}};
+        {"W2E_TUNE_RGBFOLD", "tune_rgbfold"},     {"W2E_TUNE_TAIL", "tune_tail"}};
     for (const auto& e : kEnv)
         if (const char* v = getenv(e[0])) apply(o, e[1], v);
     return o;
@@ -131,6 +132,7 @@
     else if (!strcmp(name, "tune_blur")) *value = o.tune_blur;
     else if (!strcmp(name, "tune_upblur")) *value = o.tune_upblur;
     else if (!strcmp(name, "tune_rgbfold")) *value = o.tune_rgbfold;
+    else if (!strcmp(name, "tune_tail")) *value = o.tune_tail;
     else if (!strcmp(name, "tuning_build")) {
 #ifdef W2E_TUNING
         *value = 1;
diff --git a/where2edit_amd/csrc/torgb.hip b/where2edit_amd/csrc/torgb.hip
--- a/where2edit_amd/csrc/torgb.hip
+++ b/where2edit_amd/csrc/torgb.hip
@@ -1,4 +1,5 @@
 #include "device.h"
+#include "genbwd.h"
 
 namespace w2e {
 
@@ -230,9 +231,6 @@
     return torgb_fwd_impl(x, wsc, style, bias, skip, upk, y, batch, cin, h, w, stream);
 }
 
-static int torgb_bwd_impl(const float* x, const float* wmod, const float* style, const float* gy, const float* gx_acc,
-                          float* gx, float* gwmod, int batch, int cin, int h, int w, void* stream, bool actb = false,
-                          const float* noise = nullptr, float* sums3 = nullptr, float slope = 0.f, float gain = 1.f);
 
 extern "C" int w2e_torgb_bwd(const float* x, const float* wmod, const float* gy, float* gx, float* gwmod, int batch,
                              int cin, int h, int w, void* stream) {
@@ -259,9 +257,11 @@
     return torgb_bwd_impl(x, wmod, style, gy, gx_acc, gpre, gw, batch, cin, h, w, stream, true, noise, sums3, slope, gain);
 }
 
-static int torgb_bwd_impl(const float* x, const float* wmod, const float* style, const float* gy, const float* gx_acc,
-                          float* gx, float* gwmod, int batch, int cin, int h, int w, void* stream, bool actb, const float* noise,
-                          float* sums3, float slope, float gain) {
+namespace w2e {
+
+int torgb_bwd_impl(const float* x, const float* wmod, const float* style, const float* gy, const float* gx_acc,
+                   float* gx, float* gwmod, int batch, int cin, int h, int w, void* stream, bool actb, const float* noise,
+                   float* sums3, float slope, float gain, bool prezeroed) {
     W2E_REQUIRE(x && wmod && gy && gx && gwmod, "torgb_bwd: null tensor");
     W2E_REQUIRE(batch >= 0 && cin > 0 && h > 0 && w > 0, "torgb_bwd: bad dims");
     W2E_REQUIRE(batch < 65536, "torgb_bwd: batch too large");
@@ -278,7 +278,7 @@
     int64_t per_split = ceil_div(hw, splits);
     per_split = (per_split + 255) & ~int64_t(255);
     splits = (int)ceil_div(hw, per_split);
-    if (splits > 1 && (zero_async(gwmod, sizeof(float) * (style ? 1 : 3) * (size_t)batch * cin, s) != hipSuccess ||
+    if (splits > 1 && !prezeroed && (zero_async(gwmod, sizeof(float) * (style ? 1 : 3) * (size_t)batch * cin, s) != hipSuccess ||
                        (actb && zero_async(sums3, sizeof(float) * 3 * (size_t)batch * cin, s) != hipSuccess))) {
         set_error("torgb_bwd: memset failed");
         return 2;
@@ -307,3 +307,5 @@
     W2E_LAUNCH_CHECK("torgb_bwd");
     return 0;
 }
+
+}
diff --git a/where2edit_amd/csrc/upfirdn2d.hip b/where2edit_amd/csrc/upfirdn2d.hip
--- a/where2edit_amd/csrc/upfirdn2d.hip
+++ b/where2edit_amd/csrc/upfirdn2d.hip
@@ -1,6 +1,7 @@
 #include <stdlib.h>
 
 #include "common.h"
+#include "genbwd.h"
 
 namespace w2e {
 
@@ -857,8 +858,8 @@
     return 0;
 }
 
-extern "C" int w2e_blur_adjoint_actbwd(const float* gy, const float* y_fwd, const float* noise, const float* kern, float* gt,
-                                       float* sums, int64_t planes, int h, int w, float slope, float gain, void* stream) {
+int w2e::blur_adjoint_actbwd_impl(const float* gy, const float* y_fwd, const float* noise, const float* kern, float* gt, float* sums,
+                                  int64_t planes, int h, int w, float slope, float gain, void* stream, bool prezeroed) {
     W2E_REQUIRE(gy && y_fwd && kern && gt && sums, "blur_adjoint_actbwd: null tensor");
     W2E_REQUIRE(((uintptr_t)gy & 15) == 0 && ((uintptr_t)y_fwd & 15) == 0 && ((uintptr_t)gt & 15) == 0 && (!noise || ((uintptr_t)noise & 15) == 0),
                 "blur_adjoint_actbwd: tensors must be 16-byte aligned");
@@ -868,7 +869,7 @@
     const int rc = fir_plan_actbwd(planes, h, w, opt, &pl);
     if (rc != 0 || pl.grid == 0) return rc;
     hipStream_t s = (hipStream_t)stream;
-    if (zero_async(sums, sizeof(float) * 3 * (size_t)planes, s) != hipSuccess) {
+    if (!prezeroed && zero_async(sums, sizeof(float) * 3 * (size_t)planes, s) != hipSuccess) {
         set_error("blur_adjoint_actbwd: zero fill failed");
         return 2;
     }
@@ -878,6 +879,11 @@
     if (fir_launch(pl, p, s) != 0) return 1;
     W2E_LAUNCH_CHECK("blur_adjoint_actbwd");
     return 0;
+}
+
+extern "C" int w2e_blur_adjoint_actbwd(const float* gy, const float* y_fwd, const float* noise, const float* kern, float* gt,
+                                       float* sums, int64_t planes, int h, int w, float slope, float gain, void* stream) {
+    return blur_adjoint_actbwd_impl(gy, y_fwd, noise, kern, gt, sums, planes, h, w, slope, gain, stream, false);
 }
 
 extern "C" int w2e_upfirdn2d_plan(int64_t planes, int in_h, int in_w, int out_h, int out_w, int kh, int kw, int up, int down, int pad_x0,
diff --git a/where2edit_amd/functional.py b/where2edit_amd/functional.py
--- a/where2edit_amd/functional.py
+++ b/where2edit_amd/functional.py
@@ -2,6 +2,7 @@
 import functools
 import math
 import os
+import weakref
 
 import torch
 from torch.autograd.function import once_differentiable
@@ -41,16 +42,46 @@
         _NOGRAD_PREFIX = self.prev
 
 
+class _TailLink:
+
+    __slots__ = ("ptr", "shape", "n", "full", "buf", "__weakref__")
+
+    def __init__(self, ptr, shape, n, full):
+        self.ptr, self.shape, self.n, self.full, self.buf = ptr, shape, n, full, None
+
+
+_LAST_TAIL = None
+
+
+def _tail_link_of(img):
+    link = _LAST_TAIL() if _LAST_TAIL is not None else None
+    if link is not None and link.ptr == img.data_ptr() and link.shape == tuple(img.shape):
+        return link
+    return None
+
+
 class _TailRows(torch.autograd.Function):
 
     @staticmethod
     def forward(ctx, x, n):
+        global _LAST_TAIL
         ctx.n, ctx.full = n, x.shape[0]
-        return x[n:]
+        out = x[n:]
+        ctx.link = None
+        if x.is_cuda and out.is_contiguous() and _lib.get_option("tune_tail") != 0:
+            ctx.link = _TailLink(out.data_ptr(), tuple(out.shape), n, x.shape[0])
+            _LAST_TAIL = weakref.ref(ctx.link)
+        return out
 
     @staticmethod
     @once_differentiable
     def backward(ctx, g):
+        link = ctx.link
+        if link is not None and link.buf is not None:
+            buf, link.buf = link.buf, None
+            if g.data_ptr() == buf.data_ptr() + 4 * ctx.n * buf[0].numel() and tuple(g.shape) == link.shape and g.is_contiguous() \
+                    and g.dtype == torch.float32:
+                return buf, None
         out = _grad_rows((ctx.full,) + tuple(g.shape[1:]), ctx.n, g.device)
         out[ctx.n:].copy_(g)
         return out, None
@@ -62,10 +93,11 @@
 
 class GradPool:
 
-    __slots__ = ("buf", "off", "hint")
+    __slots__ = ("buf", "off", "hint", "tail")
 
     def __init__(self, hint):
         self.buf, self.off, self.hint = None, 0, int(hint)
+        self.tail = None
 
     def zeros(self, shape, device):
         n = 1
@@ -96,6 +128,88 @@
         global _GRAD_POOL
         _GRAD_POOL = self.prev
         return False
+
+
+_BACKWARD_TAIL = False
+
+
+class backward_tail:
+    def __enter__(self):
+        global _BACKWARD_TAIL
+        self.prev = _BACKWARD_TAIL
+        _BACKWARD_TAIL = _lib.get_option("tune_tail") != 0
+        return self
+
+    def __exit__(self, *exc):
+        global _BACKWARD_TAIL
+        _BACKWARD_TAIL = self.prev
+        return False
+
+
+def backward_tail_active():
+    return _BACKWARD_TAIL
+
+
+class StyleTail:
+
+    __slots__ = ("batch", "widths", "offsets", "total", "by_ptr", "arena", "handed", "rows")
+
+    def __init__(self, out, batch, widths):
+        self.batch, self.widths, self.offsets, self.by_ptr = batch, list(widths), [], {}
+        off = 0
+        for l, cw in enumerate(self.widths):
+            self.offsets.append(off)
+            self.by_ptr[out.data_ptr() + 4 * off * batch] = l
+            off += cw
+        self.total = off
+        self.arena, self.handed, self.rows = None, set(), []
+
+    def layer_of(self, s):
+        if s is None or not s.is_cuda:
+            return None
+        l = self.by_ptr.get(s.data_ptr())
+        if l is None or tuple(s.shape) != (self.batch, self.widths[l]) or not s.is_contiguous():
+            return None
+        return l
+
+    def region(self, l):
+        o = self.offsets[l] * self.batch
+        return self.arena[o:o + self.widths[l] * self.batch].view(self.batch, self.widths[l])
+
+    def view(self, l, pool, device):
+        if l in self.handed:
+            return None
+        if self.arena is None:
+            self.arena = pool.zeros((self.total * self.batch,), device)
+        self.handed.add(l)
+        return self.region(l)
+
+    def is_region(self, l, g):
+        return self.arena is not None and g.data_ptr() == self.arena.data_ptr() + 4 * self.offsets[l] * self.batch \
+            and tuple(g.shape) == (self.batch, self.widths[l]) and g.is_contiguous() and g.dtype == torch.float32
+
+    def reset(self):
+        self.arena, self.handed, self.rows = None, set(), []
+
+
+def _tail_zeros(ctx, layer, full, n, shape, device):
+    tail = ctx.pool.tail if (layer is not None and ctx.pool is not None) else None
+    if tail is not None and full == tail.batch and tuple(shape) == (tail.widths[layer],):
+        buf = tail.view(layer, ctx.pool, device)
+        if buf is not None:
+            return buf, (buf[n:] if n else buf), True
+    return _zeros_with_tail(full, n, shape, device, ctx.pool) + (False,)
+
+
+def _demod_bwd_all(rows, batch):
+    width = CONSTS["W2E_DEMOD_BWD_ROW"]
+    step = CONSTS["W2E_DEMOD_MAX_LAYERS"]
+    for lo in range(0, len(rows), step):
+        chunk = rows[lo:lo + step]
+        table = (ctypes.c_int64 * (width * len(chunk)))()
+        for j, (sums, noise_w, bias, d, s, wsq, gs, cin, cout) in enumerate(chunk):
+            table[width * j:width * (j + 1)] = [ptr(t).value if t is not None else 0 for t in (sums, noise_w, bias, d, s, wsq, gs)] + [cin, cout]
+        call("w2e_demod_bwd_all", table, len(chunk), batch, stream_ptr())
 
 
 def _zeros_with_tail(full, n, tail_shape, device, pool=None):
@@ -545,6 +659,8 @@
         ctx.fold = fold if (upsample and weight is None and d is not None) else None
         ctx.n_skip = _NOGRAD_PREFIX if _NOGRAD_PREFIX < b else 0
         ctx.pool = _GRAD_POOL
+        ctx.tail_layer = ctx.pool.tail.layer_of(s) if (ctx.pool is not None and ctx.pool.tail is not None) else None
+        ctx.prezero = _BACKWARD_TAIL and ctx.pool is not None
         return out
 
     @staticmethod
@@ -562,7 +678,8 @@
         cout, oh, ow = out.shape[1], out.shape[2], out.shape[3]
         gx_full = _grad_rows((full, cin, h, w), n_skip, x.device) if n_skip else None
         gx_out = gx_full[n_skip:] if n_skip else None
-        gs_full, gs_out = _zeros_with_tail(full, n_skip, (cin,), x.device, ctx.pool)
+        gs_full, gs_out, in_arena = _tail_zeros(ctx, ctx.tail_layer, full, n_skip, (cin,), x.device)
+        pre = "_prezeroed" if ctx.prezero else ""
         g_bias = g_nw = g_noise = sums = dz = None
         blurred = False
         want_noise = fuse_act and noise is not None and ctx.needs_input_grad[3]
@@ -570,18 +687,18 @@
         if pre_sums is not None:
             gpre, sums = gout, pre_sums
         elif fuse_act:
-            sums = torch.empty((b, cout, 3), device=x.device, dtype=torch.float32)
+            sums = ctx.pool.zeros((b, cout, 3), x.device) if ctx.prezero else torch.empty((b, cout, 3), device=x.device, dtype=torch.float32)
             if upsample and not want_noise and _blur_actbwd_planned(b * cout, oh, ow, blur_kernel.shape):
                 gpre = torch.empty((b, cout, oh + 1, ow + 1), device=x.device, dtype=torch.float32)
                 sp = profiling.span("upfirdn2d", 4.0 * b * cout * (2 * oh * ow + (oh + 1) * (ow + 1)))
-                call("w2e_blur_adjoint_actbwd", ptr(gout), ptr(out), ptr(noise), ptr(blur_kernel), ptr(gpre), ptr(sums), b * cout, oh, ow,
+                call("w2e_blur_adjoint_actbwd" + pre, ptr(gout), ptr(out), ptr(noise), ptr(blur_kernel), ptr(gpre), ptr(sums), b * cout, oh, ow,
                      0.2, SQRT2, stream_ptr())
                 if sp is not None:
                     sp.end()
                 blurred = True
             else:
                 gpre = torch.empty_like(out)
-                call("w2e_bias_act_bwd_reduce", ptr(gout), ptr(out), ptr(noise), ptr(gpre), ptr(sums), b, cout, oh * ow,
+                call("w2e_bias_act_bwd_reduce" + pre, ptr(gout), ptr(out), ptr(noise), ptr(gpre), ptr(sums), b, cout, oh * ow,
                      0.2, SQRT2, stream_ptr())
         else:
             gpre = gout
@@ -613,7 +730,8 @@
             fold = ctx.fold
             xr, wrgb, st, nz, _ = fold.saved
             rgb_full = fold.gy.shape[0]
-            gw_full, gw = _zeros_with_tail(rgb_full, n_skip, (cin,) if st is not None else (3, cin), x.device, ctx.pool)
+            rgb_layer = ctx.pool.tail.layer_of(st) if (st is not None and ctx.pool is not None and ctx.pool.tail is not None) else None
+            gw_full, gw, _ = _tail_zeros(ctx, rgb_layer, rgb_full, n_skip, (cin,) if st is not None else (3, cin), x.device)
             sums3 = ctx.pool.zeros((b, cin, 3), x.device) if ctx.pool is not None else None
             gx, gs, sums3, _ = _modconv_down_rgbfold_raw(
                 gpre, wp_b, d, s, h, w, x, fold.gy[n_skip:] if n_skip else fold.gy, wrgb if (st is not None or not n_skip) else wrgb[n_skip:],
@@ -621,7 +739,9 @@
             fold.gpre, fold.sums, fold.gw = (gx_full if n_skip else gx), sums3, gw_full
         else:
             gx, gs = _modconv_raw(mode, gpre, wp_b, d, s, h, w, dot_with=x, out=gx_out, dot_out=gs_out)
-        if d is not None:
+        if d is not None and in_arena and sums is not None:
+            ctx.pool.tail.rows.append((ctx.tail_layer, sums, noise_w if noise is not None else None, bias, d, s, wsq, cin, cout, b))
+        elif d is not None:
             call("w2e_demod_bwd", ptr(sums), ptr(dz), ptr(noise_w) if (fuse_act and noise is not None) else None,
                  ptr(bias) if fuse_act else None, ptr(d), ptr(s), ptr(wsq), ptr(gs), None, b, cin, cout, stream_ptr())
         if n_skip:
@@ -658,6 +778,9 @@
         ctx.geom = (b, n_latent, dim)
         ctx.n_skip = _NOGRAD_PREFIX if _NOGRAD_PREFIX < b else 0
         ctx.pool = _GRAD_POOL
+        ctx.tail = None
+        if _BACKWARD_TAIL and ctx.pool is not None and latent.is_cuda:
+            ctx.tail = ctx.pool.tail = StyleTail(out, b, widths)
         outs, off = [], 0
         for cw in widths:
             outs.append(out[off * b:(off + cw) * b].view(b, cw))
@@ -672,10 +795,30 @@
         n_skip = ctx.n_skip
         b -= n_skip
         w, bias, meta, widths = ctx.pack
+        gs = list(gs)
+        tail = ctx.tail
+        glat_full, glat = _zeros_with_tail(b + n_skip, n_skip, (n_latent, dim), w.device, ctx.pool)
+        if tail is not None:
+            if tail.rows:
+                rows = []
+                for layer, sums, noise_w, bs, d, s, wsq, cin, cout, rb in tail.rows:
+                    if rb != b or gs[layer] is None:
+                        raise RuntimeError("where2edit_amd: a deferred demodulation term has no gradient tensor to be added to")
+                    if not (gs[layer].is_contiguous() and gs[layer].dtype == torch.float32):
+                        gs[layer] = gs[layer].to(torch.float32).contiguous()
+                    rows.append((sums, noise_w, bs, d, s, wsq, gs[layer][n_skip:] if n_skip else gs[layer], cin, cout))
+                _demod_bwd_all(rows, b)
+            arena = tail.arena
+            whole = arena is not None and all(g is None or tail.is_region(l, g) for l, g in enumerate(gs)) \
+                and all(g is not None or l not in tail.handed for l, g in enumerate(gs))
+            tail.reset()
+            if whole:
+                call("w2e_style_affine_bwd", ptr(arena), ptr(w), ctypes.c_void_p(meta.data_ptr()), ptr(glat_full), b + n_skip, n_latent,
+                     dim, w.shape[0], stream_ptr())
+                return glat_full, None
         parts = [(g[n_skip:].reshape(-1) if g is not None else torch.zeros(b * cw, device=w.device, dtype=torch.float32))
                  for g, cw in zip(gs, widths)]
         flat = torch.cat(parts)
-        glat_full, glat = _zeros_with_tail(b + n_skip, n_skip, (n_latent, dim), w.device, ctx.pool)
         call("w2e_style_affine_bwd", ptr(flat), ptr(w), ctypes.c_void_p(meta.data_ptr()), ptr(glat), b, n_latent, dim,
              w.shape[0], stream_ptr())
         return glat_full, None
@@ -713,6 +856,8 @@
             ctx.fold_out.saved = (x.detach(), wmod.detach(), style.detach() if style is not None else None, producer_act.noise, ctx.n_skip)
         ctx.has = (bias is not None, skip is not None, tuple(bias.shape) if bias is not None else None)
         ctx.pool = _GRAD_POOL
+        ctx.tail_layer = ctx.pool.tail.layer_of(style) if (style is not None and ctx.pool is not None and ctx.pool.tail is not None) else None
+        ctx.prezero = _BACKWARD_TAIL and ctx.pool is not None
         if passthrough:
             return y, x_in.view_as(x_in)
         return y
@@ -742,16 +887,18 @@
             xs, gys, gxs, accs = x, gy, gx, acc
         ws = wmod if style is not None else (wmod[n_skip:] if n_skip else wmod)
         sts = None if style is None else (style[n_skip:] if n_skip else style)
-        gw_full, gw = _zeros_with_tail(b, n_skip, (cin,) if style is not None else (3, cin), x.device, ctx.pool)
+        gw_full, gw, _ = _tail_zeros(ctx, ctx.tail_layer, b, n_skip, (cin,) if style is not None else (3, cin), x.device)
+        pre = "_prezeroed" if ctx.prezero else ""
         if ctx.link is not None:
-            sums3 = torch.empty((b - n_skip, cin, 3), device=x.device, dtype=torch.float32)
-            call("w2e_torgb_bwd_actbwd", ptr(xs), ptr(ws), ptr(sts), ptr(gys), ptr(accs), ptr(act_noise), ptr(gxs), ptr(gw), ptr(sums3),
+            sums3 = ctx.pool.zeros((b - n_skip, cin, 3), x.device) if ctx.prezero else \
+                torch.empty((b - n_skip, cin, 3), device=x.device, dtype=torch.float32)
+            call("w2e_torgb_bwd_actbwd" + pre, ptr(xs), ptr(ws), ptr(sts), ptr(gys), ptr(accs), ptr(act_noise), ptr(gxs), ptr(gw), ptr(sums3),
                  b - n_skip, cin, h, w, 0.2, SQRT2, stream_ptr())
             ctx.link.gpre, ctx.link.sums = gx, sums3
         elif style is None:
             call("w2e_torgb_bwd_acc", ptr(xs), ptr(ws), ptr(gys), ptr(accs), ptr(gxs), ptr(gw), b - n_skip, cin, h, w, stream_ptr())
         else:
-            call("w2e_torgb_styled_bwd", ptr(xs), ptr(ws), ptr(sts), ptr(gys), ptr(accs), ptr(gxs), ptr(gw), b - n_skip, cin, h, w,
+            call("w2e_torgb_styled_bwd" + pre, ptr(xs), ptr(ws), ptr(sts), ptr(gys), ptr(accs), ptr(gxs), ptr(gw), b - n_skip, cin, h, w,
                  stream_ptr())
         return (gx,) + _rgb_small_grads(ctx, gys, gw_full, wmod, style, upk, n_skip, b, h, w, x.device)
 
@@ -783,13 +930,19 @@
         out = torch.empty((n, c, 224, 224), device=img.device, dtype=torch.float32)
         call("w2e_clip_preproc_fwd", ptr(img), ptr(out), n * c, h, stream_ptr())
         ctx.shape = img.shape
+        ctx.link = _tail_link_of(img)
         return out
 
     @staticmethod
     @once_differentiable
     def backward(ctx, gout):
         n, c, h, w = ctx.shape
-        gimg = torch.empty(ctx.shape, device=gout.device, dtype=torch.float32)
+        link = ctx.link
+        if link is not None:
+            link.buf = _grad_rows((link.full, c, h, w), link.n, gout.device)
+            gimg = link.buf[link.n:]
+        else:
+            gimg = torch.empty(ctx.shape, device=gout.device, dtype=torch.float32)
         call("w2e_clip_preproc_bwd", ptr(_c(gout)), ptr(gimg), n * c, h, stream_ptr())
         return gimg
 
diff --git a/where2edit_amd/stylegan2.py b/where2edit_amd/stylegan2.py
--- a/where2edit_amd/stylegan2.py
+++ b/where2edit_amd/stylegan2.py
@@ -468,7 +468,8 @@
             return self._synthesis_pass(latent, noise, input_is_stylespace, on_layer, hook_layers)
         batch = (latent[0] if input_is_stylespace else latent).shape[0]
         widths = sum(m.conv.in_channel for m, _, _, _ in self._layers())
-        with K.grad_pool(batch * (3 * widths + 64 * (len(self._layers()) + 12) + self.n_latent * self.style_dim)):
+        sums = 3 * sum(m.conv.out_channel + 64 for m, is_rgb, _, _ in self._layers() if not is_rgb) if K.backward_tail_active() else 0
+        with K.grad_pool(batch * (3 * widths + sums + 64 * (len(self._layers()) + 12) + self.n_latent * self.style_dim)):
             return self._synthesis_pass(latent, noise, input_is_stylespace, on_layer, hook_layers)
 
     def _synthesis_pass(self, latent, noise, input_is_stylespace, on_layer, hook_layers):
```
